# Veason-silverbullet/NNR

Hardware: AMD Instinct MI355X
Metric: training impressions/sec on MIND-200k (CNE+SUE, bs=64) (higher is better)
Workload: dtype f32

## Files before the change

include/nnr_hip.h:

```cpp
#ifndef NNR_HIP_H
#define NNR_HIP_H
#include <stdint.h>
#include <hip/hip_runtime_api.h>

#ifdef __cplusplus
extern "C" {
#endif

#define NNR_OK 0
#define NNR_ERR_ARG (-1)
#define NNR_ERR_LAUNCH (-2)
#define NNR_ERR_UNSUPPORTED (-3)

int nnr_version(void);

typedef struct nnr_gemm_args {
  const float* A;
  const float* B;
  float* C;
  int M, N, K;
  int lda, ldb, ldc;
  int trans_a, trans_b;
  const int* dyn_dev;
  int dyn_dim;
  const int* a_idx;
  const int* b_idx;
  int drop_target;
  float drop_p;
  uint32_t drop_seed;
  int drop_cols;
  float alpha;
  const float* bias;
  const float* rowvec;
  int ldrv;
  const int* rowvec_map;
  int act;
  float* aux_out;
  int ldaux;
  const float* mul;
  int ldmul;
  const float* resid;
  int ldres;
  int accumulate;
  int atomic;
  const int* c_idx;
  int split_k;
  const float* rowdot_w;
  float* rowdot_out;
  int batch;
  long strideA, strideB, strideC, stride_aux, stride_res;
  int k_chunk;
  float* colsum_out;
  int tile;
  uint32_t drop_thresh;
  float drop_scale;
  int vec_epi;
  int sched;
  float* slab;
  long slab_floats;
  int slab_mode;
  const float* pre_add;
  int ldpre;
  int gate_bwd;
  const void* B3;
  long b3_stride;
  int ldb3;
} nnr_gemm_args;

int nnr_gemm_f32(const nnr_gemm_args* args, hipStream_t stream);
int nnr_split_bf16x3(const float* w, int rows, int cols, int ld, int ldo, void* out3, long img_stride, hipStream_t stream);

int nnr_seq_plan(uint8_t* mask, const int* ids, int n, int L, const int* perm_in, int* len_out, int* order, int* rank, int* slen,
                 int* bs, int* off, int* row_seq, int* tok, int* prev_f, int* prev_r, hipStream_t stream);

int nnr_seq_plan_pair(uint8_t* mask0, const int* ids0, int n0, uint8_t* mask1, const int* ids1, int n1, int L, const int* perm_in,
                      int* len_out, int* order, int* rank, int* slen, int* bs, int* off, int* row_seq, int* tok, int* prev_f,
                      int* prev_r, hipStream_t stream);

int nnr_cne_pair_map(const int* order_t, const int* order_c, int n0, int n, int* pm_t, int* pm_c, int* tmp, hipStream_t stream);

int nnr_mask_cover(const uint8_t* mask, int n, int L, uint8_t* cover, hipStream_t stream);
int nnr_seq_rowmap(const int* off, const int* rank, const int* len, int n, int L, int* rowmap, hipStream_t stream);

int nnr_lstm_dims(int H, int* UB, int* HP, int* NP);
int nnr_lstm_pack_weights(const float* w_ih_f, const float* w_hh_f, const float* b_ih_f, const float* b_hh_f, const float* w_ih_r,
                          const float* w_hh_r, const float* b_ih_r, const float* b_hh_r, int H, int E, float* w_ihp, float* b_p,
                          float* wf, float* wb, float* w_ihp_t, hipStream_t stream);
int nnr_lstm_unpack_grads(float* dw_ihp, float* db_p, float* dw_hhp, int H, int E, float* dw_ih_f, float* dw_hh_f,
                          float* db_ih_f, float* db_hh_f, float* dw_ih_r, float* dw_hh_r, float* db_ih_r, float* db_hh_r,
                          int accumulate , int zero_src, hipStream_t stream);
typedef struct nnr_lstm_problem {
  const int* bs; const int* off; const int* slen; const int* prev_f; const int* prev_r;
  int n, L;
  float* gates;
  float* cell;
  float* hout;
  float* cn;
  const float* wf;
  const float* wb;
  const float* dh;
  const float* dcn;
  unsigned* sync;
} nnr_lstm_problem;
size_t nnr_lstm_sync_bytes(int n);
size_t nnr_lstm_sync_diag_offset(int n);
int nnr_lstm_set_timeout_counter(unsigned* dev_counter);
int nnr_lstm_fwd(const nnr_lstm_problem* probs, int nprob, int H, hipStream_t stream);
int nnr_lstm_bwd(const nnr_lstm_problem* probs, int nprob, int H, hipStream_t stream);

typedef struct nnr_pool_args {
  const float* x; int ldx; int D; int n; int L;
  int packed;
  const int* off; const int* slen; const int* order;
  const uint8_t* mask; int mask_div;
  const float* score;
  const float* v; int ldv; float scale;
  float* alpha;
  float* out; int ldo; const float* add_in; int ldadd;
  const float* dout; int lddo; const float* dout2; int lddo2;
  float* dx; int lddx; int dx_accumulate;
  float* dscore;
  float* dv; int lddv;
  const float* th; int ldth; int A; const float* w2;
  const float* alpha_b; const float* dout_b; int lddo_b; const float* dscore_b; const float* v_b; int ldv_b; float scale_b;
} nnr_pool_args;
int nnr_attn_pool_fwd(const nnr_pool_args* a, hipStream_t stream);
int nnr_attn_pool_bwd(const nnr_pool_args* a, hipStream_t stream);

int nnr_gate_bwd(const float* dHt, const float* H, const float* G, float* dH, float* dpre, const int* rows_dev, int rows, int cols,
                 hipStream_t stream);
int nnr_packed_seq_sum(const float* x, int D, const int* off, const int* slen, int n, float* out, hipStream_t stream);
int nnr_slot_workspace_floats(int N);
int nnr_tanh_score_bwd(float* th, const float* ds, const float* w2, float* dw2, const int* rows_dev, int rows, int A, float* ws,
                       hipStream_t stream);
int nnr_colsum(const float* x, int ld, const int* rows_dev, int rows, int N, float* out_accum, float* ws, hipStream_t stream);
int nnr_rowdot(const float* x, int ld, const float* w, const int* rows_dev, int rows, int N, float* out,
               hipStream_t stream);
int nnr_small_embed_fwd(const float* table, const int* idx, int n, int dim, float* out, int ldo, float p, uint32_t seed,
                        hipStream_t stream);
int nnr_small_embed_bwd(const int* idx, int n, int dim, const float* dout, int lddo, float* dtable_accum, float p, uint32_t seed,
                        hipStream_t stream);
int nnr_embed_gather(const float* table, const int* idx, long n, const int* n_dev , int dim, float* out,
                     float p, uint32_t seed, hipStream_t stream);
int nnr_embed_scatter(const float* dout, const int* idx, long n, int dim, float* dtable_accum, float p, uint32_t seed,
                      hipStream_t stream);
int nnr_embed_scatter_dyn(const float* dout, const int* idx, long n, const int* n_dev, int dim, float* dtable, float p, uint32_t seed,
                          hipStream_t stream);
size_t nnr_token_sort_workspace_bytes(long cap, int vocab);
int nnr_token_sort(const int* tok, long cap, const int* n_dev, int vocab, unsigned* keys_tmp, int* rows_tmp, unsigned* keys_sorted,
                   int* rows_sorted, void* temp, size_t temp_bytes, hipStream_t stream);
size_t nnr_embed_scatter_sorted_workspace_floats(long cap);
int nnr_embed_scatter_sorted(const float* dout, const unsigned* keys_sorted, const int* rows_sorted, long cap, int vocab, int dim,
                             float* dtable_accum, float p, uint32_t seed, float* partial_ws, hipStream_t stream);
int nnr_transpose2d(const float* in, float* out, long rows, int cols, int accumulate, hipStream_t stream);
typedef struct nnr_transpose_desc { const float* in; float* out; int rows, cols; } nnr_transpose_desc;
int nnr_transpose_batch(const nnr_transpose_desc* descs_dev, int count, hipStream_t stream);
int nnr_add(float* y, const float* x, long n, float alpha, hipStream_t stream);
int nnr_add_atomic(float* y, const float* x, long n, float alpha, hipStream_t stream);
int nnr_add2d(float* y, int ldy, const float* x, int ldx, int rows, int cols, float alpha, int accumulate, hipStream_t stream);
int nnr_expand_rows_fwd(const float* x, float* y, int B, int N, int D, hipStream_t stream);
int nnr_expand_rows_bwd(const float* dy, float* dx, int B, int N, int D, hipStream_t stream);
int nnr_dropout(const float* x, float* y, long n, float p, uint32_t seed, hipStream_t stream);
int nnr_relu_bwd(const float* dy, const float* y, float* dx, long n, hipStream_t stream);
int nnr_gcn_aggregate_fwd(const float* graph, const float* z, const float* bias, const float* resid, float* r_out, float* y, int B, int G,
                          int D, int relu, float p, uint32_t seed, hipStream_t stream);
int nnr_gcn_aggregate_bwd(const float* graph, const float* dy, const float* r, float* ds, float* dx0, float* dz, int B, int G, int D, float p,
                          uint32_t seed, hipStream_t stream);
int nnr_relu_drop_bwd(const float* dy, const float* r, float* ds, float* dx, long n, float p, uint32_t seed, hipStream_t stream);

int nnr_mhsa_fwd(const float* qkv, const uint8_t* mask, int n, int Lq, int heads, int dh, float scale, float* out, float* prob,
                 float drop_p, uint32_t seed, hipStream_t stream);
int nnr_mhsa_bwd(const float* qkv, const uint8_t* mask, const float* prob, const float* dout, int n, int Lq, int heads, int dh,
                 float scale, float* dqkv, float drop_p, uint32_t seed, hipStream_t stream);
int nnr_mhsa_fwd_packed(const float* qkv, const uint8_t* mask, const int* rowmap, int n, int Lq, int heads, int dh, float scale, float* out,
                        float drop_p, uint32_t seed, hipStream_t stream);
int nnr_mhsa_bwd_packed(const float* qkv, const uint8_t* mask, const int* rowmap, const float* dout, int n, int Lq, int heads, int dh, float scale,
                        float* dqkv, float drop_p, uint32_t seed, hipStream_t stream);
int nnr_mhsa_pair_map(const int* off, const int* slen, const int* order, const uint8_t* mask, int n, int L, int* vrowmap, uint8_t* vmask,
                      hipStream_t stream);
int nnr_mhsa_fwd_paired(const float* qkv, const uint8_t* vmask, const int* vrowmap, const int* off, int n, int heads, int dh, float scale,
                        float* out, float drop_p, uint32_t seed, hipStream_t stream);
int nnr_mhsa_bwd_paired(const float* qkv, const uint8_t* vmask, const int* vrowmap, const int* off, const float* dout, int n, int heads, int dh,
                        float scale, float* dqkv, float drop_p, uint32_t seed, hipStream_t stream);

int nnr_sue_x0_fwd(const float* hist, const float* proxy, float* x0, int B, int Hn, int Kc, int D, float p, uint32_t seed,
                   uint8_t* cmask_fix, hipStream_t stream);
int nnr_sue_x0_bwd(const float* dx0, const float* dx0_add, float* dhist, float* dproxy_accum, int B, int Hn, int Kc, int D, float p,
                   uint32_t seed, hipStream_t stream);
int nnr_sue_slice_fwd(const float* gcn, const float* x0, float* gfeat, int B, int Hn, int G, int D, hipStream_t stream);
int nnr_sue_slice_bwd(const float* dgfeat, float* dpad, int B, int Hn, int G, int D, hipStream_t stream);
int nnr_sue_intra_fwd(const float* kf, const float* qc, const float* g, const long* cidx, int B, int N, int Hn, int C, int A, int D,
                      float* alpha, float* feat, hipStream_t stream);
int nnr_sue_intra_bwd(const float* kf, const float* qc, const float* g, const long* cidx, const float* alpha, const float* dfeat, int B,
                      int N, int Hn, int C, int A, int D, float* dg, float* dkf, float* dqc, float* ds_ws ,
                      hipStream_t stream);

int nnr_cand_attn_ws_floats(int B, int N, int H, int A);
int nnr_cand_attn_fwd(const float* P, const float* Q, const float* w2, const float* feat, int ldf, const uint8_t* mask, int B, int N,
                      int H, int A, int D, int act, float* alpha, float* out, hipStream_t stream);
int nnr_cand_attn_bwd(const float* P, const float* Q, const float* w2, const float* feat, int ldf, const uint8_t* mask, const float* alpha,
                      const float* dout, int B, int N, int H, int A, int D, int act, float* dP, float* dQ, float* dfeat,
                      int dfeat_accumulate, float* ws, float* dw2_accum, hipStream_t stream);

int nnr_omap_ws_floats(int B, int N, int H, int D, int K);
int nnr_omap_fwd(const float* hist, int ldf, const float* cand, const uint8_t* mask, const float* W, int B, int N, int H, int D, int K,
                 float* alpha, float* Y, float* beta, float* R, float* gamma, float* out, float* ws, hipStream_t stream);
int nnr_omap_bwd(const float* hist, int ldf, const float* cand, const uint8_t* mask, const float* W, const float* alpha, const float* Y,
                 const float* beta, const float* R, const float* gamma, const float* dout, int B, int N, int H, int D, int K, float* dhist,
                 int dhist_accumulate, float* dcand, float* dW_accum, float* ws, hipStream_t stream);
int nnr_omap_reg_fwd(const float* W, int D, int K, float coef, float* off, float* loss, hipStream_t stream);
int nnr_omap_reg_bwd(const float* W, const float* off, const float* gup, int D, int K, float coef, float* dW_accum, hipStream_t stream);

typedef struct nnr_corpus_tables {
  const int* news_category; const int* news_subCategory;
  const int* title_text; const uint8_t* title_mask; const int* title_entity;
  const int* abstract_text; const uint8_t* abstract_mask; const int* abstract_entity;
  const long* beh_user; const int* beh_history; const uint8_t* beh_history_mask; const int* beh_line;
  const float* graph_table; const uint8_t* cmask_table; const long* cidx_table;
  int T, C, H, G, K1;
} nnr_corpus_tables;
typedef struct nnr_batch_out {
  long* user_id;
  int* u_cat; int* u_sub; int* u_tt; uint8_t* u_tm; int* u_te; int* u_ct; uint8_t* u_cm; int* u_ce;
  uint8_t* u_hmask; float* u_graph; uint8_t* u_cmask; long* u_cidx;
  int* n_cat; int* n_sub; int* n_tt; uint8_t* n_tm; int* n_te; int* n_ct; uint8_t* n_cm; int* n_ce;
} nnr_batch_out;
int nnr_corpus_batch(const nnr_corpus_tables* t, const nnr_batch_out* o, const int* beh_idx, const int* samples, int ld_samples, int B,
                     int S, hipStream_t stream);
int nnr_history_graph(const int* cats, const uint8_t* hmask, int B, int H, int K, int norm, float* graph, uint8_t* cmask, long* cidx,
                      hipStream_t stream);
int nnr_rank_metrics(const float* scores, const uint8_t* labels, const long* offsets, int n_impressions, int* ranks,
                     double* per_impression, hipStream_t stream);

int nnr_logits_loss_fwd(const float* user, const float* cand, int B, int N, int D, float* logits, float* loss, float* dlogits,
                        hipStream_t stream);
int nnr_logits_fwd(const float* user, const float* cand, int B, int N, int D, float* logits, hipStream_t stream);
int nnr_nls_loss(const float* logits, int B, int N, float* loss, float* dlogits, hipStream_t stream);
int nnr_logits_bwd(const float* dlogits, const float* user, const float* cand, int B, int N, int D, float* duser, float* dcand,
                   int dcand_accumulate, hipStream_t stream);
int nnr_layernorm_fwd(const float* u, const float* gamma, const float* beta, float eps, long rows, int D, float* xhat, float* rstd,
                      float* r_out, const float* resid, float* y, float p, uint32_t seed, hipStream_t stream);
int nnr_layernorm_bwd(const float* dv, const float* xhat, const float* rstd, const float* gamma, long rows, int D, float* du,
                      float* dgamma, float* dbeta, hipStream_t stream);
int nnr_sumsq(const float* g, long n, float* out, hipStream_t stream);
int nnr_sumsq_part(const float* g, long n, float* out, const float* add_in, int slot, hipStream_t stream);
int nnr_clip_adam(float* p, const float* g, float* m, float* v, long n, const float* sumsq, float grad_scale, float clip, float lr,
                  float beta1, float beta2, float eps, float weight_decay, int step, hipStream_t stream);

int nnr_adam_skipped_steps(unsigned* host_out, int reset);
int nnr_adam_skipped_peek(unsigned* host_out);

typedef struct nnr_dp_ctx nnr_dp_ctx;
int nnr_dp_unique_id(void* out128);
int nnr_dp_init(const void* uid128, int rank, int world, nnr_dp_ctx** ctx);
int nnr_dp_allreduce(nnr_dp_ctx* ctx, float* flat, size_t n, hipStream_t stream);
int nnr_dp_broadcast(nnr_dp_ctx* ctx, float* flat, size_t n, int root, hipStream_t stream);
int nnr_dp_destroy(nnr_dp_ctx* ctx);
int nnr_dp_emulate_ranks(nnr_dp_ctx* ctx, int ranks);
int nnr_dp_busy(float* buf, long n, int workgroups, int iters, hipStream_t stream);
int nnr_rows_touch(const int* tok, long cap, const int* n_dev, int V, float* flags, hipStream_t stream);
int nnr_rows_compact(const float* flags, int V, int* pos, int* count, hipStream_t stream);
int nnr_rows_pack(const float* dense, const int* pos, int V, int E, float* packed, hipStream_t stream);
int nnr_rows_unpack(const float* packed, const int* pos, int V, int E, float* dense, hipStream_t stream);

int nnr_fusion_rows_fwd(const float* cat_table, const float* sub_table, const int* cat0, const int* sub0, int n0, const int* cat1,
                        const int* sub1, int n1, int cd, int sd, float* out, int ldo, float p, uint32_t seed_cat, uint32_t seed_sub,
                        hipStream_t stream);
int nnr_fusion_rows_bwd(const int* cat0, const int* sub0, int n0, const int* cat1, const int* sub1, int n1, int cd, int sd, const float* dout,
                        int lddo, float* dcat_table_accum, float* dsub_table_accum, float p, uint32_t seed_cat, uint32_t seed_sub,
                        hipStream_t stream);
int nnr_fusion_rows_bwd_det(const int* cat0, const int* sub0, int n0, const int* cat1, const int* sub1, int n1, int cd, int sd, int ncat,
                            int nsub, const float* dout, int lddo, float* dcat_table_accum, float* dsub_table_accum, float p,
                            uint32_t seed_cat, uint32_t seed_sub, hipStream_t stream);
int nnr_click_loss(const float* user, const float* cand, int B, int N, int D, float* logits, float* loss, float* dlogits, float* duser,
                   float* dcand, float* terms_ws, hipStream_t stream);

int nnr_fill_zero(void* p, size_t bytes, hipStream_t stream);
int nnr_copy_bytes(void* dst, const void* src, size_t bytes, hipStream_t stream);
int nnr_fill_column_u8(uint8_t* m, int rows, int cols, int col, int value, hipStream_t stream);

typedef struct nnr_tape nnr_tape;
int nnr_tape_create(nnr_tape** out);
int nnr_tape_destroy(nnr_tape* t);
int nnr_tape_fn_id(const char* entry_point_name);
int nnr_tape_fn_nargs(int fn);
int nnr_tape_call(nnr_tape* t, int fn, hipStream_t stream, const uint64_t* slots, int nslots, const int* blob_slot,
                  const void* const* blob_ptr, const size_t* blob_bytes, int nblobs, int tag, size_t* slot_off_out, size_t* blob_off_out);
int nnr_tape_wait_stream(nnr_tape* t, hipStream_t waiter, hipStream_t signaller);
int nnr_tape_event_record(nnr_tape* t, uint64_t key, hipStream_t s);
int nnr_tape_event_wait(nnr_tape* t, hipStream_t s, uint64_t key);
int nnr_tape_segment(nnr_tape* t);
int nnr_tape_patch(nnr_tape* t, size_t arena_byte_off, int kind, int width, int64_t addend);
int nnr_tape_finalize(nnr_tape* t);
int nnr_tape_prepare_timing(nnr_tape* t, int nsets);
int nnr_tape_info(const nnr_tape* t, int* calls, int* ops, int* segments, int* streams, size_t* arena_bytes);
int nnr_tape_replay(nnr_tape* t, int segment, const uint64_t* values, int nvalues, const uint64_t* inputs, int ninputs, int timing_set);
int nnr_tape_timings(nnr_tape* t, int set, float* ms, int n);
int nnr_tape_timeline(nnr_tape* t, int set, float* start_ms, float* dur_ms, int* stream_idx, int n);
int nnr_tape_last_error(const nnr_tape* t, int* rc, int* call, char* name, int name_cap);

#ifdef __cplusplus
}
#endif
#endif
```

nnr_amd/_lib.py:

```python
import ctypes as C
import os
import subprocess

_HERE = os.path.dirname(os.path.abspath(__file__))
LIB_PATH = os.environ.get('NNR_HIP_LIB') or os.path.join(_HERE, 'libnnr_hip.so')
_lib = None

vp, ci, cf, cu32, cl = C.c_void_p, C.c_int, C.c_float, C.c_uint32, C.c_long


class GemmArgs(C.Structure):
    _fields_ = [('A', vp), ('B', vp), ('C', vp), ('M', ci), ('N', ci), ('K', ci), ('lda', ci), ('ldb', ci), ('ldc', ci),
                ('trans_a', ci), ('trans_b', ci), ('dyn_dev', vp), ('dyn_dim', ci), ('a_idx', vp), ('b_idx', vp),
                ('drop_target', ci), ('drop_p', cf), ('drop_seed', cu32), ('drop_cols', ci), ('alpha', cf), ('bias', vp),
                ('rowvec', vp), ('ldrv', ci), ('rowvec_map', vp), ('act', ci), ('aux_out', vp), ('ldaux', ci), ('mul', vp),
                ('ldmul', ci), ('resid', vp), ('ldres', ci), ('accumulate', ci), ('atomic', ci), ('c_idx', vp),
                ('split_k', ci), ('rowdot_w', vp), ('rowdot_out', vp), ('batch', ci), ('strideA', cl), ('strideB', cl),
                ('strideC', cl), ('stride_aux', cl), ('stride_res', cl), ('k_chunk', ci), ('colsum_out', vp), ('tile', ci), ('drop_thresh', cu32),
                ('drop_scale', cf), ('vec_epi', ci), ('sched', ci), ('slab', vp), ('slab_floats', cl), ('slab_mode', ci), ('pre_add', vp), ('ldpre', ci), ('gate_bwd', ci), ('B3', vp), ('b3_stride', cl), ('ldb3', ci)]


class LstmProblem(C.Structure):
    _fields_ = [('bs', vp), ('off', vp), ('slen', vp), ('prev_f', vp), ('prev_r', vp), ('n', ci), ('L', ci), ('gates', vp),
                ('cell', vp), ('hout', vp), ('cn', vp), ('wf', vp), ('wb', vp), ('dh', vp), ('dcn', vp), ('sync', vp)]


class TransposeDesc(C.Structure):
    _fields_ = [('inp', vp), ('out', vp), ('rows', ci), ('cols', ci)]


class CorpusTables(C.Structure):
    _fields_ = [(k, vp) for k in ('news_category', 'news_subCategory', 'title_text', 'title_mask', 'title_entity', 'abstract_text',
                                  'abstract_mask', 'abstract_entity', 'beh_user', 'beh_history', 'beh_history_mask', 'beh_line',
                                  'graph_table', 'cmask_table', 'cidx_table')] + [(k, ci) for k in ('T', 'C', 'H', 'G', 'K1')]


class BatchOut(C.Structure):
    _fields_ = [(k, vp) for k in ('user_id', 'u_cat', 'u_sub', 'u_tt', 'u_tm', 'u_te', 'u_ct', 'u_cm', 'u_ce', 'u_hmask', 'u_graph',
                                  'u_cmask', 'u_cidx', 'n_cat', 'n_sub', 'n_tt', 'n_tm', 'n_te', 'n_ct', 'n_cm', 'n_ce')]


class PoolArgs(C.Structure):
    _fields_ = [('x', vp), ('ldx', ci), ('D', ci), ('n', ci), ('L', ci), ('packed', ci), ('off', vp), ('slen', vp),
                ('order', vp), ('mask', vp), ('mask_div', ci), ('score', vp), ('v', vp), ('ldv', ci), ('scale', cf),
                ('alpha', vp), ('out', vp), ('ldo', ci), ('add_in', vp), ('ldadd', ci), ('dout', vp), ('lddo', ci),
                ('dout2', vp), ('lddo2', ci), ('dx', vp), ('lddx', ci), ('dx_accumulate', ci), ('dscore', vp), ('dv', vp),
                ('lddv', ci), ('th', vp), ('ldth', ci), ('A', ci), ('w2', vp),
                ('alpha_b', vp), ('dout_b', vp), ('lddo_b', ci), ('dscore_b', vp), ('v_b', vp), ('ldv_b', ci), ('scale_b', cf)]


SIGNATURES = {
    'nnr_version': 'i32',
    'nnr_gemm_f32': 'i32 GemmArgs stream',
    'nnr_split_bf16x3': 'i32 ptr i32 i32 i32 i32 ptr i64 stream',
    'nnr_seq_plan': 'i32 ptr ptr i32 i32 ptr ptr ptr ptr ptr ptr ptr ptr ptr ptr ptr stream',
    'nnr_seq_plan_pair': 'i32 ptr ptr i32 ptr ptr i32 i32 ptr ptr ptr ptr ptr ptr ptr ptr ptr ptr ptr stream',
    'nnr_cne_pair_map': 'i32 ptr ptr i32 i32 ptr ptr ptr stream',
    'nnr_mask_cover': 'i32 ptr i32 i32 ptr stream',
    'nnr_seq_rowmap': 'i32 ptr ptr ptr i32 i32 ptr stream',
    'nnr_lstm_dims': 'i32 i32 ptr ptr ptr',
    'nnr_lstm_pack_weights': 'i32 ptr ptr ptr ptr ptr ptr ptr ptr i32 i32 ptr ptr ptr ptr ptr stream',
    'nnr_lstm_unpack_grads': 'i32 ptr ptr ptr i32 i32 ptr ptr ptr ptr ptr ptr ptr ptr i32 i32 stream',
    'nnr_lstm_sync_bytes': 'u64 i32',
    'nnr_lstm_sync_diag_offset': 'u64 i32',
    'nnr_lstm_set_timeout_counter': 'i32 ptr',
    'nnr_lstm_fwd': 'i32 LstmProblem i32 i32 stream',
    'nnr_lstm_bwd': 'i32 LstmProblem i32 i32 stream',
    'nnr_attn_pool_fwd': 'i32 PoolArgs stream',
    'nnr_attn_pool_bwd': 'i32 PoolArgs stream',
    'nnr_gate_bwd': 'i32 ptr ptr ptr ptr ptr ptr i32 i32 stream',
    'nnr_packed_seq_sum': 'i32 ptr i32 ptr ptr i32 ptr stream',
    'nnr_slot_workspace_floats': 'i32 i32',
    'nnr_tanh_score_bwd': 'i32 ptr ptr ptr ptr ptr i32 i32 ptr stream',
    'nnr_colsum': 'i32 ptr i32 ptr i32 i32 ptr ptr stream',
    'nnr_rowdot': 'i32 ptr i32 ptr ptr i32 i32 ptr stream',
    'nnr_small_embed_fwd': 'i32 ptr ptr i32 i32 ptr i32 f32 seed stream',
    'nnr_small_embed_bwd': 'i32 ptr i32 i32 ptr i32 ptr f32 seed stream',
    'nnr_embed_gather': 'i32 ptr ptr i64 ptr i32 ptr f32 seed stream',
    'nnr_embed_scatter': 'i32 ptr ptr i64 i32 ptr f32 seed stream',
    'nnr_embed_scatter_dyn': 'i32 ptr ptr i64 ptr i32 ptr f32 seed stream',
    'nnr_token_sort_workspace_bytes': 'u64 i64 i32',
    'nnr_token_sort': 'i32 ptr i64 ptr i32 ptr ptr ptr ptr ptr u64 stream',
    'nnr_embed_scatter_sorted_workspace_floats': 'u64 i64',
    'nnr_embed_scatter_sorted': 'i32 ptr ptr ptr i64 i32 i32 ptr f32 seed ptr stream',
    'nnr_transpose2d': 'i32 ptr ptr i64 i32 i32 stream',
    'nnr_transpose_batch': 'i32 TransposeDesc i32 stream',
    'nnr_add': 'i32 ptr ptr i64 f32 stream',
    'nnr_add_atomic': 'i32 ptr ptr i64 f32 stream',
    'nnr_add2d': 'i32 ptr i32 ptr i32 i32 i32 f32 i32 stream',
    'nnr_expand_rows_fwd': 'i32 ptr ptr i32 i32 i32 stream',
    'nnr_expand_rows_bwd': 'i32 ptr ptr i32 i32 i32 stream',
    'nnr_dropout': 'i32 ptr ptr i64 f32 seed stream',
    'nnr_relu_bwd': 'i32 ptr ptr ptr i64 stream',
    'nnr_gcn_aggregate_fwd': 'i32 ptr ptr ptr ptr ptr ptr i32 i32 i32 i32 f32 seed stream',
    'nnr_gcn_aggregate_bwd': 'i32 ptr ptr ptr ptr ptr ptr i32 i32 i32 f32 seed stream',
    'nnr_relu_drop_bwd': 'i32 ptr ptr ptr ptr i64 f32 seed stream',
    'nnr_mhsa_fwd': 'i32 ptr ptr i32 i32 i32 i32 f32 ptr ptr f32 seed stream',
    'nnr_mhsa_bwd': 'i32 ptr ptr ptr ptr i32 i32 i32 i32 f32 ptr f32 seed stream',
    'nnr_mhsa_fwd_packed': 'i32 ptr ptr ptr i32 i32 i32 i32 f32 ptr f32 seed stream',
    'nnr_mhsa_bwd_packed': 'i32 ptr ptr ptr ptr i32 i32 i32 i32 f32 ptr f32 seed stream',
    'nnr_mhsa_pair_map': 'i32 ptr ptr ptr ptr i32 i32 ptr ptr stream',
    'nnr_mhsa_fwd_paired': 'i32 ptr ptr ptr ptr i32 i32 i32 f32 ptr f32 seed stream',
    'nnr_mhsa_bwd_paired': 'i32 ptr ptr ptr ptr ptr i32 i32 i32 f32 ptr f32 seed stream',
    'nnr_sue_x0_fwd': 'i32 ptr ptr ptr i32 i32 i32 i32 f32 seed ptr stream',
    'nnr_sue_x0_bwd': 'i32 ptr ptr ptr ptr i32 i32 i32 i32 f32 seed stream',
    'nnr_sue_slice_fwd': 'i32 ptr ptr ptr i32 i32 i32 i32 stream',
    'nnr_sue_slice_bwd': 'i32 ptr ptr i32 i32 i32 i32 stream',
    'nnr_sue_intra_fwd': 'i32 ptr ptr ptr ptr i32 i32 i32 i32 i32 i32 ptr ptr stream',
    'nnr_sue_intra_bwd': 'i32 ptr ptr ptr ptr ptr ptr i32 i32 i32 i32 i32 i32 ptr ptr ptr ptr stream',
    'nnr_cand_attn_ws_floats': 'i32 i32 i32 i32 i32',
    'nnr_cand_attn_fwd': 'i32 ptr ptr ptr ptr i32 ptr i32 i32 i32 i32 i32 i32 ptr ptr stream',
    'nnr_cand_attn_bwd': 'i32 ptr ptr ptr ptr i32 ptr ptr ptr i32 i32 i32 i32 i32 i32 ptr ptr ptr i32 ptr ptr stream',
    'nnr_omap_ws_floats': 'i32 i32 i32 i32 i32 i32',
    'nnr_omap_fwd': 'i32 ptr i32 ptr ptr ptr i32 i32 i32 i32 i32 ptr ptr ptr ptr ptr ptr ptr stream',
    'nnr_omap_bwd': 'i32 ptr i32 ptr ptr ptr ptr ptr ptr ptr ptr ptr i32 i32 i32 i32 i32 ptr i32 ptr ptr ptr stream',
    'nnr_omap_reg_fwd': 'i32 ptr i32 i32 f32 ptr ptr stream',
    'nnr_omap_reg_bwd': 'i32 ptr ptr ptr i32 i32 f32 ptr stream',
    'nnr_corpus_batch': 'i32 CorpusTables BatchOut ptr ptr i32 i32 i32 stream',
    'nnr_history_graph': 'i32 ptr ptr i32 i32 i32 i32 ptr ptr ptr stream',
    'nnr_rank_metrics': 'i32 ptr ptr ptr i32 ptr ptr stream',
    'nnr_logits_loss_fwd': 'i32 ptr ptr i32 i32 i32 ptr ptr ptr stream',
    'nnr_logits_fwd': 'i32 ptr ptr i32 i32 i32 ptr stream',
    'nnr_nls_loss': 'i32 ptr i32 i32 ptr ptr stream',
    'nnr_logits_bwd': 'i32 ptr ptr ptr i32 i32 i32 ptr ptr i32 stream',
    'nnr_layernorm_fwd': 'i32 ptr ptr ptr f32 i64 i32 ptr ptr ptr ptr ptr f32 seed stream',
    'nnr_layernorm_bwd': 'i32 ptr ptr ptr ptr i64 i32 ptr ptr ptr stream',
    'nnr_sumsq': 'i32 ptr i64 ptr stream',
    'nnr_sumsq_part': 'i32 ptr i64 ptr ptr i32 stream',
    'nnr_clip_adam': 'i32 ptr ptr ptr ptr i64 ptr f32 f32 f32 f32 f32 f32 f32 i32 stream',
    'nnr_adam_skipped_steps': 'i32 ptr i32',
    'nnr_adam_skipped_peek': 'i32 ptr',
    'nnr_dp_unique_id': 'i32 ptr',
    'nnr_dp_init': 'i32 ptr i32 i32 handle',
    'nnr_dp_allreduce': 'i32 handle ptr u64 stream',
    'nnr_dp_broadcast': 'i32 handle ptr u64 i32 stream',
    'nnr_dp_destroy': 'i32 handle',
    'nnr_dp_emulate_ranks': 'i32 handle i32',
    'nnr_dp_busy': 'i32 ptr i64 i32 i32 stream',
    'nnr_rows_touch': 'i32 ptr i64 ptr i32 ptr stream',
    'nnr_rows_compact': 'i32 ptr i32 ptr ptr stream',
    'nnr_rows_pack': 'i32 ptr ptr i32 i32 ptr stream',
    'nnr_rows_unpack': 'i32 ptr ptr i32 i32 ptr stream',
    'nnr_fusion_rows_fwd': 'i32 ptr ptr ptr ptr i32 ptr ptr i32 i32 i32 ptr i32 f32 seed seed stream',
    'nnr_fusion_rows_bwd': 'i32 ptr ptr i32 ptr ptr i32 i32 i32 ptr i32 ptr ptr f32 seed seed stream',
    'nnr_fusion_rows_bwd_det': 'i32 ptr ptr i32 ptr ptr i32 i32 i32 i32 i32 ptr i32 ptr ptr f32 seed seed stream',
    'nnr_click_loss': 'i32 ptr ptr i32 i32 i32 ptr ptr ptr ptr ptr ptr stream',
    'nnr_fill_zero': 'i32 ptr u64 stream',
    'nnr_copy_bytes': 'i32 ptr ptr u64 stream',
    'nnr_fill_column_u8': 'i32 ptr i32 i32 i32 i32 stream',
    'nnr_tape_create': 'i32 handle',
    'nnr_tape_destroy': 'i32 handle',
    'nnr_tape_fn_id': 'i32 cstr',
    'nnr_tape_fn_nargs': 'i32 i32',
    'nnr_tape_call': 'i32 handle i32 stream ptr i32 ptr ptr ptr i32 i32 ptr ptr',
    'nnr_tape_wait_stream': 'i32 handle stream stream',
    'nnr_tape_event_record': 'i32 handle u64 stream',
    'nnr_tape_event_wait': 'i32 handle stream u64',
    'nnr_tape_segment': 'i32 handle',
    'nnr_tape_patch': 'i32 handle u64 i32 i32 i64',
    'nnr_tape_finalize': 'i32 handle',
    'nnr_tape_prepare_timing': 'i32 handle i32',
    'nnr_tape_info': 'i32 handle ptr ptr ptr ptr ptr',
    'nnr_tape_replay': 'i32 handle i32 ptr i32 ptr i32 i32',
    'nnr_tape_timings': 'i32 handle i32 ptr i32',
    'nnr_tape_timeline': 'i32 handle i32 ptr ptr ptr i32',
    'nnr_tape_last_error': 'i32 handle ptr ptr cstr i32',
}
SYMBOLS = list(SIGNATURES)
STRUCTS = {'nnr_gemm_args': GemmArgs, 'nnr_lstm_problem': LstmProblem, 'nnr_pool_args': PoolArgs, 'nnr_transpose_desc': TransposeDesc,
           'nnr_corpus_tables': CorpusTables, 'nnr_batch_out': BatchOut}
DEVICE_STRUCTS = {'TransposeDesc'}
_CTYPES = {'i32': ci, 'i64': cl, 'u64': C.c_size_t, 'f32': cf, 'seed': cu32, 'ptr': vp, 'handle': vp, 'cstr': C.c_char_p, 'stream': vp}
_CTYPES.update((c.__name__, vp if c.__name__ in DEVICE_STRUCTS else C.POINTER(c)) for c in STRUCTS.values())


def kinds(name):
    return SIGNATURES[name].split()[1:]


class NnrHipError(RuntimeError):
    pass


def build(force=False):
    if force:
        bdir = os.path.join(_HERE, 'csrc', 'build')
        if os.path.isdir(bdir):
            for f in os.listdir(bdir):
                os.remove(os.path.join(bdir, f))
    subprocess.check_call(['bash', os.path.join(_HERE, 'csrc', 'build.sh')])
    return LIB_PATH


def lib():
    global _lib
    if _lib is None:
        if not os.path.exists(LIB_PATH):
            raise NnrHipError('libnnr_hip.so not found at %s -- run `python -c "import __graft_entry__ as g; g.build()"` '
                              '(there is no CPU / PyTorch fallback on the product path)' % LIB_PATH)
        import torch
        _lib = C.CDLL(LIB_PATH)
        for name, sig in SIGNATURES.items():
            ret, *params = [_CTYPES[k] for k in sig.split()]
            fn = getattr(_lib, name)
            fn.restype, fn.argtypes = ret, params
    return _lib


def build_id():
    import hashlib
    h = hashlib.sha256()
    src = os.path.join(_HERE, 'csrc')
    for f in sorted(os.listdir(src)):
        if f.endswith(('.hip', '.h')):
            h.update(f.encode())
            h.update(open(os.path.join(src, f), 'rb').read())
    h.update(open(os.path.join(os.path.dirname(_HERE), 'include', 'nnr_hip.h'), 'rb').read())
    lib_hash = hashlib.sha256(open(LIB_PATH, 'rb').read()).hexdigest()[:16] if os.path.exists(LIB_PATH) else None
    return {'src_sha256': h.hexdigest()[:16], 'lib_sha256': lib_hash}


CALLS = [0]


def check(rc, what):
    CALLS[0] += 1
    if rc != 0:
        raise NnrHipError('%s failed with code %d' % (what, rc))
```

nnr_amd/csrc/gcn.hip:

```cpp
#include "common.h"

namespace {

constexpr int GCN_MAXG = 128;

template <int MODE, int MT>
__global__ __launch_bounds__(256) __attribute__((amdgpu_waves_per_eu(3, 8))) void gcn_aggregate_kernel(
    const float* __restrict__ graph, const float* __restrict__ in, const float* __restrict__ bias, const float* __restrict__ aux_in,
    float* __restrict__ out0, float* __restrict__ out1, float* __restrict__ out2, int G, int D, int relu, uint32_t seed, uint32_t thr, float scale) {
  extern __shared__ __attribute__((aligned(16))) float sm[];
  const int ks_n = (G + 3) >> 2, GR = ks_n * 4;
  const int A_LD = GR | 1;
  constexpr int Z_LD = 68;
  float* As = sm;
  float* Zs = sm + ((GR * A_LD + 3) & ~3);
  const int b = blockIdx.y, tid = threadIdx.x, lane = tid & 63, w = tid >> 6;
  const int r16 = lane & 15, kk = lane >> 4;
  const float* A = graph + (long)b * G * G;
  if ((G & 3) == 0) {
    const int g4 = G >> 2;
    for (int i = tid; i < G * g4; i += 256) {
      const int row = i / g4, c = (i - row * g4) * 4;
      const f32x4 v = *reinterpret_cast<const f32x4*>(A + row * G + c);
#pragma unroll
      for (int e = 0; e < 4; ++e) As[row * A_LD + c + e] = v[e];
    }
  } else {
    for (int i = tid; i < GR * A_LD; i += 256) {
      const int row = i / A_LD, col = i - row * A_LD;
      As[i] = (row < G && col < G) ? A[row * G + col] : 0.f;
    }
  }
  const int c0 = blockIdx.x * 64;
  const int c4 = (tid & 15) * 4, rr = tid >> 4;
  const bool cok = c0 + c4 < D;
  const long base = (long)b * G * D;
#pragma unroll
  for (int pass = 0; pass < MT; ++pass) {
    const int row = pass * 16 + rr;
    f32x4 v = {0.f, 0.f, 0.f, 0.f};
    if (row < G && cok) {
      const long idx = base + (long)row * D + c0 + c4;
      v = *reinterpret_cast<const f32x4*>(in + idx);
      if (MODE == 1 && aux_in) {
        if (thr) {
          bool kp[4];
          nnr_keep4(seed, (uint64_t)idx, thr, kp);
#pragma unroll
          for (int e = 0; e < 4; ++e) v[e] = kp[e] ? v[e] * scale : 0.f;
        }
        if (out1) *reinterpret_cast<f32x4*>(out1 + idx) = v;
        const f32x4 rv = *reinterpret_cast<const f32x4*>(aux_in + idx);
#pragma unroll
        for (int e = 0; e < 4; ++e) v[e] = rv[e] > 0.f ? v[e] : 0.f;
        *reinterpret_cast<f32x4*>(out0 + idx) = v;
      }
    }
    if (row < GR) *reinterpret_cast<f32x4*>(&Zs[row * Z_LD + c4]) = v;
  }
  __syncthreads();
  float bf[MT * 4];
#pragma unroll
  for (int ks = 0; ks < MT * 4; ++ks) bf[ks] = ks < ks_n ? Zs[(4 * ks + kk) * Z_LD + w * 16 + r16] : 0.f;
  f32x4 acc[MT];
  int arow[MT];
#pragma unroll
  for (int m = 0; m < MT; ++m) {
    acc[m] = f32x4{0.f, 0.f, 0.f, 0.f};
    arow[m] = min(m * 16 + r16, GR - 1);
  }
#pragma unroll
  for (int ks = 0; ks < MT * 4; ++ks) {
    if (ks < ks_n) {
#pragma unroll
      for (int m = 0; m < MT; ++m) {
        const float a = MODE == 0 ? As[arow[m] * A_LD + 4 * ks + kk] : As[(4 * ks + kk) * A_LD + arow[m]];
        acc[m] = __builtin_amdgcn_mfma_f32_16x16x4f32(a, bf[ks], acc[m], 0, 0, 0);
      }
    }
  }
  __syncthreads();
#pragma unroll
  for (int m = 0; m < MT; ++m)
#pragma unroll
    for (int e = 0; e < 4; ++e)
      if (m * 16 + 4 * kk + e < GR) Zs[(m * 16 + 4 * kk + e) * Z_LD + w * 16 + r16] = acc[m][e];
  __syncthreads();
  if (!cok) return;
  f32x4 bv = {0.f, 0.f, 0.f, 0.f};
  if (MODE == 0 && bias) bv = *reinterpret_cast<const f32x4*>(bias + c0 + c4);
#pragma unroll
  for (int pass = 0; pass < MT; ++pass) {
    const int row = pass * 16 + rr;
    if (row < G) {
      const long idx = base + (long)row * D + c0 + c4;
      f32x4 x = *reinterpret_cast<const f32x4*>(&Zs[row * Z_LD + c4]);
      if (MODE == 0) {
        x += bv;
        if (relu) {
#pragma unroll
          for (int e = 0; e < 4; ++e) x[e] = fmaxf(x[e], 0.f);
        }
        if (out1) *reinterpret_cast<f32x4*>(out1 + idx) = x;
        if (aux_in) x += *reinterpret_cast<const f32x4*>(aux_in + idx);
        if (thr) {
          bool kp[4];
          nnr_keep4(seed, (uint64_t)idx, thr, kp);
#pragma unroll
          for (int e = 0; e < 4; ++e) x[e] = kp[e] ? x[e] * scale : 0.f;
        }
        *reinterpret_cast<f32x4*>(out0 + idx) = x;
      } else {
        *reinterpret_cast<f32x4*>(out2 + idx) = x;
      }
    }
  }
}


}

extern "C" int nnr_gcn_aggregate_fwd(const float* graph, const float* z, const float* bias, const float* resid, float* r_out, float* y, int B,
                                     int G, int D, int relu, float p, uint32_t seed, hipStream_t stream) {
  if (!graph || !z || !y || B <= 0 || G <= 0 || D <= 0) return NNR_ERR_ARG;
  if (G > GCN_MAXG || (D & 3)) return NNR_ERR_UNSUPPORTED;
  const float sc = p > 0.f ? 1.f / (1.f - p) : 1.f;
  const int gp = (G + 15) / 16 * 16, gr = (G + 3) / 4 * 4;
#define GCN_CASE(MT_) case MT_: hipLaunchKernelGGL((gcn_aggregate_kernel<0, MT_>), dim3((D + 63) / 64, B), dim3(256), (size_t)(((gr * (gr | 1) + 3) & ~3) + gr * 68) * sizeof(float), \
                                                   stream, graph, z, bias, resid, y, r_out, nullptr, G, D, relu, seed, nnr_drop_thresh(p), sc); break;
  switch (gp / 16) { GCN_CASE(1) GCN_CASE(2) GCN_CASE(3) GCN_CASE(4) GCN_CASE(5) GCN_CASE(6) GCN_CASE(7) GCN_CASE(8) }
#undef GCN_CASE
  NNR_CHECK_LAUNCH();
  return NNR_OK;
}

extern "C" int nnr_gcn_aggregate_bwd(const float* graph, const float* dy, const float* r, float* ds, float* dx0, float* dz, int B, int G, int D,
                                     float p, uint32_t seed, hipStream_t stream) {
  if (!graph || !dy || !dz || B <= 0 || G <= 0 || D <= 0 || (r && !ds)) return NNR_ERR_ARG;
  if (G > GCN_MAXG || (D & 3)) return NNR_ERR_UNSUPPORTED;
  const float sc = p > 0.f ? 1.f / (1.f - p) : 1.f;
  const int gp = (G + 15) / 16 * 16, gr = (G + 3) / 4 * 4;
#define GCN_CASE(MT_) case MT_: hipLaunchKernelGGL((gcn_aggregate_kernel<1, MT_>), dim3((D + 63) / 64, B), dim3(256), (size_t)(((gr * (gr | 1) + 3) & ~3) + gr * 68) * sizeof(float), \
                                                   stream, graph, dy, nullptr, r, ds, dx0, dz, G, D, 0, seed, nnr_drop_thresh(p), sc); break;
  switch (gp / 16) { GCN_CASE(1) GCN_CASE(2) GCN_CASE(3) GCN_CASE(4) GCN_CASE(5) GCN_CASE(6) GCN_CASE(7) GCN_CASE(8) }
#undef GCN_CASE
  NNR_CHECK_LAUNCH();
  return NNR_OK;
}
```

nnr_amd/csrc/gemm.hip:

```cpp
#include "common.h"
#include <stdlib.h>
#include <type_traits>

namespace {

template <int BK>
__device__ __forceinline__ int swz(int r16) {
  return BK == 16 ? ((4 - (r16 >> 2)) & 3) : BK == 32 ? ((r16 >> 1) & 7) : (r16 & 15);
}

template <int TM, int TN>
__device__ __forceinline__ void gemm_epilogue(const nnr_gemm_args& g, f32x4 (&acc)[TM][TN], float* lds, float* __restrict__ C, int m0,
                                              int n0, int M, int N, int z) {
  constexpr int BN = 16 * TN, E_LD = BN + 4;
  const int tid = threadIdx.x, lane = tid & 63, w = tid >> 6;
  const int r = lane & 15, kk = lane >> 4;
  const uint32_t dthr = g.drop_thresh;
  const float dscale = g.drop_scale;
  const bool use_atomic = !g.slab_mode && (g.atomic || g.split_k > 1 || g.k_chunk > 0);
  float* aux = g.aux_out;
  const float* res = g.resid;
  const float* mulp = g.mul;
  if (g.batch > 1 && g.split_k <= 1 && g.k_chunk <= 0) {
    if (aux) aux += (long)z * g.stride_aux;
    if (res) res += (long)z * g.stride_res;
  }
  float* stage = lds;
#pragma unroll
  for (int m = 0; m < TM; ++m) {
    if (m > 0) __syncthreads();
#pragma unroll
    for (int n = 0; n < TN; ++n)
#pragma unroll
      for (int reg = 0; reg < 4; ++reg) stage[(w * 16 + kk * 4 + reg) * E_LD + n * 16 + r] = acc[m][n][reg];
    __syncthreads();
    if (g.rowdot_w) {
      for (int lr = w; lr < 64; lr += 4) {
        const int row = m0 + (lr >> 4) * (TM * 16) + m * 16 + (lr & 15);
        float dot = 0.f;
        if (row < M) {
          for (int c = lane; c < BN; c += 64) {
            const int col = n0 + c;
            if (col < N) {
              float x = stage[lr * E_LD + c] * g.alpha;
              if (g.bias) x += g.bias[col];
              if (g.act == 1) x = fmaxf(x, 0.f);
              else if (g.act == 2) x = fast_tanh(x);
              else if (g.act == 3) x = fast_sigmoid(x);
              if (aux) aux[(long)row * g.ldaux + col] = x;
              dot += g.rowdot_w[col] * x;
              if (C) C[(long)row * g.ldc + col] = x;
            }
          }
        }
        dot = wave_sum(dot);
        if (row < M && lane == 0) g.rowdot_out[row] = dot;
      }
    } else if (g.vec_epi) {
      constexpr int NV = BN / 4;
      for (int idx = tid; idx < 64 * NV; idx += 256) {
        const int lr = idx / NV, c4 = idx - lr * NV;
        const int row = m0 + (lr >> 4) * (TM * 16) + m * 16 + (lr & 15);
        const int col = n0 + 4 * c4;
        if (row >= M || col >= N) continue;
        f32x4 x = *reinterpret_cast<const f32x4*>(&stage[lr * E_LD + 4 * c4]) * g.alpha;
        if (g.pre_add) x += *reinterpret_cast<const f32x4*>(g.pre_add + (long)row * g.ldpre + col);
        if (g.gate_bwd) {
          const f32x4 gv = *reinterpret_cast<const f32x4*>(mulp + (long)row * g.ldmul + col);
          const f32x4 hv = *reinterpret_cast<const f32x4*>(res + (long)row * g.ldres + col);
          *reinterpret_cast<f32x4*>(aux + (long)row * g.ldaux + col) = x * hv * gv * (1.f - gv);
          *reinterpret_cast<f32x4*>(C + (long)row * g.ldc + col) = x * gv;
          continue;
        }
        if (g.accumulate == 2) x += *reinterpret_cast<const f32x4*>(C + (long)row * g.ldc + col);
        if (g.bias) x += *reinterpret_cast<const f32x4*>(g.bias + col);
        if (g.rowvec) x += *reinterpret_cast<const f32x4*>(g.rowvec + (long)(g.rowvec_map ? g.rowvec_map[row] : row) * g.ldrv + col);
        if (g.act == 1) {
#pragma unroll
          for (int e = 0; e < 4; ++e) x[e] = fmaxf(x[e], 0.f);
        } else if (g.act == 2) {
#pragma unroll
          for (int e = 0; e < 4; ++e) x[e] = fast_tanh(x[e]);
        } else if (g.act == 3) {
#pragma unroll
          for (int e = 0; e < 4; ++e) x[e] = fast_sigmoid(x[e]);
        }
        if (aux) *reinterpret_cast<f32x4*>(aux + (long)row * g.ldaux + col) = x;
        if (mulp) x *= *reinterpret_cast<const f32x4*>(mulp + (long)row * g.ldmul + col);
        if (res) x += *reinterpret_cast<const f32x4*>(res + (long)row * g.ldres + col);
        if (g.drop_target == 3) {
          bool kp[4];
          nnr_keep4(g.drop_seed, (uint64_t)(row + (long)z * g.M) * g.drop_cols + col, dthr, kp);
#pragma unroll
          for (int e = 0; e < 4; ++e) x[e] = kp[e] ? x[e] * dscale : 0.f;
        }
        if (C) {
          f32x4* cp = reinterpret_cast<f32x4*>(C + (long)row * g.ldc + col);
          if (g.accumulate == 1) x += *cp;
          *cp = x;
        }
      }
    } else {
      for (int idx = tid; idx < 64 * BN; idx += 256) {
        const int lr = idx / BN, c = idx - lr * BN;
        const int row = m0 + (lr >> 4) * (TM * 16) + m * 16 + (lr & 15);
        const int col = n0 + c;
        if (row >= M || col >= N) continue;
        int crow = row;
        if (g.c_idx) { crow = g.c_idx[row]; if (crow < 0) continue; }
        float x = stage[lr * E_LD + c] * g.alpha;
        if (g.accumulate == 2) x += C[(long)crow * g.ldc + col];
        if (g.bias) x += g.bias[col];
        if (g.rowvec) x += g.rowvec[(long)(g.rowvec_map ? g.rowvec_map[row] : row) * g.ldrv + col];
        if (g.act == 1) x = fmaxf(x, 0.f);
        else if (g.act == 2) x = fast_tanh(x);
        else if (g.act == 3) x = fast_sigmoid(x);
        if (aux) aux[(long)row * g.ldaux + col] = x;
        if (mulp) x *= mulp[(long)row * g.ldmul + col];
        if (res) x += res[(long)row * g.ldres + col];
        if (g.drop_target == 3)
          x = nnr_keep(g.drop_seed, (uint64_t)(row + (long)z * g.M) * g.drop_cols + col, dthr) ? x * dscale : 0.f;
        if (C) {
          float* cp = C + (long)crow * g.ldc + col;
          if (use_atomic) {
            if (g.drop_target == 4)
              x = nnr_keep(g.drop_seed, (uint64_t)row * g.drop_cols + col, dthr) ? x * dscale : 0.f;
            atomicAdd(cp, x);
          } else {
            if (g.accumulate == 1) x += *cp;
            *cp = x;
          }
        }
      }
    }
  }
}

template <int TM, int TN, bool TA, bool TB, int BK>
__global__ __launch_bounds__(256) void gemm_kernel(nnr_gemm_args g) {
  constexpr int BM = 64 * TM, BN = 16 * TN;
  constexpr int A_LD = BM + 4, B_LD = BN + 4;
  constexpr int KQ = BK / 4, NKG = BK / 16;
  constexpr int A_SZ = TA ? BK * A_LD : BM * BK;
  constexpr int B_SZ = TB ? BK * B_LD : BN * BK;
  constexpr int NAL = BM * KQ / 256;
  constexpr int NBL = (BN * KQ + 255) / 256;
  constexpr int E_LD = BN + 4;
  constexpr int LDS_FLOATS = (2 * (A_SZ + B_SZ) > 64 * E_LD) ? 2 * (A_SZ + B_SZ) : 64 * E_LD;
  __shared__ __attribute__((aligned(16))) float lds[LDS_FLOATS];

  const int tid = threadIdx.x, lane = tid & 63, w = tid >> 6;
  const int r = lane & 15, kk = lane >> 4;

// ... 127 lines not shown
              if (vecB && gn + 3 < N) {
                val = *reinterpret_cast<const f32x4*>(p);
              } else {
#pragma unroll
                for (int e = 0; e < 4; ++e) if (gn + e < N) val[e] = p[e];
              }
              if (g.drop_target == 2) {
                bool kp[4];
                if ((g.drop_cols & 3) == 0) nnr_keep4(g.drop_seed, (uint64_t)gk * g.drop_cols + gn, dthr, kp);
                else {
#pragma unroll
                  for (int e = 0; e < 4; ++e) kp[e] = nnr_keep(g.drop_seed, (uint64_t)gk * g.drop_cols + (gn + e), dthr);
                }
#pragma unroll
                for (int e = 0; e < 4; ++e) val[e] = kp[e] ? val[e] * dscale : 0.f;
              }
            }
          }
        }
      }
      rb[j] = val;
    }
  };

  auto store_tiles = [&](int buf) {
    float* As = lds + buf * (A_SZ + B_SZ);
    float* Bs = As + A_SZ;
#pragma unroll
    for (int j = 0; j < NAL; ++j) {
      const int f = tid + 256 * j;
      if (!TA) {
        const int row = f / KQ, kq = f % KQ;
        *reinterpret_cast<f32x4*>(&As[row * BK + 4 * (kq ^ swz<BK>(row & 15))]) = ra[j];
      } else {
        const int kr = f / (BM / 4), mq = f - kr * (BM / 4);
        *reinterpret_cast<f32x4*>(&As[kr * A_LD + 4 * mq]) = ra[j];
      }
    }
#pragma unroll
    for (int j = 0; j < NBL; ++j) {
      const int f = tid + 256 * j;
      if (f < BN * KQ || TB) {
        if (!TB) {
          const int row = f / KQ, kq = f % KQ;
          *reinterpret_cast<f32x4*>(&Bs[row * BK + 4 * (kq ^ swz<BK>(row & 15))]) = rb[j];
        } else {
          const int kr = f / (BN / 4), nq = f - kr * (BN / 4);
          if (kr < BK) *reinterpret_cast<f32x4*>(&Bs[kr * B_LD + 4 * nq]) = rb[j];
        }
      }
    }
  };

  f32x4 acc[TM][TN];
#pragma unroll
  for (int m = 0; m < TM; ++m)
#pragma unroll
    for (int n = 0; n < TN; ++n) acc[m][n] = f32x4{0.f, 0.f, 0.f, 0.f};

  load_tiles(kbeg);
  if (do_colsum) {
#pragma unroll
    for (int j = 0; j < NAL; ++j) csum[j] += ra[j];
  }
  store_tiles(0);
  __syncthreads();

  int buf = 0;
  for (int k0 = kbeg; k0 < kend; k0 += BK) {
    const bool more = (k0 + BK) < kend;
    if (more) {
      load_tiles(k0 + BK);
      if (do_colsum) {
#pragma unroll
        for (int j = 0; j < NAL; ++j) csum[j] += ra[j];
      }
    }

    const float* As = lds + buf * (A_SZ + B_SZ);
    const float* Bs = As + A_SZ;
#pragma unroll
    for (int kg2 = 0; kg2 < NKG; ++kg2) {
      f32x4 af[TM], bf[TN];
#pragma unroll
      for (int m = 0; m < TM; ++m) {
        if (!TA) {
          af[m] = *reinterpret_cast<const f32x4*>(&As[((w * TM + m) * 16 + r) * BK + 4 * ((kg2 * 4 + kk) ^ swz<BK>(r))]);
        } else {
#pragma unroll
          for (int i = 0; i < 4; ++i) af[m][i] = As[(kg2 * 16 + 4 * kk + i) * A_LD + (w * TM + m) * 16 + r];
        }
      }
#pragma unroll
      for (int n = 0; n < TN; ++n) {
        if (!TB) {
          bf[n] = *reinterpret_cast<const f32x4*>(&Bs[(n * 16 + r) * BK + 4 * ((kg2 * 4 + kk) ^ swz<BK>(r))]);
        } else {
#pragma unroll
          for (int i = 0; i < 4; ++i) bf[n][i] = Bs[(kg2 * 16 + 4 * kk + i) * B_LD + n * 16 + r];
        }
      }
#pragma unroll
      for (int i = 0; i < 4; ++i)
#pragma unroll
        for (int m = 0; m < TM; ++m)
#pragma unroll
          for (int n = 0; n < TN; ++n)
            acc[m][n] = __builtin_amdgcn_mfma_f32_16x16x4f32(af[m][i], bf[n][i], acc[m][n], 0, 0, 0);
    }

    if (more) store_tiles(buf ^ 1);
    __syncthreads();
    buf ^= 1;
  }

  if (do_colsum) {
    float* red = lds;
#pragma unroll
    for (int j = 0; j < NAL; ++j) {
      const int f = tid + 256 * j, kr = f / (BM / 4), mq = f - kr * (BM / 4);
      *reinterpret_cast<f32x4*>(&red[kr * BM + 4 * mq]) = csum[j];
    }
    __syncthreads();
    for (int i = tid; i < BM; i += 256) {
      float t = 0.f;
      for (int kr = 0; kr < BK; ++kr) t += red[kr * BM + i];
      if (m0 + i < M) {
        if (g.slab_mode) g.colsum_out[(long)z * M + m0 + i] = t;
        else atomicAdd(&g.colsum_out[m0 + i], t);
      }
    }
    __syncthreads();
  }

  gemm_epilogue<TM, TN>(g, acc, lds, g.slab_mode ? C + (long)z * M * N : C, m0, n0, M, N, z);
}

template <int TM, int TN, int BK>
int launch_cfg(const nnr_gemm_args& g, hipStream_t s) {
  constexpr int BM = 64 * TM, BN = 16 * TN;
  const int nbm = (g.M + BM - 1) / BM, nbn = (g.N + BN - 1) / BN;
  if (g.rowdot_w && nbn != 1) return NNR_ERR_ARG;
  dim3 grid(nbm * nbn, 1, g.k_chunk > 0 ? (g.K + g.k_chunk - 1) / g.k_chunk : (g.split_k > 1 ? g.split_k : (g.batch > 1 ? g.batch : 1)));
  dim3 block(256);
  if (!g.trans_a && !g.trans_b) hipLaunchKernelGGL((gemm_kernel<TM, TN, false, false, BK>), grid, block, 0, s, g);
  else if (!g.trans_a && g.trans_b) hipLaunchKernelGGL((gemm_kernel<TM, TN, false, true, BK>), grid, block, 0, s, g);
  else if (g.trans_a && g.trans_b) hipLaunchKernelGGL((gemm_kernel<TM, TN, true, true, BK>), grid, block, 0, s, g);
  else return NNR_ERR_ARG;
  NNR_CHECK_LAUNCH();
  return NNR_OK;
}


__device__ __attribute__((aligned(1024))) float nnr_zero_page[512] = {};

__device__ __forceinline__ void lds_dma16(const float* gsrc, unsigned lds_dst) {
  unsigned keep;
  asm volatile("s_mov_b32 %0, m0\n\ts_mov_b32 m0, %2\n\ts_nop 0\n\tglobal_load_lds_dwordx4 %1, off\n\ts_mov_b32 m0, %0"
               : "=&s"(keep) : "v"(gsrc), "s"(lds_dst) : "memory");
}
__device__ __forceinline__ void set_prio_dyn(unsigned p) {
  switch (p & 3) {
    case 0: __builtin_amdgcn_s_setprio(0); break;
    case 1: __builtin_amdgcn_s_setprio(1); break;
    case 2: __builtin_amdgcn_s_setprio(2); break;
    default: __builtin_amdgcn_s_setprio(3); break;
  }
}

template <int N>
__device__ __forceinline__ void wait_vmcnt() { asm volatile("s_waitcnt vmcnt(%0)" ::"n"(N) : "memory"); }
template <int CNT, int MAXA>
__device__ __forceinline__ void wait_stages(int ahead) {
  if constexpr (MAXA == 0) wait_vmcnt<0>();
  else {
    if (ahead >= MAXA) wait_vmcnt<CNT * MAXA>();
    else wait_stages<CNT, MAXA - 1>(ahead);
  }
}

template <int TM, int TN, int BK, int NS, int OCC, int PRIO = 0>
__global__ __launch_bounds__(256, OCC) void gemm_nt_pipe_kernel(nnr_gemm_args g) {
  if (PRIO == 1) set_prio_dyn(blockIdx.x >> 8);
  if (PRIO == 2) set_prio_dyn(blockIdx.x >> 5);
  if (PRIO == 3) set_prio_dyn(blockIdx.x);
  constexpr int BM = 64 * TM, BN = 16 * TN, ROWS = BM + BN;
  constexpr int KQ = BK / 4, NKG = BK / 16;
  constexpr int RPI = 64 / KQ;
  constexpr int NI = ROWS / RPI;
  constexpr int NPW = (NI + 3) / 4;
  constexpr int STAGE = ROWS * BK;
  constexpr int E_LD = BN + 4;
  constexpr int LDS_FLOATS = (NS * STAGE > 64 * E_LD) ? NS * STAGE : 64 * E_LD;
  static_assert(ROWS % RPI == 0, "tile rows must fill whole DMA instructions");
  __shared__ __attribute__((aligned(1024))) float lds[LDS_FLOATS];

  const int tid = threadIdx.x, lane = tid & 63, w = __builtin_amdgcn_readfirstlane(tid >> 6);
  const int r = lane & 15, kk = lane >> 4;

  int M = g.M;
  if (g.dyn_dim == 1) M = min(M, *g.dyn_dev);
  const int N = g.N, K = g.K;
  const int nbm = (M + BM - 1) / BM, nbn = (N + BN - 1) / BN;
  const int nblk = nbm * nbn;
  if ((int)blockIdx.x >= nblk) return;
  int v;
  {
    const int b = blockIdx.x, q = nblk >> 3, rem = nblk & 7, x = b & 7, slot = b >> 3;
    v = x * q + min(x, rem) + slot;
  }
  const int bm = v / nbn, bn = v - bm * nbn;
  const int m0 = bm * BM, n0 = bn * BN;
  const int z = blockIdx.z;
  const float* __restrict__ A = g.A;
  const float* __restrict__ B = g.B;
  float* __restrict__ C = g.C;
  if (g.batch > 1) {
    A += (long)z * g.strideA;
    B += (long)z * g.strideB;
    C += (long)z * g.strideC;
  }

  const float* rowp[NPW];
  int kch[NPW];
#pragma unroll
  for (int i = 0; i < NPW; ++i) {
    const int q = w + 4 * i;
    const int tr = q * RPI + lane / KQ;
    const int c = (lane % KQ) ^ swz<BK>(tr & 15);
    kch[i] = 4 * c;
    const float* p = nullptr;
    if (q < NI) {
      if (tr < BM) {
        const int gm = m0 + tr;
        if (gm < M) {
          const int src = g.a_idx ? g.a_idx[gm] : gm;
          if (src >= 0) p = A + (long)src * g.lda + 4 * c;
        }
      } else {
        const int gn = n0 + (tr - BM);
        if (gn < N) p = B + (long)gn * g.ldb + 4 * c;
      }
    }
    rowp[i] = p;
  }
  const float* zero = nnr_zero_page;
  asm volatile("" : "+s"(zero));
  const unsigned lds_base = (unsigned)(uintptr_t)lds;
  const int S = (K + BK - 1) / BK;

  auto issue = [&](int s) {
    const int k0 = s * BK;
    const unsigned sb = lds_base + (unsigned)((s % NS) * STAGE * 4);
#pragma unroll
    for (int i = 0; i < NPW; ++i) {
      const int q = w + 4 * i;
      if (q < NI) {
        const float* src = (rowp[i] != nullptr && k0 + kch[i] < K) ? rowp[i] + k0 : zero;
        lds_dma16(src, sb + (unsigned)(q * 1024));
      }
    }
  };

  f32x4 acc[TM][TN];
#pragma unroll
  for (int m = 0; m < TM; ++m)
#pragma unroll
    for (int n = 0; n < TN; ++n) acc[m][n] = f32x4{0.f, 0.f, 0.f, 0.f};

#pragma unroll
  for (int s = 0; s < NS - 1; ++s)
    if (s < S) issue(s);

  const int nv = (g.sched & 1) ? min(TN, (N - n0 + 15) >> 4) : TN;
  auto run = [&](auto full_tag) {
    constexpr bool FULL = decltype(full_tag)::value;
    for (int s = 0; s < S; ++s) {
      const int ahead = S - 1 - s;
      if (NI % 4 == 0 || w < NI % 4) wait_stages<NPW, NS - 2>(ahead);
      else wait_stages<NPW - 1, NS - 2>(ahead);
      __builtin_amdgcn_s_barrier();
      if (s + NS - 1 < S) issue(s + NS - 1);

      const float* As = lds + (s % NS) * STAGE;
      const float* Bs = As + BM * BK;
#pragma unroll
      for (int kg = 0; kg < NKG; ++kg) {
        f32x4 af[TM], bf[TN];
#pragma unroll
        for (int m = 0; m < TM; ++m)
          af[m] = *reinterpret_cast<const f32x4*>(&As[((w * TM + m) * 16 + r) * BK + 4 * ((kg * 4 + kk) ^ swz<BK>(r))]);
        if constexpr (FULL) {
#pragma unroll
          for (int n = 0; n < TN; ++n)
            bf[n] = *reinterpret_cast<const f32x4*>(&Bs[(n * 16 + r) * BK + 4 * ((kg * 4 + kk) ^ swz<BK>(r))]);
#pragma unroll
          for (int i = 0; i < 4; ++i)
#pragma unroll
            for (int m = 0; m < TM; ++m)
#pragma unroll
              for (int n = 0; n < TN; ++n)
                acc[m][n] = __builtin_amdgcn_mfma_f32_16x16x4f32(af[m][i], bf[n][i], acc[m][n], 0, 0, 0);
        } else {
#pragma unroll
          for (int n = 0; n < TN; ++n)
            if (n < nv) bf[n] = *reinterpret_cast<const f32x4*>(&Bs[(n * 16 + r) * BK + 4 * ((kg * 4 + kk) ^ swz<BK>(r))]);
#pragma unroll
          for (int n = 0; n < TN; ++n)
            if (n < nv) {
#pragma unroll
              for (int i = 0; i < 4; ++i)
#pragma unroll
                for (int m = 0; m < TM; ++m) acc[m][n] = __builtin_amdgcn_mfma_f32_16x16x4f32(af[m][i], bf[n][i], acc[m][n], 0, 0, 0);
            }
        }
      }
    }
  };
  if (nv == TN) run(std::true_type{});
  else run(std::false_type{});
  __syncthreads();
  gemm_epilogue<TM, TN>(g, acc, lds, C, m0, n0, M, N, z);
}

template <int N>
__device__ __forceinline__ void lds_dma16_block(const float* sbase, unsigned lds_dst, const unsigned (&voff)[8]) {
  unsigned keep;
  static_assert(N >= 1 && N <= 8, "1..8 loads per block");
#define NNR_DMA_HEAD "s_mov_b32 %[keep], m0\n\ts_mov_b32 m0, %[dst]\n\t"
#define NNR_DMA_LD(I) "s_nop 0\n\tglobal_load_lds_dwordx4 %[v" #I "], %[sb]\n\ts_add_u32 m0, m0, 0x1000\n\t"
#define NNR_DMA_TAIL "s_mov_b32 m0, %[keep]"
#define NNR_DMA_OPS : [keep] "=&s"(keep) : [dst] "s"(lds_dst), [sb] "s"(sbase), [v0] "v"(voff[0]), [v1] "v"(voff[1]), [v2] "v"(voff[2]), [v3] "v"(voff[3]), \
                      [v4] "v"(voff[4]), [v5] "v"(voff[5]), [v6] "v"(voff[6]), [v7] "v"(voff[7]) : "memory", "scc"
  if constexpr (N == 1) asm volatile(NNR_DMA_HEAD NNR_DMA_LD(0) NNR_DMA_TAIL NNR_DMA_OPS);
  if constexpr (N == 2) asm volatile(NNR_DMA_HEAD NNR_DMA_LD(0) NNR_DMA_LD(1) NNR_DMA_TAIL NNR_DMA_OPS);
  if constexpr (N == 3) asm volatile(NNR_DMA_HEAD NNR_DMA_LD(0) NNR_DMA_LD(1) NNR_DMA_LD(2) NNR_DMA_TAIL NNR_DMA_OPS);
  if constexpr (N == 4) asm volatile(NNR_DMA_HEAD NNR_DMA_LD(0) NNR_DMA_LD(1) NNR_DMA_LD(2) NNR_DMA_LD(3) NNR_DMA_TAIL NNR_DMA_OPS);
  if constexpr (N == 5) asm volatile(NNR_DMA_HEAD NNR_DMA_LD(0) NNR_DMA_LD(1) NNR_DMA_LD(2) NNR_DMA_LD(3) NNR_DMA_LD(4) NNR_DMA_TAIL NNR_DMA_OPS);
  if constexpr (N == 6) asm volatile(NNR_DMA_HEAD NNR_DMA_LD(0) NNR_DMA_LD(1) NNR_DMA_LD(2) NNR_DMA_LD(3) NNR_DMA_LD(4) NNR_DMA_LD(5) NNR_DMA_TAIL NNR_DMA_OPS);
  if constexpr (N == 7) asm volatile(NNR_DMA_HEAD NNR_DMA_LD(0) NNR_DMA_LD(1) NNR_DMA_LD(2) NNR_DMA_LD(3) NNR_DMA_LD(4) NNR_DMA_LD(5) NNR_DMA_LD(6) NNR_DMA_TAIL NNR_DMA_OPS);
  if constexpr (N == 8) asm volatile(NNR_DMA_HEAD NNR_DMA_LD(0) NNR_DMA_LD(1) NNR_DMA_LD(2) NNR_DMA_LD(3) NNR_DMA_LD(4) NNR_DMA_LD(5) NNR_DMA_LD(6) NNR_DMA_LD(7) NNR_DMA_TAIL NNR_DMA_OPS);
#undef NNR_DMA_HEAD
#undef NNR_DMA_LD
#undef NNR_DMA_TAIL
#undef NNR_DMA_OPS
}

template <int TM, int TN, int NS, int OCC>
__global__ __launch_bounds__(256, OCC) void gemm_nt_pipe2_kernel(nnr_gemm_args g) {
  constexpr int BK = 32, BM = 64 * TM, BN = 16 * TN, ROWS = BM + BN;
  constexpr int KQ = BK / 4, RPI = 64 / KQ, NI = ROWS / RPI, NPW = (NI + 3) / 4, STAGE = ROWS * BK, E_LD = BN + 4;
  constexpr int LDS_FLOATS = (NS * STAGE > 64 * E_LD) ? NS * STAGE : 64 * E_LD;
  static_assert(ROWS % RPI == 0 && NS >= 3, "tile shape");
  __shared__ __attribute__((aligned(1024))) float lds[LDS_FLOATS];
  const int tid = threadIdx.x, lane = tid & 63, w = __builtin_amdgcn_readfirstlane(tid >> 6);
  const int r = lane & 15, kk = lane >> 4;
  int M = g.M;
  if (g.dyn_dim == 1) M = min(M, *g.dyn_dev);
  const int N = g.N, K = g.K;
  const int nbm = (M + BM - 1) / BM, nbn = (N + BN - 1) / BN;
  const int nblk = nbm * nbn;
  if ((int)blockIdx.x >= nblk) return;
  int v;
  {
    const int b = blockIdx.x, q = nblk >> 3, rem = nblk & 7, x = b & 7, slot = b >> 3;
    v = x * q + min(x, rem) + slot;
  }
  const int bm = v / nbn, bn = v - bm * nbn;
  const int m0 = bm * BM, n0 = bn * BN;
  const int z = blockIdx.z;
  const float* __restrict__ A = g.A;
  const float* __restrict__ B = g.B;
  float* __restrict__ C = g.C;
  if (g.batch > 1) {
    A += (long)z * g.strideA;
    B += (long)z * g.strideB;
    C += (long)z * g.strideC;
  }
  constexpr int NIA = BM / RPI, NIB = BN / RPI, NA = NIA / 4, NBMAX = (NIB + 3) / 4;
  static_assert(NIA % 4 == 0 && NA <= 8 && NBMAX <= 8, "tile shape");
  unsigned voffA[8], voffB[8];
  int kchA[NA], kchB[NBMAX];
#pragma unroll
  for (int i = 0; i < 8; ++i) voffA[i] = voffB[i] = 0;
#pragma unroll
  for (int i = 0; i < NA; ++i) {
    const int tr = (w + 4 * i) * RPI + lane / KQ;
    const int c = (lane % KQ) ^ swz<BK>(tr & 15);
    kchA[i] = 4 * c;
    voffA[i] = (unsigned)(((long)min(tr, M - 1 - m0) * g.lda + 4 * c) * 4);
  }
#pragma unroll
  for (int j = 0; j < NBMAX; ++j) {
    const int tr = (w + 4 * j) * RPI + lane / KQ;
    const int c = (lane % KQ) ^ swz<BK>(tr & 15);
    kchB[j] = 4 * c;
    voffB[j] = (unsigned)(((long)min(tr, N - 1 - n0) * g.ldb + 4 * c) * 4);
  }
  const float* zero = nnr_zero_page;
  asm volatile("" : "+s"(zero));
  const unsigned lds_base = (unsigned)(uintptr_t)lds;
  const int S = (K + BK - 1) / BK;
  const float* Abase = A + (long)m0 * g.lda;
  const float* Bbase = B + (long)n0 * g.ldb;
  const bool ktail = (K % BK) != 0;
  const bool nb_hi = (NIB % 4 == 0) || (w < NIB % 4);
  auto issue_lean = [&](int s) {
    const int k0 = s * BK;
    const unsigned sb = lds_base + (unsigned)((s % NS) * STAGE * 4) + (unsigned)(w * 1024);
    lds_dma16_block<NA>(Abase + k0, sb, voffA);
    if (nb_hi) lds_dma16_block<NBMAX>(Bbase + k0, sb + NIA * 1024, voffB);
    else if constexpr (NBMAX > 1) lds_dma16_block<NBMAX - 1>(Bbase + k0, sb + NIA * 1024, voffB);
  };
  auto issue = [&](int s) {
    if (!(ktail && s == S - 1)) { issue_lean(s); return; }
    const int k0 = s * BK;
    const unsigned sb = lds_base + (unsigned)((s % NS) * STAGE * 4) + (unsigned)(w * 1024);
#pragma unroll
    for (int i = 0; i < NA; ++i)
      lds_dma16((k0 + kchA[i] < K) ? reinterpret_cast<const float*>(reinterpret_cast<const char*>(Abase + k0) + voffA[i]) : zero, sb + i * 4096);
#pragma unroll
    for (int j = 0; j < NBMAX; ++j)
      if (j < NBMAX - 1 || nb_hi)
        lds_dma16((k0 + kchB[j] < K) ? reinterpret_cast<const float*>(reinterpret_cast<const char*>(Bbase + k0) + voffB[j]) : zero,
                  sb + NIA * 1024 + j * 4096);
  };
  auto wait_landed = [&](int ahead) {
    if (NI % 4 == 0 || w < NI % 4) wait_stages<NPW, NS - 3>(ahead);
    else wait_stages<NPW - 1, NS - 3>(ahead);
  };
  f32x4 acc[TM][TN];
#pragma unroll
  for (int m = 0; m < TM; ++m)
#pragma unroll
    for (int n = 0; n < TN; ++n) acc[m][n] = f32x4{0.f, 0.f, 0.f, 0.f};
  f32x4 fa0[TM], fb0[TN], fa1[TM], fb1[TN];
  const int nv = (g.sched & 1) ? min(TN, (N - n0 + 15) >> 4) : TN;
  const int klast = (g.sched & 1) ? K - (S - 1) * BK : BK;
  auto run = [&](auto full_tag) {
    constexpr bool FULL = decltype(full_tag)::value;
    auto rd = [&](int s, int kg, f32x4 (&a)[TM], f32x4 (&b)[TN]) {
      const float* As = lds + (s % NS) * STAGE;
      const float* Bs = As + BM * BK;
#pragma unroll
      for (int m = 0; m < TM; ++m)
        a[m] = *reinterpret_cast<const f32x4*>(&As[((w * TM + m) * 16 + r) * BK + 4 * ((kg * 4 + kk) ^ swz<BK>(r))]);
#pragma unroll
      for (int n = 0; n < TN; ++n)
        if (FULL || n < nv) b[n] = *reinterpret_cast<const f32x4*>(&Bs[(n * 16 + r) * BK + 4 * ((kg * 4 + kk) ^ swz<BK>(r))]);
    };
    auto mm = [&](const f32x4 (&a)[TM], const f32x4 (&b)[TN], int steps) {
      if constexpr (FULL) {
#pragma unroll
        for (int i = 0; i < 4; ++i)
          if (i < steps) {
#pragma unroll
            for (int m = 0; m < TM; ++m)
#pragma unroll
              for (int n = 0; n < TN; ++n) acc[m][n] = __builtin_amdgcn_mfma_f32_16x16x4f32(a[m][i], b[n][i], acc[m][n], 0, 0, 0);
          }
      } else {
#pragma unroll
        for (int n = 0; n < TN; ++n)
          if (n < nv) {
#pragma unroll
            for (int i = 0; i < 4; ++i)
              if (i < steps) {
#pragma unroll
                for (int m = 0; m < TM; ++m) acc[m][n] = __builtin_amdgcn_mfma_f32_16x16x4f32(a[m][i], b[n][i], acc[m][n], 0, 0, 0);
              }
          }
      }
    };
    auto mm4 = [&](const f32x4 (&a)[TM], const f32x4 (&b)[TN]) {
      if constexpr (FULL) {
#pragma unroll
        for (int i = 0; i < 4; ++i)
#pragma unroll
          for (int m = 0; m < TM; ++m)
#pragma unroll
            for (int n = 0; n < TN; ++n) acc[m][n] = __builtin_amdgcn_mfma_f32_16x16x4f32(a[m][i], b[n][i], acc[m][n], 0, 0, 0);
      } else {
        mm(a, b, 4);
      }
    };

#pragma unroll
    for (int s = 0; s < NS - 1; ++s)
      if (s < S) issue(s);
    if (NI % 4 == 0 || w < NI % 4) wait_stages<NPW, NS - 2>(S - 1); else wait_stages<NPW - 1, NS - 2>(S - 1);
    __builtin_amdgcn_s_barrier();
    rd(0, 0, fa0, fb0);
    __builtin_amdgcn_s_waitcnt(0xC07F);
#define NNR_LGKM0() do { __builtin_amdgcn_sched_barrier(0); __builtin_amdgcn_s_waitcnt(0xC07F); } while (0)
    int s = 0;
    for (; s + NS < S; ++s) {
      rd(s, 1, fa1, fb1);
      __builtin_amdgcn_sched_barrier(0);
      mm4(fa0, fb0);
      NNR_LGKM0();
      wait_landed(NS);
      __builtin_amdgcn_s_barrier();
      issue_lean(s + NS - 1);
      rd(s + 1, 0, fa0, fb0);
      __builtin_amdgcn_sched_barrier(0);
      mm4(fa1, fb1);
      NNR_LGKM0();
    }
    for (; s + 1 < S; ++s) {
      rd(s, 1, fa1, fb1);
      __builtin_amdgcn_sched_barrier(0);
      mm4(fa0, fb0);
      NNR_LGKM0();
      wait_landed(S - 1 - (s + 1));
      __builtin_amdgcn_s_barrier();
      if (s + NS - 1 < S) issue(s + NS - 1);
      rd(s + 1, 0, fa0, fb0);
      __builtin_amdgcn_sched_barrier(0);
      mm4(fa1, fb1);
      NNR_LGKM0();
    }
#undef NNR_LGKM0
    rd(S - 1, 1, fa1, fb1);
    __builtin_amdgcn_sched_barrier(0);
    mm(fa0, fb0, min(4, klast));
    if (klast > 16) mm(fa1, fb1, min(4, klast - 16));
  };
  if (nv == TN) run(std::true_type{});
  else run(std::false_type{});
  __syncthreads();
  gemm_epilogue<TM, TN>(g, acc, lds, C, m0, n0, M, N, z);
}

constexpr int kNtRagged = 1;

template <int TM, int TN, int NS, int OCC>
int launch_pipe2(const nnr_gemm_args& g0, hipStream_t s) {
  constexpr int BM = 64 * TM, BN = 16 * TN;
  nnr_gemm_args g = g0;
  g.sched = kNtRagged;
  const int nbm = (g.M + BM - 1) / BM, nbn = (g.N + BN - 1) / BN;
  dim3 grid(nbm * nbn, 1, g.batch > 1 ? g.batch : 1), block(256);
  hipLaunchKernelGGL((gemm_nt_pipe2_kernel<TM, TN, NS, OCC>), grid, block, 0, s, g);
  NNR_CHECK_LAUNCH();
  return NNR_OK;
}

template <int TM, int TN, int BK, int NS, int OCC, int PRIO = 0>
int launch_pipe(const nnr_gemm_args& g0, hipStream_t s) {
  constexpr int BM = 64 * TM, BN = 16 * TN;
  nnr_gemm_args g = g0;
  g.sched = kNtRagged;
  const int nbm = (g.M + BM - 1) / BM, nbn = (g.N + BN - 1) / BN;
  dim3 grid(nbm * nbn, 1, g.batch > 1 ? g.batch : 1), block(256);
  hipLaunchKernelGGL((gemm_nt_pipe_kernel<TM, TN, BK, NS, OCC, PRIO>), grid, block, 0, s, g);
  NNR_CHECK_LAUNCH();
  return NNR_OK;
}

static bool pipe_ok(const nnr_gemm_args& g) {
  auto al = [](const void* p) { return ((uintptr_t)p & 15) == 0; };
  return !g.trans_a && !g.trans_b && !g.b_idx && g.split_k <= 1 && g.k_chunk <= 0 && !g.rowdot_w && !g.colsum_out &&
         (g.drop_target == 0 || g.drop_target == 3 || g.drop_target == 4) && (g.K & 3) == 0 && (g.lda & 3) == 0 && (g.ldb & 3) == 0 &&
         al(g.A) && al(g.B) && (g.batch <= 1 || (((g.strideA | g.strideB) & 3) == 0)) && (g.dyn_dim == 0 || g.dyn_dim == 1);
}

typedef __bf16 bf16x8_t __attribute__((ext_vector_type(8)));
__device__ __forceinline__ void split3_bf16(float x, __bf16& h1, __bf16& h2, __bf16& h3) {
  const unsigned u = __builtin_bit_cast(unsigned, x), mag = u & 0x7fffffffu;
  const bool big = mag >= 0x7f7f8000u, nonfinite = mag >= 0x7f800000u;
  h1 = (__bf16)x;
  if (big) h1 = __builtin_bit_cast(__bf16, (unsigned short)((u >> 16) | (mag > 0x7f800000u ? 0x40u : 0u)));
  const float r1 = nonfinite ? 0.f : x - (float)h1;
  h2 = (__bf16)r1;
  const float r2 = r1 - (float)h2;
  h3 = (__bf16)r2;
}
__global__ void split_bf16x3_kernel(const float* __restrict__ w, int rows, int cols, int ld, int ldo, __bf16* __restrict__ out, long img_stride) {
  const long total = (long)rows * ldo;
  for (long i = blockIdx.x * (long)blockDim.x + threadIdx.x; i < total; i += (long)gridDim.x * blockDim.x) {
    const int r = (int)(i / ldo), c = (int)(i - (long)r * ldo);
    __bf16 a, b, d;
    split3_bf16(c < cols ? w[(long)r * ld + c] : 0.f, a, b, d);
    out[i] = a; out[img_stride + i] = b; out[2 * img_stride + i] = d;
  }
}
__device__ __forceinline__ int bx3_swzA(int r) { return ((r >> 1) & 1) | (((r >> 3) & 1) << 2); }
__device__ __forceinline__ int bx3_swzB(int r) { return (r >> 1) & 3; }

typedef unsigned u32x4_t __attribute__((ext_vector_type(4)));
__device__ __forceinline__ unsigned hi16_pair(float odd, float even) {
  return __builtin_amdgcn_perm(__float_as_uint(odd), __float_as_uint(even), 0x07060302u);
}
__device__ __forceinline__ void split3_trunc8(const f32x4& x0, const f32x4& x1, bf16x8_t& a1, bf16x8_t& a2, bf16x8_t& a3) {
  const float xs[8] = {x0[0], x0[1], x0[2], x0[3], x1[0], x1[1], x1[2], x1[3]};
  unsigned w1[4], w2[4], w3[4];
#pragma unroll
  for (int p = 0; p < 4; ++p) {
    const float xe = xs[2 * p], xo = xs[2 * p + 1];
    const unsigned h1 = hi16_pair(xo, xe);
    const float re = xe - __uint_as_float(h1 << 16), ro = xo - __uint_as_float(h1 & 0xffff0000u);
    const unsigned h2 = hi16_pair(ro, re);
    const float se = re - __uint_as_float(h2 << 16), so = ro - __uint_as_float(h2 & 0xffff0000u);
    w1[p] = h1; w2[p] = h2; w3[p] = hi16_pair(so, se);
  }
  a1 = __builtin_bit_cast(bf16x8_t, u32x4_t{w1[0], w1[1], w1[2], w1[3]});
  a2 = __builtin_bit_cast(bf16x8_t, u32x4_t{w2[0], w2[1], w2[2], w2[3]});
  a3 = __builtin_bit_cast(bf16x8_t, u32x4_t{w3[0], w3[1], w3[2], w3[3]});
}

template <int TM, int TN, int NS>
__global__ __launch_bounds__(256, (NS * (64 * TM * 128 + 3 * 16 * TN * 64) > 80 * 1024 ? 1 : 2)) void gemm_nt_bx3_kernel(nnr_gemm_args g) {
  constexpr int BM = 64 * TM, BN = 16 * TN, BK = 32;
  constexpr int A_BYTES = BM * BK * 4, B_IMG_BYTES = BN * BK * 2, STAGE_BYTES = A_BYTES + 3 * B_IMG_BYTES;
  constexpr int NIA = A_BYTES / 1024, NIB1 = B_IMG_BYTES / 1024;
  static_assert(A_BYTES % 1024 == 0 && B_IMG_BYTES % 1024 == 0 && NIA % 4 == 0, "tile shape");
  constexpr int E_LD = BN + 4;
  constexpr int LDS_BYTES = NS * STAGE_BYTES > 64 * E_LD * 4 ? NS * STAGE_BYTES : 64 * E_LD * 4;
  __shared__ __attribute__((aligned(1024))) unsigned char lds_raw[LDS_BYTES];
  const int tid = threadIdx.x, lane = tid & 63, w = __builtin_amdgcn_readfirstlane(tid >> 6), r = lane & 15, q = lane >> 4;
  int M = g.M;
  if (g.dyn_dim == 1) M = min(M, *g.dyn_dev);
  const int N = g.N, K = g.K;
  const int nbm = (M + BM - 1) / BM, nbn = (N + BN - 1) / BN, nblk = nbm * nbn;
  if ((int)blockIdx.x >= nblk) return;
  int v;
  {
    const int b = blockIdx.x, qq = nblk >> 3, rem = nblk & 7, x = b & 7, slot = b >> 3;
    v = x * qq + min(x, rem) + slot;
  }
  const int bm = v / nbn, bn = v - bm * nbn, m0 = bm * BM, n0 = bn * BN;
  const int S = (K + BK - 1) / BK;
  const unsigned lds_base = (unsigned)(uintptr_t)lds_raw;
  const float* zero = nnr_zero_page;
  asm volatile("" : "+s"(zero));
  constexpr int NA = NIA / 4, NBW = (3 * NIB1 + 3) / 4;
  static_assert(NA <= 8 && NBW <= 8, "tile shape");
  unsigned voffA[8], voffB[8];
  int akc[NA], bkc[NBW];
#pragma unroll
  for (int i = 0; i < 8; ++i) voffA[i] = voffB[i] = 0;
#pragma unroll
  for (int i = 0; i < NA; ++i) {
    const int row = (w + 4 * i) * 8 + lane / 8, c = (lane % 8) ^ bx3_swzA(row & 15);
    akc[i] = 4 * c;
    voffA[i] = (unsigned)(((long)min(row, M - 1 - m0) * g.lda + 4 * c) * 4);
  }
#pragma unroll
  for (int j = 0; j < NBW; ++j) {
    const int idx = min(w + 4 * j, 3 * NIB1 - 1);
    const int img = idx / NIB1, jj = idx - img * NIB1, row = jj * 16 + lane / 4, c = (lane % 4) ^ bx3_swzB(row & 15);
    bkc[j] = 8 * c;
    voffB[j] = (unsigned)(((long)img * g.b3_stride + (long)min(row, N - 1 - n0) * g.ldb3 + 8 * c) * 2);
  }
  const float* Abase = g.A + (long)m0 * g.lda;
  const char* Bbase = reinterpret_cast<const char*>(reinterpret_cast<const __bf16*>(g.B3) + (long)n0 * g.ldb3);
  const bool nb_hi = ((3 * NIB1) % 4 == 0) || (w < (3 * NIB1) % 4);
  const bool ktail = (K % BK) != 0;
  auto issue = [&](int s) __attribute__((always_inline)) {
    const int k0 = s * BK;
    const unsigned sb = lds_base + (unsigned)((s % NS) * STAGE_BYTES) + (unsigned)(w * 1024);
    if (!(ktail && s == S - 1)) {
      lds_dma16_block<NA>(Abase + k0, sb, voffA);
      const float* bb = reinterpret_cast<const float*>(Bbase + 2L * k0);
      if (nb_hi) lds_dma16_block<NBW>(bb, sb + A_BYTES, voffB);
      else if constexpr (NBW > 1) lds_dma16_block<NBW - 1>(bb, sb + A_BYTES, voffB);
      return;
    }
#pragma unroll
    for (int i = 0; i < NA; ++i)
      lds_dma16((k0 + akc[i] < K) ? reinterpret_cast<const float*>(reinterpret_cast<const char*>(Abase + k0) + voffA[i]) : zero, sb + (unsigned)(i * 4096));
#pragma unroll
    for (int j = 0; j < NBW; ++j)
      if (j < NBW - 1 || nb_hi)
        lds_dma16((k0 + bkc[j] < K) ? reinterpret_cast<const float*>(Bbase + 2L * k0 + voffB[j]) : zero, sb + A_BYTES + (unsigned)(j * 4096));
  };
  f32x4 acc_hi[TM][TN], acc_lo[TM][TN];
#pragma unroll
  for (int m = 0; m < TM; ++m)
#pragma unroll
    for (int n = 0; n < TN; ++n) acc_hi[m][n] = acc_lo[m][n] = f32x4{0.f, 0.f, 0.f, 0.f};
#pragma unroll
  for (int s = 0; s < NS - 1; ++s)
    if (s < S) issue(s);
  for (int s = 0; s < S; ++s) {
    if (nb_hi) wait_stages<NA + NBW, NS - 2>(S - 1 - s);
    else wait_stages<NA + NBW - 1, NS - 2>(S - 1 - s);
    __builtin_amdgcn_s_barrier();
    if (s + NS - 1 < S) issue(s + NS - 1);
    const unsigned char* st = lds_raw + (s % NS) * STAGE_BYTES;
    const float* As = reinterpret_cast<const float*>(st);
    const __bf16* Bi = reinterpret_cast<const __bf16*>(st + A_BYTES);
    bf16x8_t bf[3][TN];
#pragma unroll
    for (int img = 0; img < 3; ++img)
#pragma unroll
      for (int n = 0; n < TN; ++n)
        bf[img][n] = *reinterpret_cast<const bf16x8_t*>(Bi + img * (BN * BK) + (n * 16 + r) * BK + ((q ^ bx3_swzB(r)) * 8));
#pragma unroll
    for (int m = 0; m < TM; ++m) {
      const float* arow = As + ((w * TM + m) * 16 + r) * BK;
      const f32x4 x0 = *reinterpret_cast<const f32x4*>(arow + 4 * ((2 * q) ^ bx3_swzA(r)));
      const f32x4 x1 = *reinterpret_cast<const f32x4*>(arow + 4 * ((2 * q + 1) ^ bx3_swzA(r)));
      bf16x8_t a1, a2, a3;
      split3_trunc8(x0, x1, a1, a2, a3);
#pragma unroll
      for (int n = 0; n < TN; ++n) {
        acc_hi[m][n] = __builtin_amdgcn_mfma_f32_16x16x32_bf16(a1, bf[0][n], acc_hi[m][n], 0, 0, 0);
        acc_lo[m][n] = __builtin_amdgcn_mfma_f32_16x16x32_bf16(a3, bf[0][n], acc_lo[m][n], 0, 0, 0);
        acc_lo[m][n] = __builtin_amdgcn_mfma_f32_16x16x32_bf16(a1, bf[2][n], acc_lo[m][n], 0, 0, 0);
        acc_lo[m][n] = __builtin_amdgcn_mfma_f32_16x16x32_bf16(a2, bf[1][n], acc_lo[m][n], 0, 0, 0);
        acc_lo[m][n] = __builtin_amdgcn_mfma_f32_16x16x32_bf16(a2, bf[0][n], acc_lo[m][n], 0, 0, 0);
        acc_lo[m][n] = __builtin_amdgcn_mfma_f32_16x16x32_bf16(a1, bf[1][n], acc_lo[m][n], 0, 0, 0);
      }
    }
  }
#pragma unroll
  for (int m = 0; m < TM; ++m)
#pragma unroll
    for (int n = 0; n < TN; ++n) acc_hi[m][n] += acc_lo[m][n];
  __syncthreads();
  gemm_epilogue<TM, TN>(g, acc_hi, reinterpret_cast<float*>(lds_raw), g.C, m0, n0, M, N, 0);
}

static bool bx3_ok(const nnr_gemm_args& g) {
  auto al = [](const void* p) { return ((uintptr_t)p & 15) == 0; };
  return pipe_ok(g) && !g.a_idx && g.batch <= 1 && g.B3 && al(g.B3) && (g.ldb3 & 7) == 0 && g.ldb3 >= g.K && ((g.b3_stride * 2) & 15) == 0;
}
template <int TM, int TN, int NS>
int launch_bx3(const nnr_gemm_args& g, hipStream_t s) {
  constexpr int BM = 64 * TM, BN = 16 * TN;
  const int nbm = (g.M + BM - 1) / BM, nbn = (g.N + BN - 1) / BN;
  hipLaunchKernelGGL((gemm_nt_bx3_kernel<TM, TN, NS>), dim3(nbm * nbn), dim3(256), 0, s, g);
  NNR_CHECK_LAUNCH();
  return NNR_OK;
}

__device__ __forceinline__ int tn_eff_slices(int split_k, int sched, int K, int nblk, int slots) {
  const int deal_mode = sched & 3;
  const int want_wg = ((sched >> 2) & 63) ? ((sched >> 2) & 63) * 64 : 512;
  const int slice_stages = (sched >> 8) ? (sched >> 8) : 96;
  const int ktiles = (K + 15) / 16;
  const int want = (want_wg + nblk - 1) / nblk;
  int eff = max(1, min(min(split_k, max(want, ktiles / slice_stages)), max(1, ktiles / 12)));
  if (deal_mode != 2) {
    const int W = eff * nblk, wv = W / slots;
    const int target = W < slots ? slots : (((W - wv * slots) * 2 < slots) ? wv * slots : (wv + 1) * slots);
    eff = max(1, min(target / nblk, min(split_k, max(1, ktiles / 12))));
  }
  return eff;
}

template <int TM, int TN, int NS, int OCC, int PRIO = 0>
__global__ __launch_bounds__(256, OCC) void gemm_tn_pipe_kernel(nnr_gemm_args g) {
  if (PRIO == 1) set_prio_dyn((blockIdx.x + gridDim.x * blockIdx.z) >> 8);
  constexpr int BK = 16, BM = 64 * TM, BN = 16 * TN;
  constexpr int PA = BM, PB = BN <= 64 ? 64 : (BN <= 128 ? 128 : 256);
  constexpr int RA = 256 / PA, RB = 256 / PB;
  constexpr int NIA = BK / RA, NIB = BK / RB, NI = NIA + NIB;
  constexpr int NPW = (NI + 3) / 4;
  constexpr int STAGE = BK * (PA + PB);
  constexpr int E_LD = BN + 4;
  constexpr int LDS_FLOATS = (NS * STAGE > 64 * E_LD) ? NS * STAGE : 64 * E_LD;
  static_assert(BN <= 256 && NI % 4 == 0, "tile shape");
  __shared__ __attribute__((aligned(1024))) float lds[LDS_FLOATS];

  const int tid = threadIdx.x, lane = tid & 63, w = __builtin_amdgcn_readfirstlane(tid >> 6);
  const int r = lane & 15, kk = lane >> 4;
  const int M = g.M, N = g.N;
  int K = g.K;
  if (g.dyn_dim == 2) K = min(K, *g.dyn_dev);
  const int nbm = (M + BM - 1) / BM, nbn = (N + BN - 1) / BN;
  const int nblk = nbm * nbn;
  int v, z = 0;
  int kbeg = 0, kend = K;
  if (g.split_k > 1) {
    const int deal_mode = g.sched & 3;
    const int ktiles = (K + BK - 1) / BK;
    const int eff = tn_eff_slices(g.split_k, g.sched, K, nblk, OCC * 256);
    if (deal_mode) {
      const int W = eff * nblk, per = (W + 7) >> 3;
      const int L = blockIdx.x, x = L & 7, slot = L >> 3;
      const int lin = x * per + slot;
      if (slot >= per || lin >= W) return;
      z = lin / nblk;
      v = lin - z * nblk;
    } else {
      z = blockIdx.x / nblk;
      v = blockIdx.x - z * nblk;
      if (z >= eff) return;
    }
    const int per_k = (ktiles + eff - 1) / eff;
    kbeg = z * per_k * BK;
    kend = min(K, kbeg + per_k * BK);
    if (kbeg >= kend) return;
  } else {
    const int b = blockIdx.x, q = nblk >> 3, rem = nblk & 7, x = b & 7, slot = b >> 3;
    v = x * q + min(x, rem) + slot;
  }
  const int bm = v / nbn, bn = v - bm * nbn;
  const int m0 = bm * BM, n0 = bn * BN;
  const float* __restrict__ A = g.A;
  const float* __restrict__ B = g.B;
  const int* __restrict__ bidx = g.b_idx;
  const float* zero = nnr_zero_page;
  asm volatile("" : "+s"(zero));

  long coloff[NPW];
  int krow[NPW];
#pragma unroll
  for (int i = 0; i < NPW; ++i) {
    const int q = w + 4 * i;
    if (q < NIA) {
      const int kl = q * RA + lane / (PA / 4), p4 = lane % (PA / 4);
      const int col = (4 * p4) ^ (16 * ((kl >> 2) & 1));
      krow[i] = kl;
      coloff[i] = (m0 + col < M) ? (long)(m0 + col) : -1;
    } else {
      const int kl = (q - NIA) * RB + lane / (PB / 4), p4 = lane % (PB / 4);
      const int col = (4 * p4) ^ (16 * ((kl >> 2) & 1));
      krow[i] = kl;
      coloff[i] = (col < BN && n0 + col < N) ? (long)(n0 + col) : -1;
    }
  }
  const unsigned lds_base = (unsigned)(uintptr_t)lds;
  const int S = (kend - kbeg + BK - 1) / BK;

  int bsrc[NPW][RB];
  auto fetch_idx = [&](int s) {
    if (bidx == nullptr) return;
    const int k0 = kbeg + s * BK;
#pragma unroll
    for (int i = 0; i < NPW; ++i) {
      const int q = w + 4 * i;
      if (q >= NIA) {
#pragma unroll
        for (int j = 0; j < RB; ++j) {
          const int k = min(k0 + (q - NIA) * RB + j, kend - 1);
          asm volatile("s_load_dword %0, %1, %2" : "=s"(bsrc[i][j]) : "s"(bidx), "s"(k * 4) : "memory");
        }
      }
    }
  };
  auto issue = [&](int s) {
    const int k0 = kbeg + s * BK;
    const unsigned sb = lds_base + (unsigned)((s % NS) * STAGE * 4);
#pragma unroll
    for (int i = 0; i < NPW; ++i) {
      const int q = w + 4 * i;
      const int k = k0 + krow[i];
      const float* src = zero;
      if (q < NIA) {
        if (coloff[i] >= 0 && k < kend) src = A + (long)k * g.lda + coloff[i];
        lds_dma16(src, sb + (unsigned)(q * 1024));
      } else {
        long row = k;
        if (bidx != nullptr) {
          int sel = bsrc[i][0];
#pragma unroll
          for (int j = 1; j < RB; ++j) sel = (lane / (PB / 4) == j) ? bsrc[i][j] : sel;
          row = sel;
        }
        if (coloff[i] >= 0 && k < kend && row >= 0) src = B + row * g.ldb + coloff[i];
        lds_dma16(src, sb + (unsigned)(NIA * 1024 + (q - NIA) * 1024));
      }
    }
  };

// ... 609 lines not shown
```

nnr_amd/csrc/tape.hip:

```cpp
#include <cstring>
#include <string>
#include <tuple>
#include <utility>
#include <vector>
#include "common.h"

namespace {

typedef int (*thunk_t)(const uint64_t* slots, hipStream_t stream);

template <typename T> inline T slot_as(const uint64_t* s) { T v; std::memcpy(&v, s, sizeof(T)); return v; }

template <auto Fn> struct Thunk;
template <typename... P, int (*Fn)(P...)> struct Thunk<Fn> {
  static constexpr int nargs = (int)sizeof...(P) - 1;
  template <size_t... I> static int apply(const uint64_t* s, hipStream_t st, std::index_sequence<I...>) {
    using Tup = std::tuple<P...>;
    static_assert(std::is_same<std::tuple_element_t<sizeof...(P) - 1, Tup>, hipStream_t>::value, "entry point must end with hipStream_t");
    return Fn(slot_as<std::tuple_element_t<I, Tup>>(s + I)..., st);
  }
  static int call(const uint64_t* s, hipStream_t st) { return apply(s, st, std::make_index_sequence<sizeof...(P) - 1>{}); }
};

struct Entry { const char* name; thunk_t thunk; int nargs; };
#define R(fn) { #fn, &Thunk<&fn>::call, Thunk<&fn>::nargs }
const Entry REGISTRY[] = {
  R(nnr_gemm_f32), R(nnr_seq_plan), R(nnr_seq_plan_pair), R(nnr_cne_pair_map), R(nnr_lstm_pack_weights), R(nnr_lstm_unpack_grads),
  R(nnr_lstm_fwd), R(nnr_lstm_bwd), R(nnr_attn_pool_fwd), R(nnr_attn_pool_bwd), R(nnr_gate_bwd), R(nnr_packed_seq_sum),
  R(nnr_tanh_score_bwd), R(nnr_colsum), R(nnr_rowdot), R(nnr_small_embed_fwd), R(nnr_small_embed_bwd), R(nnr_embed_gather),
  R(nnr_embed_scatter), R(nnr_embed_scatter_dyn), R(nnr_transpose2d), R(nnr_transpose_batch), R(nnr_add), R(nnr_add_atomic), R(nnr_add2d), R(nnr_expand_rows_fwd), R(nnr_expand_rows_bwd),
  R(nnr_dropout), R(nnr_relu_bwd), R(nnr_gcn_aggregate_fwd), R(nnr_gcn_aggregate_bwd), R(nnr_relu_drop_bwd), R(nnr_mhsa_fwd), R(nnr_mhsa_bwd),
  R(nnr_sue_x0_fwd), R(nnr_sue_x0_bwd), R(nnr_sue_slice_fwd), R(nnr_sue_slice_bwd), R(nnr_sue_intra_fwd), R(nnr_sue_intra_bwd),
  R(nnr_corpus_batch), R(nnr_history_graph), R(nnr_logits_loss_fwd), R(nnr_logits_fwd), R(nnr_nls_loss), R(nnr_logits_bwd),
  R(nnr_layernorm_fwd), R(nnr_layernorm_bwd), R(nnr_sumsq), R(nnr_sumsq_part), R(nnr_clip_adam), R(nnr_dp_allreduce), R(nnr_dp_broadcast), R(nnr_dp_busy), R(nnr_split_bf16x3), R(nnr_mhsa_fwd_packed), R(nnr_mhsa_bwd_packed), R(nnr_mhsa_pair_map), R(nnr_mhsa_fwd_paired), R(nnr_mhsa_bwd_paired), R(nnr_mask_cover), R(nnr_seq_rowmap),
  R(nnr_fill_zero), R(nnr_copy_bytes), R(nnr_fill_column_u8), R(nnr_fusion_rows_fwd), R(nnr_fusion_rows_bwd), R(nnr_click_loss), R(nnr_rank_metrics),
  R(nnr_token_sort), R(nnr_embed_scatter_sorted), R(nnr_fusion_rows_bwd_det),
  R(nnr_rows_touch), R(nnr_rows_compact), R(nnr_rows_pack), R(nnr_rows_unpack),
  R(nnr_cand_attn_fwd), R(nnr_cand_attn_bwd),
  R(nnr_omap_fwd), R(nnr_omap_bwd), R(nnr_omap_reg_fwd), R(nnr_omap_reg_bwd),
};
#undef R
constexpr int NREG = (int)(sizeof(REGISTRY) / sizeof(REGISTRY[0]));

enum { OP_CALL = 0, OP_RECORD = 1, OP_WAIT = 2 };
struct Op { int kind, a, b; };
struct Call { int fn, stream, nslots, tag; size_t slot_off; };
struct BlobRef { size_t slot; size_t blob_off; };
struct Patch { size_t byte_off; int kind; int width; int64_t addend; };
constexpr int MAX_TIMING_SETS = 64;

}

struct nnr_tape {
  std::vector<uint64_t> arena;
  std::vector<Call> calls;
  std::vector<Op> ops;
  std::vector<size_t> seg_begin;
  std::vector<hipStream_t> streams;
  std::vector<hipEvent_t> events;
  std::vector<uint64_t> event_keys;
  std::vector<BlobRef> blob_refs;
  std::vector<Patch> patches;
  std::vector<std::vector<hipEvent_t>> tset;
  int ntagged = 0;
  bool final = false;
  int last_rc = 0, last_failed_call = -1;
};

namespace {
int stream_index(nnr_tape* t, hipStream_t s) {
  for (size_t i = 0; i < t->streams.size(); ++i) if (t->streams[i] == s) return (int)i;
  t->streams.push_back(s);
  return (int)t->streams.size() - 1;
}
int new_event(nnr_tape* t, uint64_t key) {
  hipEvent_t e;
  if (hipEventCreateWithFlags(&e, hipEventDisableTiming) != hipSuccess) return -1;
  t->events.push_back(e);
  t->event_keys.push_back(key);
  return (int)t->events.size() - 1;
}
}

extern "C" int nnr_tape_create(nnr_tape** out) {
  if (!out) return NNR_ERR_ARG;
  *out = new nnr_tape();
  (*out)->seg_begin.push_back(0);
  return NNR_OK;
}

extern "C" int nnr_tape_destroy(nnr_tape* t) {
  if (!t) return NNR_OK;
  for (hipEvent_t e : t->events) (void)hipEventDestroy(e);
  for (auto& set : t->tset) for (hipEvent_t e : set) (void)hipEventDestroy(e);
  delete t;
  return NNR_OK;
}

extern "C" int nnr_tape_fn_id(const char* name) {
  for (int i = 0; i < NREG; ++i) if (std::strcmp(REGISTRY[i].name, name) == 0) return i;
  return -1;
}
extern "C" int nnr_tape_fn_nargs(int fn) { return (fn >= 0 && fn < NREG) ? REGISTRY[fn].nargs : -1; }

extern "C" int nnr_tape_call(nnr_tape* t, int fn, hipStream_t stream, const uint64_t* slots, int nslots, const int* blob_slot,
                             const void* const* blob_ptr, const size_t* blob_bytes, int nblobs, int tag, size_t* slot_off_out,
                             size_t* blob_off_out) {
  if (!t || t->final || fn < 0 || fn >= NREG || nslots != REGISTRY[fn].nargs || (nslots > 0 && !slots)) return NNR_ERR_ARG;
  if (nblobs < 0 || (nblobs > 0 && (!blob_slot || !blob_ptr || !blob_bytes))) return NNR_ERR_ARG;
  for (int i = 0; i < nblobs; ++i)
    if (blob_slot[i] < 0 || blob_slot[i] >= nslots || !blob_ptr[i]) return NNR_ERR_ARG;
  Call c;
  c.fn = fn; c.stream = stream_index(t, stream); c.nslots = nslots; c.tag = tag; c.slot_off = t->arena.size();
  t->arena.insert(t->arena.end(), slots, slots + nslots);
  for (int i = 0; i < nblobs; ++i) {
    const size_t units = (blob_bytes[i] + 7) / 8, off = t->arena.size();
    t->arena.resize(off + units, 0);
    std::memcpy(&t->arena[off], blob_ptr[i], blob_bytes[i]);
    t->blob_refs.push_back({c.slot_off + (size_t)blob_slot[i], off});
    if (blob_off_out) blob_off_out[i] = off * 8;
  }
  if (slot_off_out) *slot_off_out = c.slot_off * 8;
  if (tag >= 0) t->ntagged = tag + 1 > t->ntagged ? tag + 1 : t->ntagged;
  t->calls.push_back(c);
  t->ops.push_back({OP_CALL, (int)t->calls.size() - 1, 0});
  return (int)t->calls.size() - 1;
}

extern "C" int nnr_tape_wait_stream(nnr_tape* t, hipStream_t waiter, hipStream_t signaller) {
  if (!t || t->final) return NNR_ERR_ARG;
  if (waiter == signaller) return NNR_OK;
  const int e = new_event(t, 0);
  if (e < 0) return NNR_ERR_LAUNCH;
  t->ops.push_back({OP_RECORD, e, stream_index(t, signaller)});
  t->ops.push_back({OP_WAIT, stream_index(t, waiter), e});
  return NNR_OK;
}
extern "C" int nnr_tape_event_record(nnr_tape* t, uint64_t key, hipStream_t s) {
  if (!t || t->final || !key) return NNR_ERR_ARG;
  const int e = new_event(t, key);
  if (e < 0) return NNR_ERR_LAUNCH;
  t->ops.push_back({OP_RECORD, e, stream_index(t, s)});
  return NNR_OK;
}
extern "C" int nnr_tape_event_wait(nnr_tape* t, hipStream_t s, uint64_t key) {
  if (!t || t->final || !key) return NNR_ERR_ARG;
  for (int i = (int)t->events.size() - 1; i >= 0; --i)
    if (t->event_keys[i] == key) { t->ops.push_back({OP_WAIT, stream_index(t, s), i}); return NNR_OK; }
  return NNR_ERR_ARG;
}
extern "C" int nnr_tape_segment(nnr_tape* t) {
  if (!t || t->final) return NNR_ERR_ARG;
  t->seg_begin.push_back(t->ops.size());
  return (int)t->seg_begin.size() - 1;
}
extern "C" int nnr_tape_patch(nnr_tape* t, size_t byte_off, int kind, int width, int64_t addend) {
  if (!t || t->final || kind < 0 || (width != 4 && width != 8) || byte_off + (size_t)width > t->arena.size() * 8) return NNR_ERR_ARG;
  t->patches.push_back({byte_off, kind, width, addend});
  return NNR_OK;
}
extern "C" int nnr_tape_finalize(nnr_tape* t) {
  if (!t || t->final) return NNR_ERR_ARG;
  for (const BlobRef& r : t->blob_refs) t->arena[r.slot] = (uint64_t)(uintptr_t)&t->arena[r.blob_off];
  t->seg_begin.push_back(t->ops.size());
  t->final = true;
  return NNR_OK;
}
extern "C" int nnr_tape_info(const nnr_tape* t, int* calls, int* ops, int* segments, int* streams, size_t* arena_bytes) {
  if (!t) return NNR_ERR_ARG;
  if (calls) *calls = (int)t->calls.size();
  if (ops) *ops = (int)t->ops.size();
  if (segments) *segments = (int)t->seg_begin.size() - (t->final ? 1 : 0);
  if (streams) *streams = (int)t->streams.size();
  if (arena_bytes) *arena_bytes = t->arena.size() * 8;
  return NNR_OK;
}

extern "C" int nnr_tape_replay(nnr_tape* t, int segment, const uint64_t* values, int nvalues, const uint64_t* inputs, int ninputs,
                               int timing_set) {
  if (!t || !t->final || segment < 0 || segment + 1 >= (int)t->seg_begin.size()) return NNR_ERR_ARG;
  if (segment == 0) {
    uint8_t* base = reinterpret_cast<uint8_t*>(t->arena.data());
    for (const Patch& p : t->patches) {
      uint64_t v;
// ... 128 lines not shown
```

nnr_amd/ops.py:

```python
import ctypes as C
import math
import os
import weakref

import torch

from . import _lib as L
from . import profile as _prof
from . import tape as _tape

ACT_NONE, ACT_RELU, ACT_TANH, ACT_SIGMOID = 0, 1, 2, 3
K_CHUNK = 1024


class _NoSpan:
    def __enter__(self):
        return self

    def __exit__(self, *a):
        return False


_NOSPAN = _NoSpan()

# ... 232 lines not shown
    if e.stamp != stamp:
        fill()
        _refreshed([(e, stamp)], cur)
    elif e.stream != cur:
        torch.cuda.current_stream(e.bufs[0].device).wait_event(e.event)


def _stale(kind):
    jobs = []
    for (k, _), e in _DERIVED.items():
        src = e.ref() if k == kind and e.prefetch and e.served else None
        if src is not None and src.data_ptr() == e.ptr:
            stamp = _stamp((src,))
            if e.stamp != stamp:
                jobs.append((e, src, stamp))
    return jobs


def _on_leaf(dev, jobs, launch):
    leaf = leaf_stream(dev)
    leaf.wait_stream(torch.cuda.current_stream(dev))
    with torch.cuda.stream(leaf):
        launch()
        _refreshed([(e, stamp) for e, _, stamp in jobs], _s())
    for e, _, _ in jobs:
        e.served = False


def wt(w):
    rows, cols = w.shape
    e = _derived('wt', w, (rows, cols), lambda: torch.empty((cols, rows), device=w.device, dtype=torch.float32), isinstance(w, torch.nn.Parameter))
    _serve(e, (w,), lambda: transpose2d(w, e.out, rows, cols))
    return e.out


def wt_prefetch(dev):
    if torch.cuda.is_current_stream_capturing():
        return
    jobs = _stale('wt')
    if not jobs:
        return
    descs = tuple((w.data_ptr(), e.out.data_ptr(), w.shape[0], w.shape[1]) for e, w, _ in jobs)
    if _WT_DESCS[0] != descs:
        arr = (L.TransposeDesc * len(descs))()
        for d, (src, out, rows, cols) in zip(arr, descs):
            d.inp, d.out, d.rows, d.cols = src, out, rows, cols
        _WT_DESCS[:] = [descs, torch.frombuffer(bytearray(bytes(arr)), dtype=torch.uint8).to(dev)]
    table = _WT_DESCS[1]
    tape_keep(table, *[e.out for e, _, _ in jobs])
    _on_leaf(dev, jobs, lambda: L.check(L.lib().nnr_transpose_batch(_p(table), len(descs), _s()), 'nnr_transpose_batch'))


def _pack_entry(lstm, p, H, E):
    return _derived('lstm', lstm, (H, E), lambda: LstmPacked(p, H, E, fill=False), False)


def lstm_pack(lstm, H, E):
    p = lstm.param_list()
    e = _pack_entry(lstm, p, H, E)
    _serve(e, p, lambda: e.out.pack(p))
    return e.out


def lstm_prefetch(dev, lstms, H, E):
    jobs = []
    for lstm in lstms:
        p = lstm.param_list()
        e = _pack_entry(lstm, p, H, E)
        stamp = _stamp(p)
        if e.stamp != stamp:
            jobs.append((e, p, stamp))

    def launch():
        for e, p, _ in jobs:
            tape_keep(*e.bufs)
            e.out.pack(p)
    if jobs:
        _on_leaf(dev, jobs, launch)


def tn_tile(M, N, K, gather=False):
    if K >= 2048 and M >= 512 and N >= 512 and not gather and not ((M & 3) or (N & 3)):
        return 26, 128, 80, 2048
    if K < 8192 or (M & 3) or (N & 3) or (M >= 512 and N >= 512):
        return 0, 64, 80, 2048
    if not gather and M >= 1024 and 160 < N <= 320:
        return 30, 128, 160, 2048
    if N <= 208 or (N > 320 and N <= 416):
        if gather or M % 128 != 0:
            return 32, 64, 208, 640
        return 27, 128, 208, 640
    if gather:
        return 20, 128, 80, 2048
    return 26, 128, 80, 2048


def split_for(m, n, k, tile_m=64, tile_n=80, target_blocks=2048, kmin=256):
    tiles = max(1, ((m + tile_m - 1) // tile_m) * ((n + tile_n - 1) // tile_n))
    if k <= 640:
        return 1
    return int(max(1, min((k + kmin - 1) // kmin, (target_blocks + tiles - 1) // tiles)))


BX3 = [os.environ.get('NNR_BX3', '1') == '1']
_BX3_MIN_ROWS = 2048
_BX3_TILE = 50
_BX3_CLASSES = {'dx', 'sue', 'proj', 'gate'}


def bx3_class(N, K):
    if K >= 1024:
        return 'dx'
    if K >= 800:
        return 'sue'
    if N >= 1024:
        return 'proj'
    return 'gate'


BX3_SEEN = {}


def _split_bf16x3(B, N, K, ldb, img):
    ldo = img.shape[2]
    L.check(L.lib().nnr_split_bf16x3(_p(B), N, K, ldb, ldo, _p(img), N * ldo, _s()), 'nnr_split_bf16x3')


def bx3_prefetch(dev):
    if not BX3[0] or torch.cuda.is_current_stream_capturing():
        return
    jobs = _stale('bx3')

    def launch():
        for e, B, _ in jobs:
            tape_keep(e.out, B)
            _split_bf16x3(B, *e.spec, e.out)
    if jobs:
        _on_leaf(dev, jobs, launch)


def bx3_images(B, N, K, ldb):
    ldo = (K + 7) // 8 * 8
    owner = _OWNED.get(id(B))
    e = _derived('bx3', B, (N, K, ldb), lambda: torch.empty((3, N, ldo), device=B.device, dtype=torch.int16),
                 isinstance(B, torch.nn.Parameter) or (owner is not None and owner.prefetch))
    _serve(e, (B,), lambda: _split_bf16x3(B, N, K, ldb, e.out))
    return e.out, N * ldo, ldo


def _bx3_wanted(A, B, M, N, K, lda, ldb, trans_a, trans_b, a_idx, b_idx, c_idx, split_k, k_chunk, rowdot_w, colsum_out, atomic, batch, dyn_dim, drop):
    return (not trans_a and not trans_b and a_idx is None and b_idx is None and split_k <= 1 and k_chunk <= 0 and rowdot_w is None
            and colsum_out is None and batch <= 1 and dyn_dim in (0, 1) and M >= _BX3_MIN_ROWS and K >= 64 and N * K <= (1 << 22)
            and (K | lda | ldb) & 3 == 0 and (A.data_ptr() | B.data_ptr()) & 15 == 0 and (drop is None or drop[0] in (3, 4) or drop[1] <= 0.0))


def gemm(A, B, C_=None, *, M, N, K, lda, ldb, ldc=0, trans_a=False, trans_b=False, dyn=None, dyn_dim=0, a_idx=None, b_idx=None,
         drop=None, alpha=1.0, bias=None, rowvec=None, ldrv=0, rowvec_map=None, act=0, aux_out=None, ldaux=0, mul=None, ldmul=0,
         resid=None, ldres=0, accumulate=False, atomic=False, c_idx=None, split_k=1, rowdot_w=None, rowdot_out=None, batch=1,
         strideA=0, strideB=0, strideC=0, stride_aux=0, stride_res=0, tile=0, colsum_out=None, k_chunk=0, flop_scale=1.0, slab=None,
         pre_add=None, ldpre=0, gate_bwd=False, b3=None):
    g = L.GemmArgs()
    g.A, g.B = A.data_ptr(), B.data_ptr()
    if C_ is not None:
        g.C = C_.data_ptr()
    g.M, g.N, g.K, g.lda, g.ldb, g.ldc, g.alpha = M, N, K, lda, ldb, ldc, alpha
    if trans_a:
        g.trans_a = 1
    if trans_b:
        g.trans_b = 1
    if dyn is not None:
        g.dyn_dev, g.dyn_dim = dyn.data_ptr(), dyn_dim
    if a_idx is not None:
        g.a_idx = a_idx.data_ptr()
    if b_idx is not None:
        g.b_idx = b_idx.data_ptr()
    if drop is not None and drop[1] > 0.0:
        g.drop_target, g.drop_p, g.drop_seed, g.drop_cols = drop[0], float(drop[1]), int(drop[2]), int(drop[3])
    if bias is not None:
        g.bias = bias.data_ptr()
    if rowvec is not None:
        g.rowvec, g.ldrv, g.rowvec_map = rowvec.data_ptr(), ldrv, _p(rowvec_map)
    if act:
        g.act = act
    if aux_out is not None:
        g.aux_out, g.ldaux = aux_out.data_ptr(), ldaux
    if mul is not None:
        g.mul, g.ldmul = mul.data_ptr(), ldmul
    if resid is not None:
        g.resid, g.ldres = resid.data_ptr(), ldres
    if accumulate:
        g.accumulate = int(accumulate)
    if atomic:
        g.atomic = 1
    if c_idx is not None:
        g.c_idx = c_idx.data_ptr()
    g.split_k, g.batch = int(split_k), batch
    if rowdot_w is not None:
        g.rowdot_w, g.rowdot_out = rowdot_w.data_ptr(), rowdot_out.data_ptr()
    if batch > 1:
        g.strideA, g.strideB, g.strideC, g.stride_aux, g.stride_res = strideA, strideB, strideC, stride_aux, stride_res
    if tile:
        g.tile = tile
    if colsum_out is not None:
        g.colsum_out = colsum_out.data_ptr()
    if k_chunk:
        g.k_chunk = int(k_chunk)
    if pre_add is not None:
        g.pre_add, g.ldpre = pre_add.data_ptr(), ldpre
    if gate_bwd:
        g.gate_bwd = 1
    if b3 is None and BX3[0] and tile in (0, 9, 15, 16) and _bx3_wanted(A, B, M, N, K, lda, ldb, trans_a, trans_b, a_idx, b_idx, c_idx, split_k, k_chunk, rowdot_w,
                                                                    colsum_out, atomic, batch, dyn_dim, drop):
        is_w = is_weight(B)
        key = (M, N, K, 'weight' if is_w else 'other')
        BX3_SEEN[key] = BX3_SEEN.get(key, 0) + 1
        if is_w and bx3_class(N, K) in _BX3_CLASSES:
            b3 = bx3_images(B, N, K, ldb)
            tile = _BX3_TILE
            g.tile = _BX3_TILE
    if b3 is not None:
        g.B3, g.b3_stride, g.ldb3 = b3[0].data_ptr(), b3[1], b3[2]
    if slab is None and TN_SLAB and trans_a and trans_b and split_k > 1 and not k_chunk and c_idx is None and (N & 3) == 0 and C_ is not None:
        slab = _slab_ws(A.device, int(split_k) * (M * N + M))
    if slab is not None:
        g.slab, g.slab_floats = slab.data_ptr(), slab.numel()
    if not (A.is_cuda and B.is_cuda):
        raise L.NnrHipError('nnr_amd ops need device tensors (no CPU fallback on the product path)')
    if not _prof.active():
        L.check(L.lib().nnr_gemm_f32(C.byref(g), _s()), 'nnr_gemm_f32')
        return
    pipe_nt = (not trans_a and not trans_b and b_idx is None and split_k <= 1 and k_chunk <= 0 and rowdot_w is None and colsum_out is None
               and (drop is None or drop[0] in (3, 4) or drop[1] <= 0.0) and (K | lda | ldb) & 3 == 0 and (A.data_ptr() | B.data_ptr()) & 15 == 0)
    wg128 = ((M + 127) // 128) * ((N + 79) // 80) * (split_k if split_k > 1 else max(1, batch)) * (1 if k_chunk <= 0 else max(1, K // k_chunk))
    wg64 = ((M + 63) // 64) * ((N + 79) // 80) * (split_k if split_k > 1 else max(1, batch))
    if tile:
        t = tile
    elif rowdot_w is not None:
        t = 3
    elif (not trans_a and a_idx is None and b_idx is None and c_idx is None and dyn is None and split_k <= 1 and k_chunk <= 0
          and colsum_out is None and not atomic and wg64 <= 512 and K >= 64 and drop is None):
        t = 7
    elif pipe_nt and a_idx is None and K >= 800 and wg64 > 512:
        t = 9
    elif pipe_nt and (dyn is not None or wg128 >= 640):
        t = 15
    elif pipe_nt and wg64 > 512 and K >= 128:
        t = 16
    elif wg64 <= 512 and dyn is None and k_chunk <= 0 and K >= 128:
        t = 6
    elif M <= 512 or (wg128 < 640 and dyn is None) or trans_a:
        t = 2
    else:
        t = 5 if not trans_b else 4
    fam = 'gemm_%s_%s' % ('tn' if trans_a else ('nn' if trans_b else 'nt'),
                          {2: '64x80', 3: '128x208', 4: '128x80', 5: '128x80k32', 6: '64x80k64', 7: '16x80skinny', 9: 'pipe2_128x80', 15: 'pipe128x80', 16: 'pipe128x80s2',
                           20: 'pipe128x80', 26: 'pipe2_128x80', 27: 'pipe2_128x208', 30: 'pipe2_128x160', 32: 'pipe2_64x208', 50: 'bx3_128x80', 51: 'bx3_64x80'}.get(t, 'tile%d' % t))

    def flops(vals=None, M=M, N=N, K=K, dyn=dyn, dyn_dim=dyn_dim, batch=batch):
        m, k = M, K
        if dyn is not None:
            d = int(vals[dyn.data_ptr()]) if vals is not None else int(dyn.item())
            m, k = (min(M, d), K) if dyn_dim == 1 else (M, min(K, d))
        return 2.0 * m * N * k * max(1, batch) * flop_scale
    flops.dyn = [dyn] if dyn is not None else []
    flops.scale = flop_scale

    def op_bytes(vals=None, M=M, N=N, K=K, dyn=dyn, dyn_dim=dyn_dim, batch=batch):
        m, k = M, K
        if dyn is not None:
            d = int(vals[dyn.data_ptr()]) if vals is not None else int(dyn.item())
            m, k = (min(M, d), K) if dyn_dim == 1 else (M, min(K, d))
        outs = (1 if C_ is not None else 0) + (1 if accumulate else 0) + (1 if aux_out is not None else 0) + (1 if mul is not None else 0) + (1 if resid is not None else 0) + (1 if pre_add is not None else 0)
        return 4.0 * max(1, batch) * (m * k + N * k + m * N * outs)
    flops.bytes_fn = op_bytes
    if trans_a and trans_b and split_k > 1:
        flops.tn_dims = (M, N, flop_scale)
    flops.tag = 'M%d N%d K%d%s%s%s' % (M, N, K, ' b%d' % batch if batch > 1 else '', (' sk%d' % split_k if split_k > 1 else '') + (' kc%d' % k_chunk if k_chunk > 0 else ''), ' dyn' if dyn is not None else '')
    with _prof.span(fam, flops):
        L.check(L.lib().nnr_gemm_f32(C.byref(g), _s()), 'nnr_gemm_f32')


def linear_fwd(x, w, bias=None, out=None, act=0, **kw):
    M, K = x.shape
    N = w.shape[0]
    if out is None:
        out = torch.empty((M, N), device=x.device, dtype=torch.float32)
    gemm(x, w, out, M=M, N=N, K=K, lda=x.stride(0), ldb=w.stride(0), ldc=out.stride(0), bias=bias, act=act, **kw)
    return out


def linear_bwd_data(dy, w, out=None, accumulate=False, **kw):
    M, N = dy.shape
    K = w.shape[1]
    if out is None:
        out = torch.empty((M, K), device=dy.device, dtype=torch.float32)
    if M >= 1024 and w.is_contiguous() and (N & 3) == 0:
        gemm(dy, wt(w), out, M=M, N=K, K=N, lda=dy.stride(0), ldb=N, ldc=out.stride(0), accumulate=accumulate, **kw)
    else:
        gemm(dy, w, out, M=M, N=K, K=N, lda=dy.stride(0), ldb=w.stride(0), ldc=out.stride(0), trans_b=True, accumulate=accumulate, **kw)
    return out


def linear_bwd_weight(dy, x, dw, dyn=None, rows=None, db=None, small_lds=False, **kw):
    R = dy.shape[0] if rows is None else rows
    N, K = dw.shape
    t, bm, bn, target = tn_tile(N, K, R)
    if small_lds:
        t, bm, bn, target = 2, 64, 80, 2048
    if t and ((dy.stride(0) | x.stride(0)) & 3 or (dy.data_ptr() | x.data_ptr()) & 15):
        t, bm, bn, target = 0, 64, 80, 2048
    gemm(dy, x, dw, M=N, N=K, K=R, lda=dy.stride(0), ldb=x.stride(0), ldc=dw.stride(0), trans_a=True, trans_b=True,
         atomic=True, dyn=dyn, dyn_dim=2, colsum_out=db, split_k=split_for(N, K, R, bm, bn, target), tile=t, **kw)


def rowdot(x, w, out, dyn=None, rows=None):
    R = x.shape[0] if rows is None else rows
    L.check(L.lib().nnr_rowdot(_p(x), x.stride(0), _p(w), _p(dyn), R, x.shape[1], _p(out), _s()), 'nnr_rowdot')


_SLOT_WS = {}
_SLAB_WS = {}
TN_SLAB = True
def _slab_ws(dev, floats):
    key = torch._C._cuda_getCurrentRawStream(dev.index if dev.index is not None else torch.cuda.current_device())
    ws = _SLAB_WS.get(key)
    if ws is None or ws.numel() < floats:
        ws = torch.empty(max(int(floats), 1 << 22), device=dev, dtype=torch.float32)
        _SLAB_WS[key] = ws
    tape_keep(ws)
    return ws



def _slot_ws(dev, n):
    key = torch._C._cuda_getCurrentRawStream(dev.index if dev.index is not None else torch.cuda.current_device())
    need = L.lib().nnr_slot_workspace_floats(n)
    ws = _SLOT_WS.get(key)
    if ws is None or ws.numel() < need:
        ws = torch.zeros(max(need, 32 * 1024), device=dev, dtype=torch.float32)
        _SLOT_WS[key] = ws
    tape_keep(ws)
    return ws


def bias_grad(dy, db, dyn=None, rows=None):
    R = dy.shape[0] if rows is None else rows
    ws = _slot_ws(dy.device, db.numel())
    L.check(L.lib().nnr_colsum(_p(dy), dy.stride(0), _p(dyn), R, db.numel(), _p(db), _p(ws), _s()), 'nnr_colsum')


class SeqPlan:

    def __init__(self, mask, ids, perm=None, mask1=None, ids1=None):
        n0, Lx = mask.shape
        n = n0 + (mask1.shape[0] if mask1 is not None else 0)
        dev = mask.device
        self.n, self.L, self.n0 = n, Lx, n0
        i32 = dict(device=dev, dtype=torch.int32)
        self.len = torch.empty(n, **i32)
        self.order = torch.empty(n, **i32)
        self.rank = torch.empty(n, **i32)
        self.slen = torch.empty(n, **i32)
        self.bs = torch.empty(Lx, **i32)
        self.off = torch.empty(Lx + 1, **i32)
        self.row_seq = torch.empty(n * Lx, **i32)
        self.tok = torch.empty(n * Lx, **i32) if ids is not None else None
        self.prev_f = torch.empty(n * Lx, **i32)
        self.prev_r = torch.empty(n * Lx, **i32)
        self.total = self.off[Lx:]
        self.cap = n * Lx
        m8 = mask.view(torch.uint8) if mask.dtype == torch.bool else mask
        assert m8.is_contiguous() and (ids is None or (ids.is_contiguous() and ids.dtype == torch.int32))
# ... 124 lines not shown
    arr = _lstm_probs(items, H)
    with _prof.span('lstm_fwd', _lstm_flops(items, H)):
        L.check(L.lib().nnr_lstm_fwd(arr, len(items), H, _s()), 'nnr_lstm_fwd')


def lstm_bwd(items, H):
    arr = _lstm_probs(items, H, backward=True)
    with _prof.span('lstm_bwd', _lstm_flops(items, H)):
        L.check(L.lib().nnr_lstm_bwd(arr, len(items), H, _s()), 'nnr_lstm_bwd')


def _pool_args(x, ldx, D, n, Lx, plan=None, mask=None, mask_div=1, score=None, v=None, ldv=0, scale=1.0, alpha=None, out=None,
               ldo=0, add_in=None, ldadd=0, dout=None, lddo=0, dout2=None, lddo2=0, dx=None, lddx=0, dx_accumulate=False,
               dscore=None, dv=None, lddv=0, th=None, w2=None, alpha_b=None, dout_b=None, lddo_b=0, dscore_b=None, v_b=None, ldv_b=0, scale_b=1.0):
    a = L.PoolArgs()
    a.x, a.ldx, a.D, a.n, a.L = _p(x), ldx, D, n, Lx
    a.packed = int(plan is not None)
    if plan is not None:
        a.off, a.slen, a.order = _p(plan.off), _p(plan.slen), _p(plan.order)
    if mask is not None:
        a.mask = _p(mask.view(torch.uint8) if mask.dtype == torch.bool else mask)
    a.mask_div = mask_div
    a.score, a.v, a.ldv, a.scale, a.alpha = _p(score), _p(v), ldv, float(scale), _p(alpha)
    a.out, a.ldo, a.add_in, a.ldadd = _p(out), ldo, _p(add_in), ldadd
    a.dout, a.lddo, a.dout2, a.lddo2 = _p(dout), lddo, _p(dout2), lddo2
    a.dx, a.lddx, a.dx_accumulate, a.dscore, a.dv, a.lddv = _p(dx), lddx, int(dx_accumulate), _p(dscore), _p(dv), lddv
    if th is not None:
        a.th, a.ldth, a.A, a.w2 = _p(th), th.stride(0), th.shape[1], _p(w2)
    if alpha_b is not None:
        a.alpha_b, a.dout_b, a.lddo_b, a.dscore_b, a.v_b, a.ldv_b, a.scale_b = _p(alpha_b), _p(dout_b), lddo_b, _p(dscore_b), _p(v_b), ldv_b, float(scale_b)
    return a


def _pool_span(family, kw, per_token_arrays):
    if not _prof.active():
        return _NOSPAN
    plan, D, n, Lx = kw.get('plan'), kw['D'], kw['n'], kw['Lx']
    th = kw.get('th')
    per_row = 4.0 * (D * per_token_arrays + (th.shape[1] if th is not None else 0) + 2)
    return _hbm_span(family, per_row, n * Lx, dyn=plan.total if plan is not None else None, fixed=4.0 * n * D * 3)


def pool_fwd(**kw):
    with _pool_span('pool_fwd', kw, 1):
        L.check(L.lib().nnr_attn_pool_fwd(C.byref(_pool_args(**kw)), _s()), 'nnr_attn_pool_fwd')


def pool_bwd(**kw):
    with _pool_span('pool_bwd', kw, (3 if kw.get('dx_accumulate') else 2) if kw.get('dx') is not None else 1):
        L.check(L.lib().nnr_attn_pool_bwd(C.byref(_pool_args(**kw)), _s()), 'nnr_attn_pool_bwd')


def add_(y, x, alpha=1.0):
    assert y.is_contiguous() and x.is_contiguous() and y.numel() == x.numel()
    L.check(L.lib().nnr_add(_p(y), _p(x), y.numel(), alpha, _s()), 'nnr_add')
    return y


def add_atomic_(y, x, alpha=1.0):
    assert y.is_contiguous() and x.is_contiguous() and y.numel() == x.numel()
    L.check(L.lib().nnr_add_atomic(_p(y), _p(x), y.numel(), alpha, _s()), 'nnr_add_atomic')
    return y


def expand_rows(x, N):
    B, D = x.shape
    y = torch.empty((B, N, D), device=x.device, dtype=torch.float32)
    L.check(L.lib().nnr_expand_rows_fwd(_p(x), _p(y), B, N, D, _s()), 'nnr_expand_rows_fwd')
    return y


def expand_rows_bwd(dy):
    B, N, D = dy.shape
    dx = torch.empty((B, D), device=dy.device, dtype=torch.float32)
    L.check(L.lib().nnr_expand_rows_bwd(_p(dy), _p(dx), B, N, D, _s()), 'nnr_expand_rows_bwd')
    return dx


def add2d(y, ldy, x, ldx, rows, cols, alpha=1.0, accumulate=False):
    L.check(L.lib().nnr_add2d(_p(y), ldy, _p(x), ldx, rows, cols, alpha, accumulate, _s()), 'nnr_add2d')


def gate_bwd(dHt, H, G, dH, dpre, plan, cols):
    with _hbm_span('gate_bwd', 5 * 4.0 * cols, plan.cap, dyn=plan.total):
        return _gate_bwd(dHt, H, G, dH, dpre, plan, cols)


def _gate_bwd(dHt, H, G, dH, dpre, plan, cols):
    L.check(L.lib().nnr_gate_bwd(_p(dHt), _p(H), _p(G), _p(dH), _p(dpre), _p(plan.total), plan.cap, cols, _s()), 'nnr_gate_bwd')


def packed_seq_sum(x, D, plan, out):
    L.check(L.lib().nnr_packed_seq_sum(_p(x), D, _p(plan.off), _p(plan.slen), plan.n, _p(out), _s()), 'nnr_packed_seq_sum')


def tanh_score_bwd(th, ds, w2, dw2, plan, A):
    rows = plan.cap if plan is not None else th.shape[0]
    ws = _slot_ws(th.device, A)
    L.check(L.lib().nnr_tanh_score_bwd(_p(th), _p(ds), _p(w2), _p(dw2), _p(plan.total) if plan is not None else None, rows, A, _p(ws),
                                       _s()), 'nnr_tanh_score_bwd')


def small_embed_fwd(table, idx, out_view, ldo, p, seed):
    n, dim = idx.numel(), table.shape[1]
    L.check(L.lib().nnr_small_embed_fwd(_p(table), _p(idx), n, dim, _p(out_view), ldo, p, seed, _s()), 'nnr_small_embed_fwd')


def small_embed_bwd(idx, dim, dout_view, lddo, dtable, p, seed):
    L.check(L.lib().nnr_small_embed_bwd(_p(idx), idx.numel(), dim, _p(dout_view), lddo, _p(dtable), p, seed, _s()), 'nnr_small_embed_bwd')


def dropout(x, p, seed, out=None):
    if out is None:
        out = torch.empty_like(x)
    L.check(L.lib().nnr_dropout(_p(x), _p(out), x.numel(), p, seed, _s()), 'nnr_dropout')
    return out


def layernorm_fwd(u, gamma, beta, eps, xhat, rstd, r_out, resid, y, p, seed):
    rows, D = u.numel() // u.shape[-1], u.shape[-1]
    L.check(L.lib().nnr_layernorm_fwd(_p(u), _p(gamma), _p(beta), eps, rows, D, _p(xhat), _p(rstd), _p(r_out), _p(resid), _p(y), p, seed, _s()),
                                      'nnr_layernorm_fwd')


def layernorm_bwd(dv, xhat, rstd, gamma, du, dgamma, dbeta):
    rows, D = dv.numel() // dv.shape[-1], dv.shape[-1]
    L.check(L.lib().nnr_layernorm_bwd(_p(dv), _p(xhat), _p(rstd), _p(gamma), rows, D, _p(du), _p(dgamma), _p(dbeta), _s()), 'nnr_layernorm_bwd')


def relu_bwd(dy, y, dx=None):
    if dx is None:
        dx = torch.empty_like(dy)
    L.check(L.lib().nnr_relu_bwd(_p(dy), _p(y), _p(dx), dy.numel(), _s()), 'nnr_relu_bwd')
    return dx


def relu_drop_bwd(dy, r, ds, dx, p, seed):
    L.check(L.lib().nnr_relu_drop_bwd(_p(dy), _p(r), _p(ds), _p(dx), dy.numel(), p, seed, _s()), 'nnr_relu_drop_bwd')


def gcn_aggregate_fwd(graph, z, bias, resid, r_out, y, B, G, D, relu, p, seed):
    arrays = 3 + (1 if resid is not None else 0)
    with _hbm_span('gcn_aggregate_fwd', 4.0 * (G * D * arrays + G * G), B):
        L.check(L.lib().nnr_gcn_aggregate_fwd(_p(graph), _p(z), _p(bias), _p(resid), _p(r_out), _p(y), B, G, D, relu, p, seed, _s()),
                                              'nnr_gcn_aggregate_fwd')


def gcn_aggregate_bwd(graph, dy, r, ds, dx0, dz, B, G, D, p, seed):
    arrays = 4 + (1 if dx0 is not None else 0)
    with _hbm_span('gcn_aggregate_bwd', 4.0 * (G * D * arrays + G * G), B):
        L.check(L.lib().nnr_gcn_aggregate_bwd(_p(graph), _p(dy), _p(r), _p(ds), _p(dx0), _p(dz), B, G, D, p, seed, _s()), 'nnr_gcn_aggregate_bwd')


def sue_x0_fwd(hist, proxy, x0, B, Hn, Kc, D, p, seed, cmask_fix=None):
    if cmask_fix is not None:
        assert cmask_fix.is_contiguous() and cmask_fix.element_size() == 1 and tuple(cmask_fix.shape) == (B, Kc + 1)
    L.check(L.lib().nnr_sue_x0_fwd(_p(hist), _p(proxy), _p(x0), B, Hn, Kc, D, p, seed, _p(cmask_fix), _s()), 'nnr_sue_x0_fwd')


def sue_x0_bwd(dx0, dhist, dproxy, B, Hn, Kc, D, p, seed, dx0_add=None):
    L.check(L.lib().nnr_sue_x0_bwd(_p(dx0), _p(dx0_add), _p(dhist), _p(dproxy), B, Hn, Kc, D, p, seed, _s()), 'nnr_sue_x0_bwd')


def sue_slice_fwd(gcn, x0, gfeat, B, Hn, G, D):
    L.check(L.lib().nnr_sue_slice_fwd(_p(gcn), _p(x0), _p(gfeat), B, Hn, G, D, _s()), 'nnr_sue_slice_fwd')


def sue_slice_bwd(dgfeat, dpad, B, Hn, G, D):
    L.check(L.lib().nnr_sue_slice_bwd(_p(dgfeat), _p(dpad), B, Hn, G, D, _s()), 'nnr_sue_slice_bwd')


def sue_intra_fwd(kf, qc, g, cidx, B, N, Hn, Cn, A, D, alpha, feat):
    with _hbm_span('sue_intra_fwd', 4.0 * (Hn * A + N * A + Hn * D + N * Hn + N * Cn * D) + 8.0 * Hn, B):
        return _sue_intra_fwd(kf, qc, g, cidx, B, N, Hn, Cn, A, D, alpha, feat)


def _sue_intra_fwd(kf, qc, g, cidx, B, N, Hn, Cn, A, D, alpha, feat):
    L.check(L.lib().nnr_sue_intra_fwd(_p(kf), _p(qc), _p(g), _p(cidx), B, N, Hn, Cn, A, D, _p(alpha), _p(feat), _s()), 'nnr_sue_intra_fwd')


def sue_intra_bwd(kf, qc, g, cidx, alpha, dfeat, B, N, Hn, Cn, A, D, dg, dkf, dqc):
    ws = torch.empty(B * N * Hn, device=kf.device, dtype=torch.float32)
    with _hbm_span('sue_intra_bwd', 4.0 * (N * Cn * D + 2 * Hn * D + 2 * Hn * A + 2 * N * A + N * Hn) + 8.0 * Hn, B):
        return _sue_intra_bwd(kf, qc, g, cidx, alpha, dfeat, B, N, Hn, Cn, A, D, dg, dkf, dqc, ws)


def _sue_intra_bwd(kf, qc, g, cidx, alpha, dfeat, B, N, Hn, Cn, A, D, dg, dkf, dqc, ws):
    L.check(L.lib().nnr_sue_intra_bwd(_p(kf), _p(qc), _p(g), _p(cidx), _p(alpha), _p(dfeat), B, N, Hn, Cn, A, D, _p(dg), _p(dkf), _p(dqc),
                                      _p(ws), _s()), 'nnr_sue_intra_bwd')


def _u8(mask):
    return None if mask is None else (mask.view(torch.uint8) if mask.dtype == torch.bool else mask)


def cand_attn_fwd(P, Q, w2, feat, mask, B, N, H, A, D, act, alpha, out):
    with _hbm_span('cand_attn_fwd', 4.0 * (N * A + H * A + H * D + N * H + N * D) + 1.0 * H, B, fixed=4.0 * A):
        L.check(L.lib().nnr_cand_attn_fwd(_p(P), _p(Q), _p(w2), _p(feat), feat.stride(1), _p(_u8(mask)), B, N, H, A, D, act, _p(alpha), _p(out),
                                          _s()), 'nnr_cand_attn_fwd')


def cand_attn_bwd(P, Q, w2, feat, mask, alpha, dout, B, N, H, A, D, act, dP, dQ, dfeat, dw2, accumulate=False):
    ws = torch.empty(L.lib().nnr_cand_attn_ws_floats(B, N, H, A), device=P.device, dtype=torch.float32)
    with _hbm_span('cand_attn_bwd', 4.0 * (2 * N * A + 2 * H * A + (3 if accumulate else 2) * H * D + 3 * N * H + N * D + 2 * N * A) + 1.0 * H, B,
                   fixed=8.0 * A):
        L.check(L.lib().nnr_cand_attn_bwd(_p(P), _p(Q), _p(w2), _p(feat), feat.stride(1), _p(_u8(mask)), _p(alpha), _p(dout), B, N, H, A, D, act,
                                          _p(dP), _p(dQ), _p(dfeat), accumulate, _p(ws), _p(dw2), _s()), 'nnr_cand_attn_bwd')


def omap_ws(B, N, H, D, K, device):
    n = L.lib().nnr_omap_ws_floats(B, N, H, D, K)
    if n < 0:
        raise L.NnrHipError('nnr_omap_ws_floats failed with code %d (B %d, N %d, H %d, D %d, K %d)' % (n, B, N, H, D, K))
    return torch.empty(n, device=device, dtype=torch.float32)


def omap_fwd(hist, cand, mask, W, B, N, H, D, K, alpha, Y, beta, R, gamma, out):
    ws = omap_ws(B, N, H, D, K, hist.device)
    with _hbm_span('omap_fwd', 4.0 * (2 * H * D + 2 * H * H + 2 * H * D + N * D + 2 * K * D + N * D + 2 * H * K + N * K) + 1.0 * H, B,
                   fixed=4.0 * D * K):
        L.check(L.lib().nnr_omap_fwd(_p(hist), hist.stride(1), _p(cand), _p(_u8(mask)), _p(W), B, N, H, D, K, _p(alpha), _p(Y), _p(beta), _p(R),
                                     _p(gamma), _p(out), _p(ws), _s()), 'nnr_omap_fwd')


def omap_bwd(hist, cand, mask, W, alpha, Y, beta, R, gamma, dout, B, N, H, D, K, dhist, dcand, dW, accumulate=False):
    ws = omap_ws(B, N, H, D, K, hist.device)
    with _hbm_span('omap_bwd', 4.0 * (2 * H * D + 2 * H * D + 2 * H * H + 2 * H * H + 2 * N * D + K * D + 3 * K * D + N * D +
                                      (2 if accumulate else 1) * H * D + 2 * D * K + 3 * H * K) + 1.0 * H, B, fixed=12.0 * D * K):
        L.check(L.lib().nnr_omap_bwd(_p(hist), hist.stride(1), _p(cand), _p(_u8(mask)), _p(W), _p(alpha), _p(Y), _p(beta), _p(R), _p(gamma), _p(dout),
                                     B, N, H, D, K, _p(dhist), accumulate, _p(dcand), _p(dW), _p(ws), _s()), 'nnr_omap_bwd')


def omap_reg_fwd(W, coef, off, loss):
    D, K = W.shape
    L.check(L.lib().nnr_omap_reg_fwd(_p(W), D, K, coef, _p(off), _p(loss), _s()), 'nnr_omap_reg_fwd')


def omap_reg_bwd(W, off, gup, coef, dW):
    D, K = W.shape
    L.check(L.lib().nnr_omap_reg_bwd(_p(W), _p(off), _p(gup), D, K, coef, _p(dW), _s()), 'nnr_omap_reg_bwd')


def logits_loss_fwd(user, cand, B, N, D, logits, loss, dlogits):
    L.check(L.lib().nnr_logits_loss_fwd(_p(user), _p(cand), B, N, D, _p(logits), _p(loss), _p(dlogits), _s()), 'nnr_logits_loss_fwd')


def logits_fwd(user, cand, B, N, D, logits):
    L.check(L.lib().nnr_logits_fwd(_p(user), _p(cand), B, N, D, _p(logits), _s()), 'nnr_logits_fwd')


def nls_loss(logits, B, N, loss, dlogits):
    L.check(L.lib().nnr_nls_loss(_p(logits), B, N, _p(loss), _p(dlogits), _s()), 'nnr_nls_loss')


def logits_bwd(dlogits, user, cand, B, N, D, duser, dcand, accumulate=False):
    L.check(L.lib().nnr_logits_bwd(_p(dlogits), _p(user), _p(cand), B, N, D, _p(duser), _p(dcand), accumulate, _s()), 'nnr_logits_bwd')


def sumsq(g, out):
    with _hbm_span('sumsq', 4.0, g.numel()):
        return _sumsq(g, out)


def _sumsq(g, out):
    L.check(L.lib().nnr_sumsq(_p(g), g.numel(), _p(out), _s()), 'nnr_sumsq')


def sumsq_part(g, out, add_in=None, slot=0):
    with _hbm_span('sumsq', 4.0, g.numel()):
        L.check(L.lib().nnr_sumsq_part(_p(g), g.numel(), _p(out), _p(add_in), slot, _s()), 'nnr_sumsq_part')


def fusion_rows_fwd(cat_table, sub_table, cat0, sub0, cat1, sub1, out_view, ldo, p, seed_cat, seed_sub):
    n0, n1 = cat0.numel(), (cat1.numel() if cat1 is not None else 0)
    L.check(L.lib().nnr_fusion_rows_fwd(_p(cat_table), _p(sub_table), _p(cat0), _p(sub0), n0, _p(cat1), _p(sub1), n1, cat_table.shape[1],
                                        sub_table.shape[1], _p(out_view), ldo, p, seed_cat, seed_sub, _s()), 'nnr_fusion_rows_fwd')


def fusion_rows_bwd(cat0, sub0, cat1, sub1, cd, sd, dout_view, lddo, dcat_table, dsub_table, p, seed_cat, seed_sub):
    n0, n1 = cat0.numel(), (cat1.numel() if cat1 is not None else 0)
    if cd <= 128 and sd <= 128:
        L.check(L.lib().nnr_fusion_rows_bwd_det(_p(cat0), _p(sub0), n0, _p(cat1), _p(sub1), n1, cd, sd, dcat_table.shape[0], dsub_table.shape[0],
                                                _p(dout_view), lddo, _p(dcat_table), _p(dsub_table), p, seed_cat, seed_sub, _s()),
                                                'nnr_fusion_rows_bwd_det')
        return
    L.check(L.lib().nnr_fusion_rows_bwd(_p(cat0), _p(sub0), n0, _p(cat1), _p(sub1), n1, cd, sd, _p(dout_view), lddo, _p(dcat_table), _p(dsub_table),
                                        p, seed_cat, seed_sub, _s()), 'nnr_fusion_rows_bwd')


def click_loss(user, cand, B, N, D, logits, loss, dlogits, duser, dcand, terms_ws):
    L.check(L.lib().nnr_click_loss(_p(user), _p(cand), B, N, D, _p(logits), _p(loss), _p(dlogits), _p(duser), _p(dcand), _p(terms_ws), _s()),
            'nnr_click_loss')


def clip_adam(p, g, m, v, sumsq_buf, grad_scale, clip, lr, beta1, beta2, eps, wd, step):
    with _hbm_span('clip_adam', 7 * 4.0, p.numel()):
        return _clip_adam(p, g, m, v, sumsq_buf, grad_scale, clip, lr, beta1, beta2, eps, wd, step)


def _clip_adam(p, g, m, v, sumsq_buf, grad_scale, clip, lr, beta1, beta2, eps, wd, step):
    L.check(L.lib().nnr_clip_adam(_p(p), _p(g), _p(m), _p(v), p.numel(), _p(sumsq_buf), grad_scale, clip, lr, beta1, beta2, eps, wd, step, _s()),
                                  'nnr_clip_adam')


def mhsa_fwd(qkv, mask, n, Lq, heads, dh, out, prob, p=0.0, seed=0):
    if mask is not None and mask.dtype == torch.bool:
# ... 189 lines not shown
```

nnr_amd/profile.py:

```python
import os

import torch

_on = False
_records = []

KERNEL_OF = {
    'gemm_nt_256x80': 'gemm_kernel<4, 5, false, false, 16>', 'gemm_nn_256x80': 'gemm_kernel<4, 5, false, true, 16>',
    'gemm_tn_256x80': 'gemm_kernel<4, 5, true, true, 16>', 'gemm_nt_64x80': 'gemm_kernel<1, 5, false, false, 16>',
    'gemm_nn_64x80': 'gemm_kernel<1, 5, false, true, 16>', 'gemm_tn_64x80': 'gemm_kernel<1, 5, true, true, 16>',
    'gemm_nt_128x208': 'gemm_kernel<2, 13, false, false, 16>', 'gemm_nt_128x80': 'gemm_kernel<2, 5, false, false, 16>', 'gemm_nt_128x80k32': 'gemm_kernel<2, 5, false, false, 32>',
    'gemm_nt_64x80k64': 'gemm_kernel<1, 5, false, false, 64>', 'gemm_nn_64x80k64': 'gemm_kernel<1, 5, false, true, 64>',
    'gemm_tn_64x80k64': 'gemm_kernel<1, 5, true, true, 64>',
    'gemm_nt_pipe128x80': 'gemm_nt_pipe_kernel<2, 5, 16, 3, 4, 0>', 'gemm_nt_pipe128x80s2': 'gemm_nt_pipe_kernel<2, 5, 16, 2, 5, 0>',
    'gemm_nt_bx3_128x80': 'gemm_nt_bx3_kernel<2, 5, 2>', 'gemm_nt_bx3_64x80': 'gemm_nt_bx3_kernel<1, 5, 2>',
    'gemm_nt_pipe2_128x80': 'gemm_nt_pipe2_kernel<2, 5, 3, 2>', 'gemm_nt_pipe2_128x64': 'gemm_nt_pipe2_kernel<2, 4, 3, 2>',
    'gemm_tn_pipe2_128x80': 'gemm_tn_pipe2_kernel<2, 5, 3, 3>', 'gemm_tn_pipe2_128x208': 'gemm_tn_pipe2_kernel<2, 13, 3, 2>', 'gemm_tn_pipe2_128x160': 'gemm_tn_pipe2_kernel<2, 10, 3, 2>', 'gemm_tn_pipe2_64x208': 'gemm_tn_pipe2_kernel<1, 13, 3, 2>',
    'gemm_tn_pipe128x80': 'gemm_tn_pipe_kernel<2, 5, 3, 3, 0>', 'gemm_tn_pipe128x208': 'gemm_tn_pipe_kernel<2, 13, 3, 2, 0>',
    'gemm_nn_128x80': 'gemm_kernel<2, 5, false, true, 16>', 'gemm_tn_128x80': 'gemm_kernel<2, 5, true, true, 16>', 'lstm_fwd': 'lstm_fwd_pair_kernel<13>', 'lstm_bwd': 'lstm_bwd_pair_kernel<13, true>',
}


_enabled, _every = False, 1
TAPE_HOOK = [None]
TAPE_RECORDS = []


_eager = True


def enable(every=1, eager=True):
    global _on, _enabled, _every, _eager
    _enabled, _every, _eager = True, max(1, int(every)), bool(eager)
    _on = _eager
    _records.clear()
    TAPE_RECORDS.clear()


def begin_step(i):
    global _on
    inst = _enabled and (i % _every == 0)
    _on = inst and _eager
    return inst


def disable():
    global _on, _enabled
    _on = _enabled = False


def active():
    return _on or TAPE_HOOK[0] is not None


class span:

    def __init__(self, family, flops_fn):
        self.family, self.flops_fn = family, flops_fn

    def __enter__(self):
        if TAPE_HOOK[0] is not None:
            TAPE_HOOK[0](self.family, self.flops_fn)
        if _on:
            self.s = torch.cuda.Event(enable_timing=True)
            self.e = torch.cuda.Event(enable_timing=True)
            self.s.record()
        return self

    def __exit__(self, *a):
        if _on:
            self.e.record()
            _records.append((self.family, self.s, self.e, self.flops_fn))
        return False


def by_shape():
    out = {}
    for family, fn, ms in _all_records():
        tag = getattr(fn, 'tag', '')
        d = out.setdefault((family, tag), dict(ms=0.0, flops=0.0, launches=0))
        d['ms'] += ms
        d['flops'] += float(fn())
        d['launches'] += 1
    return out


def _all_records():
    torch.cuda.synchronize()
    for family, s, e, fn in _records:
        yield family, fn, s.elapsed_time(e)
    for family, fn, ms in TAPE_RECORDS:
        yield family, fn, ms


def _bytes_of(fn):
    if hasattr(fn, 'op_bytes'):
        return float(fn.op_bytes)
    if hasattr(fn, 'bytes_fn'):
        return float(fn.bytes_fn())
    return None


def summary(hbm=False):
    fam = {}
    for family, fn, ms in _all_records():
        if bool(getattr(fn, 'hbm', False)) != bool(hbm):
            continue
        d = fam.setdefault(family, dict(ms=0.0, flops=0.0, launches=0, bytes=0.0, executed=0.0))
        d['ms'] += ms
        f = float(fn())
        d['flops'] += f
        d['executed'] += f / float(getattr(fn, 'scale', 1.0) or 1.0)
        d['launches'] += 1
        if hbm:
            d['bytes'] += _bytes_of(fn) or 0.0
    return fam


HBM_KERNELS = {
    'embed_gather': (('embed_gather_kernel',), 1), 'embed_scatter': (('embed_scatter_kernel', 'embed_scatter_sorted_kernel'), 1),
    'pool_fwd': (('pool_kernel<false', 'pool_packed_kernel<false'), 1), 'pool_bwd': (('pool_kernel<true', 'pool_packed_kernel<true'), 1), 'gate_bwd': (('gate_bwd_kernel',), 1),
    'gcn_aggregate_fwd': (('gcn_aggregate_kernel<0',), 1), 'gcn_aggregate_bwd': (('gcn_aggregate_kernel<1',), 1),
    'sue_intra_fwd': (('sue_intra_fwd_kernel',), 1), 'sue_intra_bwd': (('sue_intra_bwd_ds_kernel', 'sue_intra_bwd_dg_kernel'), 2),
    'clip_adam': (('adam_kernel',), 1), 'sumsq': (('sumsq_kernel',), 1),
}
HBM_KERNELS_OTHER = {
    'cand_attn_fwd': (('cand_attn_fwd_kernel',), 1), 'cand_attn_bwd': (('cand_attn_bwd_da_kernel', 'cand_attn_bwd_dx_kernel'), 2),
    'omap_fwd': (('omap_alpha_kernel', 'omap_mix_kernel', 'omap_pool_kernel'), 3),
    'omap_bwd': (('omap_bwd_pool_kernel', 'omap_bwd_dalpha_kernel', 'omap_bwd_dx_kernel', 'omap_dw_reduce_kernel'), 4),
}
PEAK_HBM_GBS = 8000.0


def pmc_traffic_family(family):
    d = _pmc_file()
    spec = HBM_KERNELS.get(family) or HBM_KERNELS_OTHER.get(family)
    if d is None or spec is None:
        return None
    names, per_call = spec
    tot = launches = 0.0
    for k in d.get('kernels', []):
        if any(k['kernel'].startswith(n) for n in names):
            tot += k['hbm_bytes_per_launch'] * k['launches']
            launches += k['launches']
    return round(tot / (launches / per_call)) if launches else None


def mfma_busy(kernel_prefix):
    import json
    import os
    from . import _lib
    path = os.path.join(os.path.dirname(os.path.dirname(os.path.abspath(__file__))), 'profiles', 'pmc_mfma_busy.json')
    try:
        d = json.load(open(path))
    except (OSError, ValueError):
        return None
    have, now = d.get('build_id') or {}, _lib.build_id()
    if not (have.get('src_sha256') == now['src_sha256'] or (have.get('lib_sha256') and have.get('lib_sha256') == now['lib_sha256'])):
        return None
    hits = [k for k in d.get('kernels', []) if k['kernel'].startswith(kernel_prefix)]
    if not hits:
        return None
    busy = sum(k['mfma_busy_cycles_per_launch'] * k['launches'] for k in hits)
    active = sum(k['gui_active_per_launch'] * k['launches'] for k in hits)
    return {'kernel': ' + '.join(k['kernel'] for k in hits), 'launches': sum(k['launches'] for k in hits),
            'mfma_busy': round(busy / (active / 8.0 * 1024.0), 4) if active else None}


# ... 167 lines not shown
```

nnr_amd/user_encoders.py:

```python
import math

import torch
import torch.nn as nn

from . import ops
from .layers import Attention, ScaledDotProduct_CandidateAttention, MultiHeadAttention, GCN, grad_of, _CandAttnFn
from .news_encoders import NewsEncoder


class UserEncoder(nn.Module):

    def __init__(self, news_encoder: NewsEncoder, config):
        super().__init__()
        self.news_embedding_dim = news_encoder.news_embedding_dim
        self.news_encoder = news_encoder
        self.auxiliary_loss = None
        self._seed_base = int(getattr(config, 'seed', 0)) * 104723 + 29
        self._calls = 0

    def _next_seed(self):
        self._calls += 1
        return (self._seed_base + 15485863 * self._calls) & 0x7FFFFFFF

    def forward(self, user_title_text, user_title_mask, user_title_entity, user_content_text, user_content_mask, user_content_entity,
                user_category, user_subCategory, user_history_mask, user_history_graph, user_history_category_mask,
                user_history_category_indices, user_embedding, candidate_news_representation):
        raise Exception('Function forward must be implemented at sub-class')


class _SUEFunction(torch.autograd.Function):
    @staticmethod
    def forward(ctx, hist, cand, mod, graph, cmask, cidx):
        out, saved = sue_forward(mod, hist.contiguous(), cand.contiguous(), graph, cmask, cidx)
        ctx.mod, ctx.saved = mod, saved
        return out

    @staticmethod
    def backward(ctx, dout):
        dhist, dcand = sue_backward(ctx.mod, ctx.saved, dout.contiguous())
        ctx.saved = None
        return dhist, dcand, None, None, None, None


_SIDE = {}
ops.STREAM_CACHES.append(_SIDE)


def _sue_side(dev):
    if ops.ONE_STREAM[0]:
        return None
    key = (dev.type, dev.index)
    if key not in _SIDE:
        _SIDE[key] = ops.new_stream(dev)
    return _SIDE[key]


def gcn_forward(gcn, x0, graph, seed0, training):
    B, G, D = x0.shape
    f32 = dict(device=x0.device, dtype=torch.float32)
    Lg = gcn.num_layers
    xs, rs, lns = [x0], [], []
    x = x0
    for l, layer in enumerate(gcn.gcn_layers):
        y = torch.empty((B, G, D), **f32)
        r = torch.empty((B, G, D), **f32)
        pl = (gcn.dropout_rate if training else 0.0) if l + 1 < Lg else 0.0
        z = ops.linear_fwd(x.view(B * G, D), layer.W.weight)
        if getattr(layer, 'layer_norm', False):
            u = torch.empty((B, G, D), **f32)
            ops.gemm(graph, z, u, M=G, N=D, K=G, lda=G, ldb=D, ldc=D, trans_b=True, bias=layer.W.bias, batch=B, strideA=G * G, strideB=G * D,
                     strideC=G * D, tile=2)
            xhat = torch.empty((B, G, D), **f32)
            rstd = torch.empty(B * G, **f32)
            ln = layer.layer_normalization
            ops.layernorm_fwd(u, ln.weight, ln.bias, ln.eps, xhat, rstd, r, x if gcn.residual else None, y, pl, seed0 + l)
            lns.append((xhat, rstd))
        elif G <= 128 and D % 4 == 0:
            ops.gcn_aggregate_fwd(graph, z, layer.W.bias, x if gcn.residual else None, r, y, B, G, D, True, pl, seed0 + l)
            lns.append(None)
        else:
            ops.gemm(graph, z, y, M=G, N=D, K=G, lda=G, ldb=D, ldc=D, trans_b=True, bias=layer.W.bias, act=ops.ACT_RELU, aux_out=r,
                     ldaux=D, resid=x if gcn.residual else None, ldres=D, drop=(3, pl, seed0 + l, D), batch=B, strideA=G * G,
                     strideB=G * D, strideC=G * D, stride_aux=G * D, stride_res=G * D, tile=2)
            lns.append(None)
        xs.append(y)
        rs.append(r)
        x = y
    return x, dict(xs=xs, rs=rs, lns=lns, seed0=seed0, training=training)


def gcn_backward(gcn, gsv, dy, graph, leaf):
    B, G, D = dy.shape
    f32 = dict(device=dy.device, dtype=torch.float32)
    Lg = gcn.num_layers
    for l in range(Lg - 1, -1, -1):
        layer = gcn.gcn_layers[l]
        pl = (gcn.dropout_rate if gsv['training'] else 0.0) if l + 1 < Lg else 0.0
        dS = torch.empty((B, G, D), **f32)
        dx = torch.empty((B, G, D), **f32)
        if G <= 128 and D % 4 == 0 and gsv['lns'][l] is None:
            dz = torch.empty((B, G, D), **f32)
            ops.gcn_aggregate_bwd(graph, dy, gsv['rs'][l], dS, dx if gcn.residual else None, dz, B, G, D, pl, gsv['seed0'] + l)
            ops.linear_bwd_data(dz.view(B * G, D), layer.W.weight, out=dx.view(B * G, D), accumulate=bool(gcn.residual))
            leaf(lambda dS=dS, dz=dz, l=l, layer=layer: (ops.bias_grad(dS.view(B * G, D), grad_of(layer.W.bias)),
                                                         ops.linear_bwd_weight(dz.view(B * G, D), gsv['xs'][l].view(B * G, D), grad_of(layer.W.weight))), dS, dz)
            dy = dx
            continue
        ops.relu_drop_bwd(dy, gsv['rs'][l], dS, dx, pl, gsv['seed0'] + l)
        if not gcn.residual:
            ops.fill_zero(dx)
        if gsv['lns'][l] is not None:
            xhat, rstd = gsv['lns'][l]
            ln = layer.layer_normalization
            du = torch.empty((B, G, D), **f32)
            ops.layernorm_bwd(dS, xhat, rstd, ln.weight, du, grad_of(ln.weight), grad_of(ln.bias))
            dS = du
        dz = torch.empty((B, G, D), **f32)
        ops.gemm(graph, dS, dz, M=G, N=D, K=G, lda=G, ldb=D, ldc=D, trans_a=True, trans_b=True, batch=B, strideA=G * G, strideB=G * D,
                 strideC=G * D, tile=2)
        ops.linear_bwd_data(dz.view(B * G, D), layer.W.weight, out=dx.view(B * G, D), accumulate=True)
        leaf(lambda dS=dS, dz=dz, l=l, layer=layer: (ops.bias_grad(dS.view(B * G, D), grad_of(layer.W.bias)),
                                                     ops.linear_bwd_weight(dz.view(B * G, D), gsv['xs'][l].view(B * G, D), grad_of(layer.W.weight))), dS, dz)
        dy = dx
    return dy


class _GCNFunction(torch.autograd.Function):

    @staticmethod
    def forward(ctx, feature, gcn, graph):
        seed = (getattr(gcn, '_calls', 0) * 7919 + 101) & 0x7FFFFFFF
        gcn.__dict__['_calls'] = getattr(gcn, '_calls', 0) + 1
        out, gsv = gcn_forward(gcn, feature.contiguous(), graph.contiguous(), seed, gcn.training)
        ctx.gcn, ctx.gsv, ctx.graph = gcn, gsv, graph.contiguous()
        return out

    @staticmethod
    def backward(ctx, dy):
        with ops.leaf_scope(dy.device, enable=False) as leaf:
            dx = gcn_backward(ctx.gcn, ctx.gsv, dy.contiguous(), ctx.graph, leaf)
        ctx.gsv = None
        return dx, None, None


CAPTURE = [None]


def sue_forward(mod, hist, cand, graph, cmask, cidx):
    B, Hn, D = hist.shape
    N = cand.shape[1]
    Kc = mod.proxy_node_embedding.shape[0]
    G, Cn, A = Hn + Kc, Kc + 1, mod.attention_dim
    dev = hist.device
    f32 = dict(device=dev, dtype=torch.float32)
    p = mod.dropout_rate if mod.training else 0.0
    seed = mod._next_seed()
    sv = dict(B=B, Hn=Hn, D=D, N=N, Kc=Kc, G=G, Cn=Cn, A=A, p=p, seed=seed, hist=hist, cand=cand, cidx=cidx, cmask=cmask,
              graph=graph)
    x0 = torch.empty((B, G, D), **f32)
    cand2 = cand.view(B * N, D)
    ia = mod.interClusterAttention
    qc = torch.empty((B * N, A), **f32)
    qv = torch.empty((B * N, A), **f32)
    v = torch.empty((B * N, D), **f32)

    def cand_side():
        ops.linear_fwd(cand2, mod.intraCluster_Q.weight, mod.intraCluster_Q.bias, out=qc)
        ops.linear_fwd(cand2, ia.Q.weight, ia.Q.bias, out=qv)
        ops.gemm(qv, ia.K.weight, v, M=B * N, N=D, K=A, lda=A, ldb=D, ldc=D, trans_b=True)
    side = _sue_side(dev)
    side_ev = None
    if side is not None:
        side.wait_stream(torch.cuda.current_stream(dev))
        with torch.cuda.stream(side):
            cand_side()
            side_ev = torch.cuda.Event()
            side_ev.record()
    fix = cmask if (cmask.is_cuda and cmask.dim() == 2 and cmask.is_contiguous() and tuple(cmask.shape) == (B, Kc + 1)) else None
    if fix is None:
        if cmask.is_cuda and cmask.dim() == 2 and cmask.is_contiguous() and cmask.element_size() == 1:
            ops.fill_column_u8(cmask, -1, 1)
        else:
            cmask[:, -1] = 1
    ops.sue_x0_fwd(hist, mod.proxy_node_embedding, x0, B, Hn, Kc, D, p, seed + 1, cmask_fix=fix)
    x, gsv = gcn_forward(mod.gcn, x0, graph, seed + 10, mod.training)
    sv['gcn'] = gsv
    gfeat = torch.empty((B, Hn, D), **f32)
    ops.sue_slice_fwd(x, x0, gfeat, B, Hn, G, D)
    kf = ops.linear_fwd(gfeat.view(B * Hn, D), mod.intraCluster_K.weight)
    if side is None:
        cand_side()
    else:
        torch.cuda.current_stream(dev).wait_event(side_ev)
    alpha_i = torch.empty((B, N, Hn), **f32)
    feat = torch.empty((B * N * Cn, D), **f32)
    ops.sue_intra_fwd(kf, qc, gfeat, cidx, B, N, Hn, Cn, A, D, alpha_i, feat)
    rc = torch.empty((B * N * Cn, D), **f32)
    f2 = torch.empty((B * N * Cn, D), **f32)
    ops.gemm(feat, mod.clusterFeatureAffine.weight, f2, M=B * N * Cn, N=D, K=D, lda=D, ldb=D, ldc=D, bias=mod.clusterFeatureAffine.bias,
             act=ops.ACT_RELU, aux_out=rc, ldaux=D, resid=feat, ldres=D, drop=(3, p, seed + 2, D))
    alpha_o = torch.empty(B * N * Cn, **f32)
    out = torch.empty((B * N, D), **f32)
    ops.pool_fwd(x=f2, ldx=D, D=D, n=B * N, Lx=Cn, mask=cmask, mask_div=N, v=v, ldv=D, scale=1.0 / math.sqrt(A), alpha=alpha_o, out=out,
                 ldo=D)
    sv.update(gfeat=gfeat, kf=kf, qc=qc, alpha_i=alpha_i, feat=feat, rc=rc, f2=f2, qv=qv, v=v, alpha_o=alpha_o)
    if CAPTURE[0] is not None:
        CAPTURE[0].append(sv)
    return out.view(B, N, D), sv


def sue_backward(mod, sv, dout, dhist_out=None, dcand_accum=None):
    B, Hn, D, N, Kc, G, Cn, A, p, seed = (sv[k] for k in ('B', 'Hn', 'D', 'N', 'Kc', 'G', 'Cn', 'A', 'p', 'seed'))
    dev = dout.device
    f32 = dict(device=dev, dtype=torch.float32)
    cand2 = sv['cand'].view(B * N, D)
    dout = dout.view(B * N, D)
    ia = mod.interClusterAttention
    hook = mod.__dict__.get('_grads_ready_hook')
    exchange = getattr(hook, '__self__', None)
    need_now = (exchange is not None and exchange.active()) or not ops._DEFER.get('step_joins')
    with ops.leaf_scope(dev, defer_join=not need_now) as leaf:
        res = _sue_backward_body(mod, sv, dout, leaf, B, Hn, D, N, Kc, G, Cn, A, p, seed, dev, f32, cand2, ia, dhist_out, dcand_accum)
    if hook is not None:
        hook()
    return res


def _sue_backward_body(mod, sv, dout, leaf, B, Hn, D, N, Kc, G, Cn, A, p, seed, dev, f32, cand2, ia, dhist_out=None, dcand_accum=None):
    df2 = torch.empty((B * N * Cn, D), **f32)
    dv = torch.empty((B * N, D), **f32)
    ops.pool_bwd(x=sv['f2'], ldx=D, D=D, n=B * N, Lx=Cn, mask=sv['cmask'], mask_div=N, v=sv['v'], ldv=D, scale=1.0 / math.sqrt(A),
                 alpha=sv['alpha_o'], dout=dout, lddo=D, dx=df2, lddx=D, dv=dv, lddv=D)
    dqv = torch.empty((B * N, A), **f32)
    dcand = dcand_accum if dcand_accum is not None else torch.empty((B * N, D), **f32)
    main = torch.cuda.current_stream(dev)
    side = _sue_side(dev)

    def on_side(fn):
        if side is None:
            return fn()
        side.wait_stream(main)
        with torch.cuda.stream(side):
            return fn()

    def inter_q():
        ops.gemm(dv, ia.K.weight, dqv, M=B * N, N=A, K=D, lda=D, ldb=D, ldc=A)
        leaf(lambda: (ops.linear_bwd_weight(sv['qv'], dv, grad_of(ia.K.weight)),
                      ops.linear_bwd_weight(dqv, cand2, grad_of(ia.Q.weight), db=grad_of(ia.Q.bias))), dv, dqv)
        ops.linear_bwd_data(dqv, ia.Q.weight, out=dcand, accumulate=dcand_accum is not None)
    on_side(inter_q)
    dS = torch.empty((B * N * Cn, D), **f32)
    dfeat = torch.empty((B * N * Cn, D), **f32)
    ops.relu_drop_bwd(df2, sv['rc'], dS, dfeat, p, seed + 2)
    ops.linear_bwd_data(dS, mod.clusterFeatureAffine.weight, out=dfeat, accumulate=True)
    dS_aff = dS
    leaf(lambda: ops.linear_bwd_weight(dS_aff, sv['feat'], grad_of(mod.clusterFeatureAffine.weight), db=grad_of(mod.clusterFeatureAffine.bias)), dS_aff)
    dg = torch.empty((B, Hn, D), **f32)
    dkf = torch.empty((B * Hn, A), **f32)
    dqc = torch.empty((B * N, A), **f32)
    ops.sue_intra_bwd(sv['kf'], sv['qc'], sv['gfeat'], sv['cidx'], sv['alpha_i'], dfeat, B, N, Hn, Cn, A, D, dg, dkf, dqc)
# ... 228 lines not shown
```

Before: 6727.

## Fuse GCN layer linear GEMM with graph aggregation in one bx3 kernel

Adds a fused GCN layer kernel that runs the dense weight GEMM with split-bf16x3 MFMA and async LDS DMA, then does the per-graph aggregation, bias, residual, ReLU and dropout from the same LDS tile. The backward pass chains the data-gradient GEMM of layer l with the aggregate backward of layer l-1 in one launch. This removes the z intermediate round trip through global memory and cuts kernel launches per layer. In exchange it applies only for G in 65..80 with weight shapes that qualify for bx3, and the bx3 path approximates f32 with three bf16 pieces.

```diff
diff --git a/include/nnr_hip.h b/include/nnr_hip.h
--- a/include/nnr_hip.h
+++ b/include/nnr_hip.h
@@ -166,6 +166,10 @@
                           int D, int relu, float p, uint32_t seed, hipStream_t stream);
 int nnr_gcn_aggregate_bwd(const float* graph, const float* dy, const float* r, float* ds, float* dx0, float* dz, int B, int G, int D, float p,
                           uint32_t seed, hipStream_t stream);
+int nnr_gcn_layer_fwd(const float* graph, const float* x, const void* w3, long w3_stride, int ldw3, const float* bias, const float* resid,
+                      float* r_out, float* y, int B, int G, int D, int relu, float p, uint32_t seed, hipStream_t stream);
+int nnr_gcn_layer_bwd(const float* graph, const float* dz_in, const void* wt3, long wt3_stride, int ldwt3, const float* pre_add, const float* r,
+                      float* ds, float* dx0, float* dz, int B, int G, int D, float p, uint32_t seed, hipStream_t stream);
 int nnr_relu_drop_bwd(const float* dy, const float* r, float* ds, float* dx, long n, float p, uint32_t seed, hipStream_t stream);
 
 int nnr_mhsa_fwd(const float* qkv, const uint8_t* mask, int n, int Lq, int heads, int dh, float scale, float* out, float* prob,
diff --git a/nnr_amd/_lib.py b/nnr_amd/_lib.py
--- a/nnr_amd/_lib.py
+++ b/nnr_amd/_lib.py
@@ -94,6 +94,8 @@
     'nnr_relu_bwd': 'i32 ptr ptr ptr i64 stream',
     'nnr_gcn_aggregate_fwd': 'i32 ptr ptr ptr ptr ptr ptr i32 i32 i32 i32 f32 seed stream',
     'nnr_gcn_aggregate_bwd': 'i32 ptr ptr ptr ptr ptr ptr i32 i32 i32 f32 seed stream',
+    'nnr_gcn_layer_fwd': 'i32 ptr ptr ptr i64 i32 ptr ptr ptr ptr i32 i32 i32 i32 f32 seed stream',
+    'nnr_gcn_layer_bwd': 'i32 ptr ptr ptr i64 i32 ptr ptr ptr ptr ptr i32 i32 i32 f32 seed stream',
     'nnr_relu_drop_bwd': 'i32 ptr ptr ptr ptr i64 f32 seed stream',
     'nnr_mhsa_fwd': 'i32 ptr ptr i32 i32 i32 i32 f32 ptr ptr f32 seed stream',
     'nnr_mhsa_bwd': 'i32 ptr ptr ptr ptr i32 i32 i32 i32 f32 ptr f32 seed stream',
diff --git a/nnr_amd/csrc/bx3_loop.h b/nnr_amd/csrc/bx3_loop.h
--- /dev/null
+++ b/nnr_amd/csrc/bx3_loop.h
@@ -0,0 +1,98 @@
+#pragma once
+#include "common.h"
+
+static __device__ __attribute__((aligned(1024))) float nnr_zero_page[512] = {};
+
+__device__ __forceinline__ void lds_dma16(const float* gsrc, unsigned lds_dst) {
+  unsigned keep;
+  asm volatile("s_mov_b32 %0, m0\n\ts_mov_b32 m0, %2\n\ts_nop 0\n\tglobal_load_lds_dwordx4 %1, off\n\ts_mov_b32 m0, %0"
+               : "=&s"(keep) : "v"(gsrc), "s"(lds_dst) : "memory");
+}
+
+template <int N>
+__device__ __forceinline__ void wait_vmcnt() { asm volatile("s_waitcnt vmcnt(%0)" ::"n"(N) : "memory"); }
+template <int CNT, int MAXA>
+__device__ __forceinline__ void wait_stages(int ahead) {
+  if constexpr (MAXA == 0) wait_vmcnt<0>();
+  else {
+    if (ahead >= MAXA) wait_vmcnt<CNT * MAXA>();
+    else wait_stages<CNT, MAXA - 1>(ahead);
+  }
+}
+
+template <int N, int STEP = 0x1000>
+__device__ __forceinline__ void lds_dma16_block(const float* sbase, unsigned lds_dst, const unsigned (&voff)[8]) {
+  unsigned keep;
+  static_assert(N >= 1 && N <= 8, "1..8 loads per block");
+#define NNR_DMA_HEAD "s_mov_b32 %[keep], m0\n\ts_mov_b32 m0, %[dst]\n\t"
+#define NNR_DMA_LD(I) "s_nop 0\n\tglobal_load_lds_dwordx4 %[v" #I "], %[sb]\n\ts_add_u32 m0, m0, %[step]\n\t"
+#define NNR_DMA_TAIL "s_mov_b32 m0, %[keep]"
+#define NNR_DMA_OPS : [keep] "=&s"(keep) : [dst] "s"(lds_dst), [sb] "s"(sbase), [v0] "v"(voff[0]), [v1] "v"(voff[1]), [v2] "v"(voff[2]), [v3] "v"(voff[3]), \
+                      [v4] "v"(voff[4]), [v5] "v"(voff[5]), [v6] "v"(voff[6]), [v7] "v"(voff[7]), [step] "n"(STEP) : "memory", "scc"
+  if constexpr (N == 1) asm volatile(NNR_DMA_HEAD NNR_DMA_LD(0) NNR_DMA_TAIL NNR_DMA_OPS);
+  if constexpr (N == 2) asm volatile(NNR_DMA_HEAD NNR_DMA_LD(0) NNR_DMA_LD(1) NNR_DMA_TAIL NNR_DMA_OPS);
+  if constexpr (N == 3) asm volatile(NNR_DMA_HEAD NNR_DMA_LD(0) NNR_DMA_LD(1) NNR_DMA_LD(2) NNR_DMA_TAIL NNR_DMA_OPS);
+  if constexpr (N == 4) asm volatile(NNR_DMA_HEAD NNR_DMA_LD(0) NNR_DMA_LD(1) NNR_DMA_LD(2) NNR_DMA_LD(3) NNR_DMA_TAIL NNR_DMA_OPS);
+  if constexpr (N == 5) asm volatile(NNR_DMA_HEAD NNR_DMA_LD(0) NNR_DMA_LD(1) NNR_DMA_LD(2) NNR_DMA_LD(3) NNR_DMA_LD(4) NNR_DMA_TAIL NNR_DMA_OPS);
+  if constexpr (N == 6) asm volatile(NNR_DMA_HEAD NNR_DMA_LD(0) NNR_DMA_LD(1) NNR_DMA_LD(2) NNR_DMA_LD(3) NNR_DMA_LD(4) NNR_DMA_LD(5) NNR_DMA_TAIL NNR_DMA_OPS);
+  if constexpr (N == 7) asm volatile(NNR_DMA_HEAD NNR_DMA_LD(0) NNR_DMA_LD(1) NNR_DMA_LD(2) NNR_DMA_LD(3) NNR_DMA_LD(4) NNR_DMA_LD(5) NNR_DMA_LD(6) NNR_DMA_TAIL NNR_DMA_OPS);
+  if constexpr (N == 8) asm volatile(NNR_DMA_HEAD NNR_DMA_LD(0) NNR_DMA_LD(1) NNR_DMA_LD(2) NNR_DMA_LD(3) NNR_DMA_LD(4) NNR_DMA_LD(5) NNR_DMA_LD(6) NNR_DMA_LD(7) NNR_DMA_TAIL NNR_DMA_OPS);
+#undef NNR_DMA_HEAD
+#undef NNR_DMA_LD
+#undef NNR_DMA_TAIL
+#undef NNR_DMA_OPS
+}
+
+typedef __bf16 bf16x8_t __attribute__((ext_vector_type(8)));
+
+__device__ __forceinline__ int bx3_swzA(int r) { return ((r >> 1) & 1) | (((r >> 3) & 1) << 2); }
+__device__ __forceinline__ int bx3_swzB(int r) { return (r >> 1) & 3; }
+
+typedef unsigned u32x4_t __attribute__((ext_vector_type(4)));
+__device__ __forceinline__ unsigned hi16_pair(float odd, float even) {
+  return __builtin_amdgcn_perm(__float_as_uint(odd), __float_as_uint(even), 0x07060302u);
+}
+__device__ __forceinline__ void split3_trunc8(const f32x4& x0, const f32x4& x1, bf16x8_t& a1, bf16x8_t& a2, bf16x8_t& a3) {
+  const float xs[8] = {x0[0], x0[1], x0[2], x0[3], x1[0], x1[1], x1[2], x1[3]};
+  unsigned w1[4], w2[4], w3[4];
+#pragma unroll
+  for (int p = 0; p < 4; ++p) {
+    const float xe = xs[2 * p], xo = xs[2 * p + 1];
+    const unsigned h1 = hi16_pair(xo, xe);
+    const float re = xe - __uint_as_float(h1 << 16), ro = xo - __uint_as_float(h1 & 0xffff0000u);
+    const unsigned h2 = hi16_pair(ro, re);
+    const float se = re - __uint_as_float(h2 << 16), so = ro - __uint_as_float(h2 & 0xffff0000u);
+    w1[p] = h1; w2[p] = h2; w3[p] = hi16_pair(so, se);
+  }
+  a1 = __builtin_bit_cast(bf16x8_t, u32x4_t{w1[0], w1[1], w1[2], w1[3]});
+  a2 = __builtin_bit_cast(bf16x8_t, u32x4_t{w2[0], w2[1], w2[2], w2[3]});
+  a3 = __builtin_bit_cast(bf16x8_t, u32x4_t{w3[0], w3[1], w3[2], w3[3]});
+}
+
+template <int TM, int TN>
+__device__ __forceinline__ void bx3_stage_mma(const float* As, const __bf16* Bi, int wtile0, int r, int q, f32x4 (&acc_hi)[TM][TN], f32x4 (&acc_lo)[TM][TN]) {
+  constexpr int BN = 16 * TN, BK = 32;
+  bf16x8_t bf[3][TN];
+#pragma unroll
+  for (int img = 0; img < 3; ++img)
+#pragma unroll
+    for (int n = 0; n < TN; ++n)
+      bf[img][n] = *reinterpret_cast<const bf16x8_t*>(Bi + img * (BN * BK) + (n * 16 + r) * BK + ((q ^ bx3_swzB(r)) * 8));
+#pragma unroll
+  for (int m = 0; m < TM; ++m) {
+    const float* arow = As + ((wtile0 + m) * 16 + r) * BK;
+    const f32x4 x0 = *reinterpret_cast<const f32x4*>(arow + 4 * ((2 * q) ^ bx3_swzA(r)));
+    const f32x4 x1 = *reinterpret_cast<const f32x4*>(arow + 4 * ((2 * q + 1) ^ bx3_swzA(r)));
+    bf16x8_t a1, a2, a3;
+    split3_trunc8(x0, x1, a1, a2, a3);
+#pragma unroll
+    for (int n = 0; n < TN; ++n) {
+      acc_hi[m][n] = __builtin_amdgcn_mfma_f32_16x16x32_bf16(a1, bf[0][n], acc_hi[m][n], 0, 0, 0);
+      acc_lo[m][n] = __builtin_amdgcn_mfma_f32_16x16x32_bf16(a3, bf[0][n], acc_lo[m][n], 0, 0, 0);
+      acc_lo[m][n] = __builtin_amdgcn_mfma_f32_16x16x32_bf16(a1, bf[2][n], acc_lo[m][n], 0, 0, 0);
+      acc_lo[m][n] = __builtin_amdgcn_mfma_f32_16x16x32_bf16(a2, bf[1][n], acc_lo[m][n], 0, 0, 0);
+      acc_lo[m][n] = __builtin_amdgcn_mfma_f32_16x16x32_bf16(a2, bf[0][n], acc_lo[m][n], 0, 0, 0);
+      acc_lo[m][n] = __builtin_amdgcn_mfma_f32_16x16x32_bf16(a1, bf[1][n], acc_lo[m][n], 0, 0, 0);
+    }
+  }
+}
diff --git a/nnr_amd/csrc/gcn.hip b/nnr_amd/csrc/gcn.hip
--- a/nnr_amd/csrc/gcn.hip
+++ b/nnr_amd/csrc/gcn.hip
@@ -1,8 +1,27 @@
 #include "common.h"
+#include "bx3_loop.h"
 
 namespace {
 
 constexpr int GCN_MAXG = 128;
+
+template <int NT>
+__device__ __forceinline__ void gcn_load_graph(float* As, const float* __restrict__ A, int G, int GR, int A_LD, int tid) {
+  if ((G & 3) == 0) {
+    const int g4 = G >> 2;
+    for (int i = tid; i < G * g4; i += NT) {
+      const int row = i / g4, c = (i - row * g4) * 4;
+      const f32x4 v = *reinterpret_cast<const f32x4*>(A + row * G + c);
+#pragma unroll
+      for (int e = 0; e < 4; ++e) As[row * A_LD + c + e] = v[e];
+    }
+  } else {
+    for (int i = tid; i < GR * A_LD; i += NT) {
+      const int row = i / A_LD, col = i - row * A_LD;
+      As[i] = (row < G && col < G) ? A[row * G + col] : 0.f;
+    }
+  }
+}
 
 template <int MODE, int MT>
 __global__ __launch_bounds__(256) __attribute__((amdgpu_waves_per_eu(3, 8))) void gcn_aggregate_kernel(
@@ -17,20 +36,7 @@
   const int b = blockIdx.y, tid = threadIdx.x, lane = tid & 63, w = tid >> 6;
   const int r16 = lane & 15, kk = lane >> 4;
   const float* A = graph + (long)b * G * G;
-  if ((G & 3) == 0) {
-    const int g4 = G >> 2;
-    for (int i = tid; i < G * g4; i += 256) {
-      const int row = i / g4, c = (i - row * g4) * 4;
-      const f32x4 v = *reinterpret_cast<const f32x4*>(A + row * G + c);
-#pragma unroll
-      for (int e = 0; e < 4; ++e) As[row * A_LD + c + e] = v[e];
-    }
-  } else {
-    for (int i = tid; i < GR * A_LD; i += 256) {
-      const int row = i / A_LD, col = i - row * A_LD;
-      As[i] = (row < G && col < G) ? A[row * G + col] : 0.f;
-    }
-  }
+  gcn_load_graph<256>(As, A, G, GR, A_LD, tid);
   const int c0 = blockIdx.x * 64;
   const int c4 = (tid & 15) * 4, rr = tid >> 4;
   const bool cok = c0 + c4 < D;
@@ -117,6 +123,214 @@
   }
 }
 
+
+struct gcn_layer_args {
+  const float* A; const void* B3; long b3_stride; int ldb3;
+  const float* graph;
+  const float* vec;
+  const float* aux;
+  float* out0;
+  float* out1;
+  float* out2;
+  int B, G, D, relu; uint32_t seed, thr; float scale;
+};
+constexpr int GL_GMIN = 65, GL_GMAX = 80, GL_THREADS = 320;
+
+template <int MODE>
+__global__ __launch_bounds__(GL_THREADS) __attribute__((amdgpu_waves_per_eu(3, 3))) void gcn_layer_bx3_kernel(gcn_layer_args a) {
+  constexpr int TM = 2, TN = 5, NS = 2, NW = 5, MT = 5, GP = 16 * MT, BM = 2 * GP, BN = 16 * TN, BK = 32;
+  constexpr int A_BYTES = BM * BK * 4, B_IMG_BYTES = BN * BK * 2, STAGE_BYTES = A_BYTES + 3 * B_IMG_BYTES;
+  constexpr int NA = A_BYTES / 1024 / NW, NBW = 3 * B_IMG_BYTES / 1024 / NW, STEP = NW * 1024;
+  static_assert(NA * NW * 1024 == A_BYTES && NBW * NW * 1024 == 3 * B_IMG_BYTES && NW * TM == 2 * MT, "tile shape");
+  constexpr int Z_LD = BN + 4;
+  static_assert((GL_GMAX * (GL_GMAX | 1) + 3 + GP * Z_LD) * 4 <= NS * STAGE_BYTES, "the aggregate works out of the main loop's LDS");
+  __shared__ __attribute__((aligned(1024))) unsigned char lds_raw[NS * STAGE_BYTES];
+  const int tid = threadIdx.x, lane = tid & 63, w = __builtin_amdgcn_readfirstlane(tid >> 6), r = lane & 15, q = lane >> 4;
+  const int B = a.B, G = a.G, D = a.D;
+  const int nbm = (B + 1) >> 1, nbn = (D + BN - 1) / BN, nblk = nbm * nbn;
+  if ((int)blockIdx.x >= nblk) return;
+  int v;
+  {
+    const int b = blockIdx.x, qq = nblk >> 3, rem = nblk & 7, x = b & 7, slot = b >> 3;
+    v = x * qq + min(x, rem) + slot;
+  }
+  const int bm = v / nbn, bn = v - bm * nbn, u0 = 2 * bm, n0 = bn * BN;
+  const int S = (D + BK - 1) / BK;
+  const unsigned lds_base = (unsigned)(uintptr_t)lds_raw;
+  const float* zero = nnr_zero_page;
+  asm volatile("" : "+s"(zero));
+  unsigned voffA[8], voffB[8];
+#pragma unroll
+  for (int i = 0; i < 8; ++i) voffA[i] = voffB[i] = 0;
+#pragma unroll
+  for (int i = 0; i < NA; ++i) {
+    const int row = (w + NW * i) * 8 + lane / 8, usr = row >= GP ? 1 : 0, c = (lane % 8) ^ bx3_swzA(row & 15);
+    const int grow = (min(u0 + usr, B - 1) - u0) * G + min(row - usr * GP, G - 1);
+    voffA[i] = (unsigned)(((long)grow * D + 4 * c) * 4);
+  }
+#pragma unroll
+  for (int j = 0; j < NBW; ++j) {
+    const int idx = w + NW * j, img = idx / (BN / 16), jj = idx - img * (BN / 16), row = jj * 16 + lane / 4, c = (lane % 4) ^ bx3_swzB(row & 15);
+    voffB[j] = (unsigned)(((long)img * a.b3_stride + (long)min(row, D - 1 - n0) * a.ldb3 + 8 * c) * 2);
+  }
+  const float* Abase = a.A + (long)u0 * G * D;
+  const char* Bbase = reinterpret_cast<const char*>(reinterpret_cast<const __bf16*>(a.B3) + (long)n0 * a.ldb3);
+  const bool ktail = (D % BK) != 0;
+  auto issue = [&](int s) __attribute__((always_inline)) {
+    const int k0 = s * BK;
+    const unsigned sb = lds_base + (unsigned)((s % NS) * STAGE_BYTES) + (unsigned)(w * 1024);
+    if (!(ktail && s == S - 1)) {
+      lds_dma16_block<NA, STEP>(Abase + k0, sb, voffA);
+      lds_dma16_block<NBW, STEP>(reinterpret_cast<const float*>(Bbase + 2L * k0), sb + A_BYTES, voffB);
+      return;
+    }
+    int l = lane;
+    asm volatile("" : "+v"(l));
+#pragma unroll
+    for (int i = 0; i < NA; ++i) {
+      unsigned o = voffA[i];
+      asm volatile("" : "+v"(o));
+      const int c = (l % 8) ^ bx3_swzA(((w + NW * i) * 8 + l / 8) & 15);
+      lds_dma16((k0 + 4 * c < D) ? reinterpret_cast<const float*>(reinterpret_cast<const char*>(Abase + k0) + o) : zero, sb + (unsigned)(i * STEP));
+    }
+#pragma unroll
+    for (int j = 0; j < NBW; ++j) {
+      unsigned o = voffB[j];
+      asm volatile("" : "+v"(o));
+      const int c = (l % 4) ^ bx3_swzB((l / 4) & 15);
+      lds_dma16((k0 + 8 * c < D) ? reinterpret_cast<const float*>(Bbase + 2L * k0 + o) : zero, sb + A_BYTES + (unsigned)(j * STEP));
+    }
+  };
+  f32x4 acc[TM][TN], acc_lo[TM][TN];
+#pragma unroll
+  for (int m = 0; m < TM; ++m)
+#pragma unroll
+    for (int n = 0; n < TN; ++n) acc[m][n] = acc_lo[m][n] = f32x4{0.f, 0.f, 0.f, 0.f};
+  issue(0);
+  for (int s = 0; s < S; ++s) {
+    wait_stages<NA + NBW, NS - 2>(S - 1 - s);
+    __builtin_amdgcn_s_barrier();
+    if (s + 1 < S) issue(s + 1);
+    const unsigned char* st = lds_raw + (s % NS) * STAGE_BYTES;
+    bx3_stage_mma<TM, TN>(reinterpret_cast<const float*>(st), reinterpret_cast<const __bf16*>(st + A_BYTES), w * TM, r, q, acc, acc_lo);
+  }
+#pragma unroll
+  for (int m = 0; m < TM; ++m)
+#pragma unroll
+    for (int n = 0; n < TN; ++n) acc[m][n] += acc_lo[m][n];
+
+  const int ks_n = (G + 3) >> 2, GR = ks_n * 4, A_LD = GR | 1;
+  float* As = reinterpret_cast<float*>(lds_raw);
+  float* Zs = As + ((GR * A_LD + 3) & ~3);
+  constexpr int NV = BN / 4;
+  for (int usr = 0; usr < 2 && u0 + usr < B; ++usr) {
+    const int b = u0 + usr;
+    const long base = (long)b * G * D;
+    __syncthreads();
+    gcn_load_graph<GL_THREADS>(As, a.graph + (long)b * G * G, G, GR, A_LD, tid);
+#pragma unroll
+    for (int m = 0; m < TM; ++m) {
+      const int t = w * TM + m - usr * MT;
+      if (t >= 0 && t < MT) {
+#pragma unroll
+        for (int n = 0; n < TN; ++n)
+#pragma unroll
+          for (int e = 0; e < 4; ++e) {
+            const int row = t * 16 + 4 * q + e;
+            Zs[row * Z_LD + n * 16 + r] = row < G ? acc[m][n][e] : 0.f;
+          }
+      }
+    }
+    __syncthreads();
+    if (MODE == 1) {
+      for (int i = tid; i < GP * NV; i += GL_THREADS) {
+        const int row = i / NV, c4 = (i - row * NV) * 4;
+        if (row >= G || n0 + c4 >= D) continue;
+        const long idx = base + (long)row * D + n0 + c4;
+        f32x4 x = *reinterpret_cast<const f32x4*>(&Zs[row * Z_LD + c4]);
+        if (a.vec) x += *reinterpret_cast<const f32x4*>(a.vec + idx);
+        if (a.thr) {
+          bool kp[4];
+          nnr_keep4(a.seed, (uint64_t)idx, a.thr, kp);
+#pragma unroll
+          for (int e = 0; e < 4; ++e) x[e] = kp[e] ? x[e] * a.scale : 0.f;
+        }
+        if (a.out1) *reinterpret_cast<f32x4*>(a.out1 + idx) = x;
+        const f32x4 rv = *reinterpret_cast<const f32x4*>(a.aux + idx);
+#pragma unroll
+        for (int e = 0; e < 4; ++e) x[e] = rv[e] > 0.f ? x[e] : 0.f;
+        *reinterpret_cast<f32x4*>(a.out0 + idx) = x;
+        *reinterpret_cast<f32x4*>(&Zs[row * Z_LD + c4]) = x;
+      }
+      __syncthreads();
+    }
+    float bf[MT * 4];
+#pragma unroll
+    for (int ks = 0; ks < MT * 4; ++ks) bf[ks] = ks < ks_n ? Zs[(4 * ks + q) * Z_LD + w * 16 + r] : 0.f;
+    f32x4 agg[MT];
+    int arow[MT];
+#pragma unroll
+    for (int m = 0; m < MT; ++m) {
+      agg[m] = f32x4{0.f, 0.f, 0.f, 0.f};
+      arow[m] = min(m * 16 + r, GR - 1);
+    }
+#pragma unroll
+    for (int ks = 0; ks < MT * 4; ++ks) {
+      if (ks < ks_n) {
+#pragma unroll
+        for (int m = 0; m < MT; ++m) {
+          const float av = MODE == 0 ? As[arow[m] * A_LD + 4 * ks + q] : As[(4 * ks + q) * A_LD + arow[m]];
+          agg[m] = __builtin_amdgcn_mfma_f32_16x16x4f32(av, bf[ks], agg[m], 0, 0, 0);
+        }
+      }
+    }
+    __syncthreads();
+#pragma unroll
+    for (int m = 0; m < MT; ++m)
+#pragma unroll
+      for (int e = 0; e < 4; ++e) Zs[(m * 16 + 4 * q + e) * Z_LD + w * 16 + r] = agg[m][e];
+    __syncthreads();
+    for (int i = tid; i < GP * NV; i += GL_THREADS) {
+      const int row = i / NV, c4 = (i - row * NV) * 4;
+      if (row >= G || n0 + c4 >= D) continue;
+      const long idx = base + (long)row * D + n0 + c4;
+      f32x4 x = *reinterpret_cast<const f32x4*>(&Zs[row * Z_LD + c4]);
+      if (MODE == 0) {
+        if (a.vec) x += *reinterpret_cast<const f32x4*>(a.vec + n0 + c4);
+        if (a.relu) {
+#pragma unroll
+          for (int e = 0; e < 4; ++e) x[e] = fmaxf(x[e], 0.f);
+        }
+        if (a.out1) *reinterpret_cast<f32x4*>(a.out1 + idx) = x;
+        if (a.aux) x += *reinterpret_cast<const f32x4*>(a.aux + idx);
+        if (a.thr) {
+          bool kp[4];
+          nnr_keep4(a.seed, (uint64_t)idx, a.thr, kp);
+#pragma unroll
+          for (int e = 0; e < 4; ++e) x[e] = kp[e] ? x[e] * a.scale : 0.f;
+        }
+        *reinterpret_cast<f32x4*>(a.out0 + idx) = x;
+      } else {
+        *reinterpret_cast<f32x4*>(a.out2 + idx) = x;
+      }
+    }
+  }
+}
+
+int gcn_layer_launch(int mode, gcn_layer_args a, float p, hipStream_t stream) {
+  auto al = [](const void* q) { return ((uintptr_t)q & 15) == 0; };
+  if (!a.graph || !a.A || !a.out0 || a.B <= 0 || a.G <= 0 || a.D <= 0) return NNR_ERR_ARG;
+  if (mode == 1 && (!a.aux || !a.out2)) return NNR_ERR_ARG;
+  if (a.G < GL_GMIN || a.G > GL_GMAX || (a.D & 3) || !a.B3 || (a.ldb3 & 7) || a.ldb3 < a.D || ((a.b3_stride * 2) & 15)) return NNR_ERR_UNSUPPORTED;
+  if (!(al(a.A) && al(a.B3) && al(a.vec) && al(a.aux) && al(a.out0) && al(a.out1) && al(a.out2)) || (!(a.G & 3) && !al(a.graph))) return NNR_ERR_UNSUPPORTED;
+  a.thr = nnr_drop_thresh(p);
+  a.scale = p > 0.f ? 1.f / (1.f - p) : 1.f;
+  const dim3 grid(((a.B + 1) / 2) * ((a.D + 79) / 80));
+  if (mode == 0) hipLaunchKernelGGL((gcn_layer_bx3_kernel<0>), grid, dim3(GL_THREADS), 0, stream, a);
+  else hipLaunchKernelGGL((gcn_layer_bx3_kernel<1>), grid, dim3(GL_THREADS), 0, stream, a);
+  NNR_CHECK_LAUNCH();
+  return NNR_OK;
+}
 
 }
 
@@ -147,3 +361,16 @@
   NNR_CHECK_LAUNCH();
   return NNR_OK;
 }
+
+extern "C" int nnr_gcn_layer_fwd(const float* graph, const float* x, const void* w3, long w3_stride, int ldw3, const float* bias, const float* resid,
+                                 float* r_out, float* y, int B, int G, int D, int relu, float p, uint32_t seed, hipStream_t stream) {
+  gcn_layer_args a = {x, w3, w3_stride, ldw3, graph, bias, resid, y, r_out, nullptr, B, G, D, relu, seed, 0u, 1.f};
+  return gcn_layer_launch(0, a, p, stream);
+}
+
+extern "C" int nnr_gcn_layer_bwd(const float* graph, const float* dz_in, const void* wt3, long wt3_stride, int ldwt3, const float* pre_add, const float* r,
+                                 float* ds, float* dx0, float* dz, int B, int G, int D, float p, uint32_t seed, hipStream_t stream) {
+  if (!ds) return NNR_ERR_ARG;
+  gcn_layer_args a = {dz_in, wt3, wt3_stride, ldwt3, graph, pre_add, r, ds, dx0, dz, B, G, D, 0, seed, 0u, 1.f};
+  return gcn_layer_launch(1, a, p, stream);
+}
diff --git a/nnr_amd/csrc/gemm.hip b/nnr_amd/csrc/gemm.hip
--- a/nnr_amd/csrc/gemm.hip
+++ b/nnr_amd/csrc/gemm.hip
@@ -1,4 +1,5 @@
 #include "common.h"
+#include "bx3_loop.h"
 #include <stdlib.h>
 #include <type_traits>
 
@@ -432,13 +433,7 @@
 }
 
 
-__device__ __attribute__((aligned(1024))) float nnr_zero_page[512] = {};
-
-__device__ __forceinline__ void lds_dma16(const float* gsrc, unsigned lds_dst) {
-  unsigned keep;
-  asm volatile("s_mov_b32 %0, m0\n\ts_mov_b32 m0, %2\n\ts_nop 0\n\tglobal_load_lds_dwordx4 %1, off\n\ts_mov_b32 m0, %0"
-               : "=&s"(keep) : "v"(gsrc), "s"(lds_dst) : "memory");
-}
+
 __device__ __forceinline__ void set_prio_dyn(unsigned p) {
   switch (p & 3) {
     case 0: __builtin_amdgcn_s_setprio(0); break;
@@ -448,16 +443,6 @@
   }
 }
 
-template <int N>
-__device__ __forceinline__ void wait_vmcnt() { asm volatile("s_waitcnt vmcnt(%0)" ::"n"(N) : "memory"); }
-template <int CNT, int MAXA>
-__device__ __forceinline__ void wait_stages(int ahead) {
-  if constexpr (MAXA == 0) wait_vmcnt<0>();
-  else {
-    if (ahead >= MAXA) wait_vmcnt<CNT * MAXA>();
-    else wait_stages<CNT, MAXA - 1>(ahead);
-  }
-}
 
 template <int TM, int TN, int BK, int NS, int OCC, int PRIO = 0>
 __global__ __launch_bounds__(256, OCC) void gemm_nt_pipe_kernel(nnr_gemm_args g) {
@@ -603,28 +588,6 @@
   gemm_epilogue<TM, TN>(g, acc, lds, C, m0, n0, M, N, z);
 }
 
-template <int N>
-__device__ __forceinline__ void lds_dma16_block(const float* sbase, unsigned lds_dst, const unsigned (&voff)[8]) {
-  unsigned keep;
-  static_assert(N >= 1 && N <= 8, "1..8 loads per block");
-#define NNR_DMA_HEAD "s_mov_b32 %[keep], m0\n\ts_mov_b32 m0, %[dst]\n\t"
-#define NNR_DMA_LD(I) "s_nop 0\n\tglobal_load_lds_dwordx4 %[v" #I "], %[sb]\n\ts_add_u32 m0, m0, 0x1000\n\t"
-#define NNR_DMA_TAIL "s_mov_b32 m0, %[keep]"
-#define NNR_DMA_OPS : [keep] "=&s"(keep) : [dst] "s"(lds_dst), [sb] "s"(sbase), [v0] "v"(voff[0]), [v1] "v"(voff[1]), [v2] "v"(voff[2]), [v3] "v"(voff[3]), \
-                      [v4] "v"(voff[4]), [v5] "v"(voff[5]), [v6] "v"(voff[6]), [v7] "v"(voff[7]) : "memory", "scc"
-  if constexpr (N == 1) asm volatile(NNR_DMA_HEAD NNR_DMA_LD(0) NNR_DMA_TAIL NNR_DMA_OPS);
-  if constexpr (N == 2) asm volatile(NNR_DMA_HEAD NNR_DMA_LD(0) NNR_DMA_LD(1) NNR_DMA_TAIL NNR_DMA_OPS);
-  if constexpr (N == 3) asm volatile(NNR_DMA_HEAD NNR_DMA_LD(0) NNR_DMA_LD(1) NNR_DMA_LD(2) NNR_DMA_TAIL NNR_DMA_OPS);
-  if constexpr (N == 4) asm volatile(NNR_DMA_HEAD NNR_DMA_LD(0) NNR_DMA_LD(1) NNR_DMA_LD(2) NNR_DMA_LD(3) NNR_DMA_TAIL NNR_DMA_OPS);
-  if constexpr (N == 5) asm volatile(NNR_DMA_HEAD NNR_DMA_LD(0) NNR_DMA_LD(1) NNR_DMA_LD(2) NNR_DMA_LD(3) NNR_DMA_LD(4) NNR_DMA_TAIL NNR_DMA_OPS);
-  if constexpr (N == 6) asm volatile(NNR_DMA_HEAD NNR_DMA_LD(0) NNR_DMA_LD(1) NNR_DMA_LD(2) NNR_DMA_LD(3) NNR_DMA_LD(4) NNR_DMA_LD(5) NNR_DMA_TAIL NNR_DMA_OPS);
-  if constexpr (N == 7) asm volatile(NNR_DMA_HEAD NNR_DMA_LD(0) NNR_DMA_LD(1) NNR_DMA_LD(2) NNR_DMA_LD(3) NNR_DMA_LD(4) NNR_DMA_LD(5) NNR_DMA_LD(6) NNR_DMA_TAIL NNR_DMA_OPS);
-  if constexpr (N == 8) asm volatile(NNR_DMA_HEAD NNR_DMA_LD(0) NNR_DMA_LD(1) NNR_DMA_LD(2) NNR_DMA_LD(3) NNR_DMA_LD(4) NNR_DMA_LD(5) NNR_DMA_LD(6) NNR_DMA_LD(7) NNR_DMA_TAIL NNR_DMA_OPS);
-#undef NNR_DMA_HEAD
-#undef NNR_DMA_LD
-#undef NNR_DMA_TAIL
-#undef NNR_DMA_OPS
-}
 
 template <int TM, int TN, int NS, int OCC>
 __global__ __launch_bounds__(256, OCC) void gemm_nt_pipe2_kernel(nnr_gemm_args g) {
@@ -845,7 +808,6 @@
          al(g.A) && al(g.B) && (g.batch <= 1 || (((g.strideA | g.strideB) & 3) == 0)) && (g.dyn_dim == 0 || g.dyn_dim == 1);
 }
 
-typedef __bf16 bf16x8_t __attribute__((ext_vector_type(8)));
 __device__ __forceinline__ void split3_bf16(float x, __bf16& h1, __bf16& h2, __bf16& h3) {
   const unsigned u = __builtin_bit_cast(unsigned, x), mag = u & 0x7fffffffu;
   const bool big = mag >= 0x7f7f8000u, nonfinite = mag >= 0x7f800000u;
@@ -865,29 +827,7 @@
     out[i] = a; out[img_stride + i] = b; out[2 * img_stride + i] = d;
   }
 }
-__device__ __forceinline__ int bx3_swzA(int r) { return ((r >> 1) & 1) | (((r >> 3) & 1) << 2); }
-__device__ __forceinline__ int bx3_swzB(int r) { return (r >> 1) & 3; }
-
-typedef unsigned u32x4_t __attribute__((ext_vector_type(4)));
-__device__ __forceinline__ unsigned hi16_pair(float odd, float even) {
-  return __builtin_amdgcn_perm(__float_as_uint(odd), __float_as_uint(even), 0x07060302u);
-}
-__device__ __forceinline__ void split3_trunc8(const f32x4& x0, const f32x4& x1, bf16x8_t& a1, bf16x8_t& a2, bf16x8_t& a3) {
-  const float xs[8] = {x0[0], x0[1], x0[2], x0[3], x1[0], x1[1], x1[2], x1[3]};
-  unsigned w1[4], w2[4], w3[4];
-#pragma unroll
-  for (int p = 0; p < 4; ++p) {
-    const float xe = xs[2 * p], xo = xs[2 * p + 1];
-    const unsigned h1 = hi16_pair(xo, xe);
-    const float re = xe - __uint_as_float(h1 << 16), ro = xo - __uint_as_float(h1 & 0xffff0000u);
-    const unsigned h2 = hi16_pair(ro, re);
-    const float se = re - __uint_as_float(h2 << 16), so = ro - __uint_as_float(h2 & 0xffff0000u);
-    w1[p] = h1; w2[p] = h2; w3[p] = hi16_pair(so, se);
-  }
-  a1 = __builtin_bit_cast(bf16x8_t, u32x4_t{w1[0], w1[1], w1[2], w1[3]});
-  a2 = __builtin_bit_cast(bf16x8_t, u32x4_t{w2[0], w2[1], w2[2], w2[3]});
-  a3 = __builtin_bit_cast(bf16x8_t, u32x4_t{w3[0], w3[1], w3[2], w3[3]});
-}
+
 
 template <int TM, int TN, int NS>
 __global__ __launch_bounds__(256, (NS * (64 * TM * 128 + 3 * 16 * TN * 64) > 80 * 1024 ? 1 : 2)) void gemm_nt_bx3_kernel(nnr_gemm_args g) {
@@ -971,29 +911,7 @@
     const unsigned char* st = lds_raw + (s % NS) * STAGE_BYTES;
     const float* As = reinterpret_cast<const float*>(st);
     const __bf16* Bi = reinterpret_cast<const __bf16*>(st + A_BYTES);
-    bf16x8_t bf[3][TN];
-#pragma unroll
-    for (int img = 0; img < 3; ++img)
-#pragma unroll
-      for (int n = 0; n < TN; ++n)
-        bf[img][n] = *reinterpret_cast<const bf16x8_t*>(Bi + img * (BN * BK) + (n * 16 + r) * BK + ((q ^ bx3_swzB(r)) * 8));
-#pragma unroll
-    for (int m = 0; m < TM; ++m) {
-      const float* arow = As + ((w * TM + m) * 16 + r) * BK;
-      const f32x4 x0 = *reinterpret_cast<const f32x4*>(arow + 4 * ((2 * q) ^ bx3_swzA(r)));
-      const f32x4 x1 = *reinterpret_cast<const f32x4*>(arow + 4 * ((2 * q + 1) ^ bx3_swzA(r)));
-      bf16x8_t a1, a2, a3;
-      split3_trunc8(x0, x1, a1, a2, a3);
-#pragma unroll
-      for (int n = 0; n < TN; ++n) {
-        acc_hi[m][n] = __builtin_amdgcn_mfma_f32_16x16x32_bf16(a1, bf[0][n], acc_hi[m][n], 0, 0, 0);
-        acc_lo[m][n] = __builtin_amdgcn_mfma_f32_16x16x32_bf16(a3, bf[0][n], acc_lo[m][n], 0, 0, 0);
-        acc_lo[m][n] = __builtin_amdgcn_mfma_f32_16x16x32_bf16(a1, bf[2][n], acc_lo[m][n], 0, 0, 0);
-        acc_lo[m][n] = __builtin_amdgcn_mfma_f32_16x16x32_bf16(a2, bf[1][n], acc_lo[m][n], 0, 0, 0);
-        acc_lo[m][n] = __builtin_amdgcn_mfma_f32_16x16x32_bf16(a2, bf[0][n], acc_lo[m][n], 0, 0, 0);
-        acc_lo[m][n] = __builtin_amdgcn_mfma_f32_16x16x32_bf16(a1, bf[1][n], acc_lo[m][n], 0, 0, 0);
-      }
-    }
+    bx3_stage_mma<TM, TN>(As, Bi, w * TM, r, q, acc_hi, acc_lo);
   }
 #pragma unroll
   for (int m = 0; m < TM; ++m)
diff --git a/nnr_amd/csrc/tape.hip b/nnr_amd/csrc/tape.hip
--- a/nnr_amd/csrc/tape.hip
+++ b/nnr_amd/csrc/tape.hip
@@ -29,7 +29,7 @@
   R(nnr_lstm_fwd), R(nnr_lstm_bwd), R(nnr_attn_pool_fwd), R(nnr_attn_pool_bwd), R(nnr_gate_bwd), R(nnr_packed_seq_sum),
   R(nnr_tanh_score_bwd), R(nnr_colsum), R(nnr_rowdot), R(nnr_small_embed_fwd), R(nnr_small_embed_bwd), R(nnr_embed_gather),
   R(nnr_embed_scatter), R(nnr_embed_scatter_dyn), R(nnr_transpose2d), R(nnr_transpose_batch), R(nnr_add), R(nnr_add_atomic), R(nnr_add2d), R(nnr_expand_rows_fwd), R(nnr_expand_rows_bwd),
-  R(nnr_dropout), R(nnr_relu_bwd), R(nnr_gcn_aggregate_fwd), R(nnr_gcn_aggregate_bwd), R(nnr_relu_drop_bwd), R(nnr_mhsa_fwd), R(nnr_mhsa_bwd),
+  R(nnr_dropout), R(nnr_relu_bwd), R(nnr_gcn_aggregate_fwd), R(nnr_gcn_aggregate_bwd), R(nnr_gcn_layer_fwd), R(nnr_gcn_layer_bwd), R(nnr_relu_drop_bwd), R(nnr_mhsa_fwd), R(nnr_mhsa_bwd),
   R(nnr_sue_x0_fwd), R(nnr_sue_x0_bwd), R(nnr_sue_slice_fwd), R(nnr_sue_slice_bwd), R(nnr_sue_intra_fwd), R(nnr_sue_intra_bwd),
   R(nnr_corpus_batch), R(nnr_history_graph), R(nnr_logits_loss_fwd), R(nnr_logits_fwd), R(nnr_nls_loss), R(nnr_logits_bwd),
   R(nnr_layernorm_fwd), R(nnr_layernorm_bwd), R(nnr_sumsq), R(nnr_sumsq_part), R(nnr_clip_adam), R(nnr_dp_allreduce), R(nnr_dp_broadcast), R(nnr_dp_busy), R(nnr_split_bf16x3), R(nnr_mhsa_fwd_packed), R(nnr_mhsa_bwd_packed), R(nnr_mhsa_pair_map), R(nnr_mhsa_fwd_paired), R(nnr_mhsa_bwd_paired), R(nnr_mask_cover), R(nnr_seq_rowmap),
diff --git a/nnr_amd/ops.py b/nnr_amd/ops.py
--- a/nnr_amd/ops.py
+++ b/nnr_amd/ops.py
@@ -408,6 +408,27 @@
     return (not trans_a and not trans_b and a_idx is None and b_idx is None and split_k <= 1 and k_chunk <= 0 and rowdot_w is None
             and colsum_out is None and batch <= 1 and dyn_dim in (0, 1) and M >= _BX3_MIN_ROWS and K >= 64 and N * K <= (1 << 22)
             and (K | lda | ldb) & 3 == 0 and (A.data_ptr() | B.data_ptr()) & 15 == 0 and (drop is None or drop[0] in (3, 4) or drop[1] <= 0.0))
+
+
+def bx3_takes(A, B, M, N, K, lda, ldb, trans_a=False, trans_b=False, a_idx=None, b_idx=None, c_idx=None, split_k=1, k_chunk=0, rowdot_w=None,
+              colsum_out=None, atomic=False, batch=1, dyn_dim=0, drop=None, tile=0, seen=False):
+    if not (BX3[0] and tile in (0, 9, 15, 16) and _bx3_wanted(A, B, M, N, K, lda, ldb, trans_a, trans_b, a_idx, b_idx, c_idx, split_k, k_chunk, rowdot_w,
+                                                              colsum_out, atomic, batch, dyn_dim, drop)):
+        return False
+    is_w = is_weight(B)
+    if seen:
+        key = (M, N, K, 'weight' if is_w else 'other')
+        BX3_SEEN[key] = BX3_SEEN.get(key, 0) + 1
+    return is_w and bx3_class(N, K) in _BX3_CLASSES
+
+
+GCN_FUSED_G = (65, 80)
+
+
+def gcn_layer_fused(x, w, G, layer_norm=False):
+    M, K = x.shape
+    return (not layer_norm and GCN_FUSED_G[0] <= G <= GCN_FUSED_G[1] and M % G == 0 and tuple(w.shape) == (K, K) and x.is_contiguous()
+            and w.is_contiguous() and bx3_takes(x, w, M, K, K, K, K))
 
 
 def gemm(A, B, C_=None, *, M, N, K, lda, ldb, ldc=0, trans_a=False, trans_b=False, dyn=None, dyn_dim=0, a_idx=None, b_idx=None,
@@ -465,15 +486,11 @@
         g.pre_add, g.ldpre = pre_add.data_ptr(), ldpre
     if gate_bwd:
         g.gate_bwd = 1
-    if b3 is None and BX3[0] and tile in (0, 9, 15, 16) and _bx3_wanted(A, B, M, N, K, lda, ldb, trans_a, trans_b, a_idx, b_idx, c_idx, split_k, k_chunk, rowdot_w,
-                                                                    colsum_out, atomic, batch, dyn_dim, drop):
-        is_w = is_weight(B)
-        key = (M, N, K, 'weight' if is_w else 'other')
-        BX3_SEEN[key] = BX3_SEEN.get(key, 0) + 1
-        if is_w and bx3_class(N, K) in _BX3_CLASSES:
-            b3 = bx3_images(B, N, K, ldb)
-            tile = _BX3_TILE
-            g.tile = _BX3_TILE
+    if b3 is None and bx3_takes(A, B, M, N, K, lda, ldb, trans_a, trans_b, a_idx, b_idx, c_idx, split_k, k_chunk, rowdot_w, colsum_out, atomic, batch,
+                                dyn_dim, drop, tile, seen=True):
+        b3 = bx3_images(B, N, K, ldb)
+        tile = _BX3_TILE
+        g.tile = _BX3_TILE
     if b3 is not None:
         g.B3, g.b3_stride, g.ldb3 = b3[0].data_ptr(), b3[1], b3[2]
     if slab is None and TN_SLAB and trans_a and trans_b and split_k > 1 and not k_chunk and c_idx is None and (N & 3) == 0 and C_ is not None:
@@ -904,6 +921,35 @@
         L.check(L.lib().nnr_gcn_aggregate_bwd(_p(graph), _p(dy), _p(r), _p(ds), _p(dx0), _p(dz), B, G, D, p, seed, _s()), 'nnr_gcn_aggregate_bwd')
 
 
+def _gcn_layer_span(family, B, G, D, arrays):
+    if not _prof.active():
+        return _NOSPAN
+    M = B * G
+
+    def flops(vals=None):
+        return 2.0 * M * D * D
+
+    def op_bytes(vals=None):
+        return 4.0 * (M * D * arrays + D * D + B * G * G)
+    flops.dyn, flops.scale, flops.bytes_fn = [], 1.0, op_bytes
+    flops.tag = 'M%d N%d K%d G%d' % (M, D, D, G)
+    return _prof.span(family, flops)
+
+
+def gcn_layer_fwd(graph, x, w, bias, resid, r_out, y, B, G, D, relu, p, seed):
+    img, stride, ldo = bx3_images(w, D, D, w.stride(0))
+    with _gcn_layer_span('gemm_nt_bx3_gcn_fwd', B, G, D, 3 + (1 if resid is not None else 0)):
+        L.check(L.lib().nnr_gcn_layer_fwd(_p(graph), _p(x), _p(img), stride, ldo, _p(bias), _p(resid), _p(r_out), _p(y), B, G, D, int(bool(relu)), p, seed,
+                                          _s()), 'nnr_gcn_layer_fwd')
+
+
+def gcn_layer_bwd(graph, dz_in, wT, pre_add, r, ds, dx0, dz, B, G, D, p, seed):
+    img, stride, ldo = bx3_images(wT, D, D, D)
+    with _gcn_layer_span('gemm_nt_bx3_gcn_bwd', B, G, D, 4 + (1 if pre_add is not None else 0) + (1 if dx0 is not None else 0)):
+        L.check(L.lib().nnr_gcn_layer_bwd(_p(graph), _p(dz_in), _p(img), stride, ldo, _p(pre_add), _p(r), _p(ds), _p(dx0), _p(dz), B, G, D, p, seed, _s()),
+                'nnr_gcn_layer_bwd')
+
+
 def sue_x0_fwd(hist, proxy, x0, B, Hn, Kc, D, p, seed, cmask_fix=None):
     if cmask_fix is not None:
         assert cmask_fix.is_contiguous() and cmask_fix.element_size() == 1 and tuple(cmask_fix.shape) == (B, Kc + 1)
diff --git a/nnr_amd/profile.py b/nnr_amd/profile.py
--- a/nnr_amd/profile.py
+++ b/nnr_amd/profile.py
@@ -14,6 +14,7 @@
     'gemm_tn_64x80k64': 'gemm_kernel<1, 5, true, true, 64>',
     'gemm_nt_pipe128x80': 'gemm_nt_pipe_kernel<2, 5, 16, 3, 4, 0>', 'gemm_nt_pipe128x80s2': 'gemm_nt_pipe_kernel<2, 5, 16, 2, 5, 0>',
     'gemm_nt_bx3_128x80': 'gemm_nt_bx3_kernel<2, 5, 2>', 'gemm_nt_bx3_64x80': 'gemm_nt_bx3_kernel<1, 5, 2>',
+    'gemm_nt_bx3_gcn_fwd': 'gcn_layer_bx3_kernel<0>', 'gemm_nt_bx3_gcn_bwd': 'gcn_layer_bx3_kernel<1>',
     'gemm_nt_pipe2_128x80': 'gemm_nt_pipe2_kernel<2, 5, 3, 2>', 'gemm_nt_pipe2_128x64': 'gemm_nt_pipe2_kernel<2, 4, 3, 2>',
     'gemm_tn_pipe2_128x80': 'gemm_tn_pipe2_kernel<2, 5, 3, 3>', 'gemm_tn_pipe2_128x208': 'gemm_tn_pipe2_kernel<2, 13, 3, 2>', 'gemm_tn_pipe2_128x160': 'gemm_tn_pipe2_kernel<2, 10, 3, 2>', 'gemm_tn_pipe2_64x208': 'gemm_tn_pipe2_kernel<1, 13, 3, 2>',
     'gemm_tn_pipe128x80': 'gemm_tn_pipe_kernel<2, 5, 3, 3, 0>', 'gemm_tn_pipe128x208': 'gemm_tn_pipe_kernel<2, 13, 3, 2, 0>',
diff --git a/nnr_amd/user_encoders.py b/nnr_amd/user_encoders.py
--- a/nnr_amd/user_encoders.py
+++ b/nnr_amd/user_encoders.py
@@ -65,6 +65,13 @@
         y = torch.empty((B, G, D), **f32)
         r = torch.empty((B, G, D), **f32)
         pl = (gcn.dropout_rate if training else 0.0) if l + 1 < Lg else 0.0
+        if ops.gcn_layer_fused(x.view(B * G, D), layer.W.weight, G, getattr(layer, 'layer_norm', False)):
+            ops.gcn_layer_fwd(graph, x, layer.W.weight, layer.W.bias, x if gcn.residual else None, r, y, B, G, D, True, pl, seed0 + l)
+            lns.append(None)
+            xs.append(y)
+            rs.append(r)
+            x = y
+            continue
         z = ops.linear_fwd(x.view(B * G, D), layer.W.weight)
         if getattr(layer, 'layer_norm', False):
             u = torch.empty((B, G, D), **f32)
@@ -93,19 +100,34 @@
     B, G, D = dy.shape
     f32 = dict(device=dy.device, dtype=torch.float32)
     Lg = gcn.num_layers
+    nxt = None
     for l in range(Lg - 1, -1, -1):
         layer = gcn.gcn_layers[l]
         pl = (gcn.dropout_rate if gsv['training'] else 0.0) if l + 1 < Lg else 0.0
+        if G <= 128 and D % 4 == 0 and gsv['lns'][l] is None:
+            if nxt is None:
+                dS, dz = torch.empty((B, G, D), **f32), torch.empty((B, G, D), **f32)
+                dx = torch.empty((B, G, D), **f32) if gcn.residual else None
+                ops.gcn_aggregate_bwd(graph, dy, gsv['rs'][l], dS, dx, dz, B, G, D, pl, gsv['seed0'] + l)
+            else:
+                dS, dx, dz = nxt
+            nxt = None
+            w = layer.W.weight
+            wT = ops.wt(w) if l > 0 and B * G >= 1024 and w.is_contiguous() else None
+            if wT is not None and gsv['lns'][l - 1] is None and ops.gcn_layer_fused(dz.view(B * G, D), wT, G):
+                pm = gcn.dropout_rate if gsv['training'] else 0.0
+                nxt = (torch.empty((B, G, D), **f32), torch.empty((B, G, D), **f32) if gcn.residual else None, torch.empty((B, G, D), **f32))
+                ops.gcn_layer_bwd(graph, dz, wT, dx, gsv['rs'][l - 1], nxt[0], nxt[1], nxt[2], B, G, D, pm, gsv['seed0'] + l - 1)
+            else:
+                if dx is None:
+                    dx = torch.empty((B, G, D), **f32)
+                ops.linear_bwd_data(dz.view(B * G, D), w, out=dx.view(B * G, D), accumulate=bool(gcn.residual))
+                dy = dx
+            leaf(lambda dS=dS, dz=dz, l=l, layer=layer: (ops.bias_grad(dS.view(B * G, D), grad_of(layer.W.bias)),
+                                                         ops.linear_bwd_weight(dz.view(B * G, D), gsv['xs'][l].view(B * G, D), grad_of(layer.W.weight))), dS, dz)
+            continue
         dS = torch.empty((B, G, D), **f32)
         dx = torch.empty((B, G, D), **f32)
-        if G <= 128 and D % 4 == 0 and gsv['lns'][l] is None:
-            dz = torch.empty((B, G, D), **f32)
-            ops.gcn_aggregate_bwd(graph, dy, gsv['rs'][l], dS, dx if gcn.residual else None, dz, B, G, D, pl, gsv['seed0'] + l)
-            ops.linear_bwd_data(dz.view(B * G, D), layer.W.weight, out=dx.view(B * G, D), accumulate=bool(gcn.residual))
-            leaf(lambda dS=dS, dz=dz, l=l, layer=layer: (ops.bias_grad(dS.view(B * G, D), grad_of(layer.W.bias)),
-                                                         ops.linear_bwd_weight(dz.view(B * G, D), gsv['xs'][l].view(B * G, D), grad_of(layer.W.weight))), dS, dz)
-            dy = dx
-            continue
         ops.relu_drop_bwd(dy, gsv['rs'][l], dS, dx, pl, gsv['seed0'] + l)
         if not gcn.residual:
             ops.fill_zero(dx)
```

After: 6498. -3.4%, worse.
